# RWAlgorithms/ConjugateGradientOptim.jl

Hardware: NVIDIA B200
Metric: cg_iterations_per_s (higher is better)
Workload: dtype f64

## Files before the change

conjugategradientoptim.jl_b200/csrc/blas1.cu:

```cuda
#include "internal.cuh"
#include "reduce.cuh"

template <class Op>
__global__ void __launch_bounds__(CGO_B, Op::OCC) k_blas1(Op op, int64_t n, RedArgs red) {
    constexpr int K = Op::K;
    __shared__ double sm[K * CGO_NW];
    const int64_t nq = (n + 1) >> 1;
    constexpr int64_t tileq = (int64_t)CGO_B * CGO_U_VEC;
    const int64_t ntiles = (nq + tileq - 1) / tileq;
    const int nact = (int)(ntiles < (int64_t)red.G ? ntiles : (int64_t)red.G);
    cgo_wait_flags(red, BarAll());
    op.prologue();
    for (int v = blockIdx.x; v < nact; v += gridDim.x) {
        double acc[K];
#pragma unroll
        for (int k = 0; k < K; ++k) acc[k] = 0.0;
        for (int64_t tile = v; tile < ntiles; tile += red.G) {
            const int64_t q0 = tile * tileq + threadIdx.x;
            typename Op::In in[CGO_U_VEC];
#pragma unroll
            for (int j = 0; j < CGO_U_VEC; ++j) {
                const int64_t q = q0 + (int64_t)j * CGO_B;
                if (q < nq) in[j] = op.load(q);
            }
#pragma unroll
            for (int j = 0; j < CGO_U_VEC; ++j) {
                const int64_t q = q0 + (int64_t)j * CGO_B;
                if (q < nq) op.apply(q, in[j], acc, 2 * q + 1 < n);
            }
        }
        cgo_cta_combine<K>(acc, sm);
        cgo_publish<K>(red, v, acc);
    }
    cgo_grid_finish<K>(red, nact, sm);
}

template <class Op>
static int launch_blas1(cgo_ctx *c, const Op &op, int64_t n, const RedArgs &red) {
    const int64_t nq = (n + 1) >> 1;
    const int64_t tileq = (int64_t)CGO_B * CGO_U_VEC;
    int64_t ntiles = (nq + tileq - 1) / tileq;
    int64_t nact = ntiles < red.G ? ntiles : red.G;
    int64_t phys = (int64_t)c->sms * Op::OCC;
    int grid = (int)(nact < phys ? nact : phys);
    if (grid < 1) grid = 1;
    cgo_timer_begin(c, Op::TCLASS);
    k_blas1<Op><<<grid, CGO_B, 0, c->stream>>>(op, n, red);
    cgo_timer_end(c);
    c->launches++;
    CGO_CUDA(cudaGetLastError());
    return 0;
}

__device__ __forceinline__ double2 ld2rw(const double2 *p) {
    double2 r;
    asm volatile("ld.global.L1::no_allocate.v2.f64 {%0, %1}, [%2];" : "=d"(r.x), "=d"(r.y) : "l"(p) : "memory");
    return r;
}

template <bool FUSED>
struct RosenTrial {
    static constexpr int TCLASS = CGO_T_TRIAL;
    static constexpr int K = 9;
    static constexpr int OCC = 2;
    struct In { double2 x, u, g; };
    const double2 *x, *g;
    double2 *u;
    double2 *xp, *gp;
    double a, beta;
    __device__ __forceinline__ void prologue() {}
    __device__ __forceinline__ In load(int64_t q) const {
        In r;
        r.x = cgo_ld2(x + q);
        r.g = cgo_ld2(g + q);
        r.u = FUSED ? ld2rw(u + q) : cgo_ld2(u + q);
        return r;
    }
    __device__ __forceinline__ void apply(int64_t q, const In &in, double (&acc)[K], bool) const {
        double2 uu = in.u;
        if (FUSED) {
            uu.x = -in.g.x + beta * in.u.x;
            uu.y = -in.g.y + beta * in.u.y;
            cgo_st2(u + q, uu);
        }
        double2 p;
        p.x = in.x.x + a * uu.x;
        p.y = in.x.y + a * uu.y;
        cgo_st2(xp + q, p);
        const double t = p.y - p.x * p.x;
        const double om = 1.0 - p.x;
        const double f = (100.0 * t) * t + om * om;
        double2 gn;
        gn.x = (-400.0 * p.x) * t - 2.0 * om;
        gn.y = 200.0 * t;
        cgo_st2(gp + q, gn);
        const double y1 = gn.x - in.g.x, y2 = gn.y - in.g.y;
        acc[CGO_P_PHI] = acc[CGO_P_PHI] + f;
        acc[CGO_P_DPHI] = acc[CGO_P_DPHI] + gn.x * uu.x;   acc[CGO_P_DPHI] = acc[CGO_P_DPHI] + gn.y * uu.y;
        acc[CGO_P_GPGP] = acc[CGO_P_GPGP] + gn.x * gn.x;   acc[CGO_P_GPGP] = acc[CGO_P_GPGP] + gn.y * gn.y;
        acc[CGO_P_YY] = acc[CGO_P_YY] + y1 * y1;           acc[CGO_P_YY] = acc[CGO_P_YY] + y2 * y2;
        acc[CGO_P_UY] = acc[CGO_P_UY] + uu.x * y1;         acc[CGO_P_UY] = acc[CGO_P_UY] + uu.y * y2;
        acc[CGO_P_YGP] = acc[CGO_P_YGP] + y1 * gn.x;       acc[CGO_P_YGP] = acc[CGO_P_YGP] + y2 * gn.y;
        acc[CGO_P_GPG] = acc[CGO_P_GPG] + gn.x * in.g.x;   acc[CGO_P_GPG] = acc[CGO_P_GPG] + gn.y * in.g.y;
        acc[CGO_P_UG] = acc[CGO_P_UG] + uu.x * in.g.x;     acc[CGO_P_UG] = acc[CGO_P_UG] + uu.y * in.g.y;
        acc[CGO_P_UU] = acc[CGO_P_UU] + uu.x * uu.x;       acc[CGO_P_UU] = acc[CGO_P_UU] + uu.y * uu.y;
    }
};

template <bool RESET>
struct DirUpdate {
    static constexpr int TCLASS = CGO_T_DIR;
    static constexpr int K = 2;
    static constexpr int OCC = 4;
    struct In { double2 g, u; };
    const double2 *g;
    double2 *u;
    double beta;
    __device__ __forceinline__ void prologue() {}
    __device__ __forceinline__ In load(int64_t q) const {
        In r;
        r.g = cgo_ld2(g + q);
        if (!RESET) r.u = ld2rw(u + q);
        return r;
    }
    __device__ __forceinline__ void apply(int64_t q, const In &in, double (&acc)[K], bool v2) const {
        double2 un;
        if (RESET) { un.x = -in.g.x; un.y = -in.g.y; }
        else { un.x = -in.g.x + beta * in.u.x; un.y = -in.g.y + beta * in.u.y; }
        if (!v2) un.y = 0.0;
        cgo_st2(u + q, un);
        acc[CGO_D_GU] = acc[CGO_D_GU] + in.g.x * un.x;
        acc[CGO_D_UU] = acc[CGO_D_UU] + un.x * un.x;
        if (v2) {
            acc[CGO_D_GU] = acc[CGO_D_GU] + in.g.y * un.y;
            acc[CGO_D_UU] = acc[CGO_D_UU] + un.y * un.y;
        }
    }
};

struct BetaLiteral {
    static constexpr int TCLASS = CGO_T_OTHER;
    static constexpr int K = 1;
    static constexpr int OCC = 2;
    struct In { double2 gp, g, u; };
    const double2 *gp, *g, *u;
    double R, m;
    __device__ __forceinline__ void prologue() {}
    __device__ __forceinline__ In load(int64_t q) const {
        In r;
        r.gp = cgo_ld2(gp + q); r.g = cgo_ld2(g + q); r.u = cgo_ld2(u + q);
        return r;
    }
    __device__ __forceinline__ void apply(int64_t, const In &in, double (&acc)[K], bool v2) const {
        const double y1 = in.gp.x - in.g.x;
        const double t2a = in.gp.x / R;
        const double t1a = y1 - m * in.u.x;
        acc[0] = acc[0] + t1a * t2a;
        if (v2) {
            const double y2 = in.gp.y - in.g.y;
            const double t2b = in.gp.y / R;
            const double t1b = y2 - m * in.u.y;
            acc[0] = acc[0] + t1b * t2b;
        }
    }
};

struct NormUPlusG {
    static constexpr int TCLASS = CGO_T_OTHER;
    static constexpr int K = 1;
    static constexpr int OCC = 4;
    struct In { double2 g, u; };
    const double2 *g, *u;
    __device__ __forceinline__ void prologue() {}
    __device__ __forceinline__ In load(int64_t q) const {
        In r;
        r.g = cgo_ld2(g + q); r.u = cgo_ld2(u + q);
        return r;
    }
    __device__ __forceinline__ void apply(int64_t, const In &in, double (&acc)[K], bool v2) const {
        const double t1 = in.u.x + in.g.x;
        acc[0] = acc[0] + t1 * t1;
        if (v2) { const double t2 = in.u.y + in.g.y; acc[0] = acc[0] + t2 * t2; }
    }
};

template <bool FUSED, int PUSH>
struct AxpyDir {
    static constexpr int TCLASS = CGO_T_AXPY;
    static constexpr int K = 3;
    static constexpr int OCC = 2;
    struct In { double2 x, u, g; };
    const double2 *x, *g;
    double2 *u, *xp;
    double a, beta;
    double2 *prev_right, *next_left;
    int64_t hq, nq;
    void *const *dst_all;
    int nranks;
    __device__ __forceinline__ void prologue() {}
    __device__ __forceinline__ In load(int64_t q) const {
        In r;
        r.x = cgo_ld2(x + q);
        r.g = cgo_ld2(g + q);
        r.u = FUSED ? ld2rw(u + q) : cgo_ld2(u + q);
        return r;
    }
    __device__ __forceinline__ void apply(int64_t q, const In &in, double (&acc)[K], bool v2) const {
        double2 uu = in.u;
        if (FUSED) {
            uu.x = -in.g.x + beta * in.u.x;
            uu.y = v2 ? -in.g.y + beta * in.u.y : 0.0;
            cgo_st2(u + q, uu);
        }
        double2 p;
        p.x = in.x.x + a * uu.x;
        p.y = v2 ? in.x.y + a * uu.y : 0.0;
        cgo_st2(xp + q, p);
        if (PUSH == 1) {
            if (q < hq) cgo_st2(prev_right + q, p);
            if (q >= nq - hq) cgo_st2(next_left + (q - (nq - hq)), p);
        }
        if (PUSH == 2) {
            for (int r = 0; r < nranks; ++r) cgo_st2((double2 *)dst_all[r] + q, p);
        }
        acc[0] = acc[0] + in.g.x * uu.x;
        acc[1] = acc[1] + uu.x * uu.x;
        acc[2] = acc[2] + p.x * p.x;
        if (v2) {
            acc[0] = acc[0] + in.g.y * uu.y;
            acc[1] = acc[1] + uu.y * uu.y;
            acc[2] = acc[2] + p.y * p.y;
        }
    }
};

struct GradCombine {
    static constexpr int TCLASS = CGO_T_OTHER;
    static constexpr int K = 8;
    static constexpr int OCC = 2;
    struct In { double2 s, u, g, w; };
    const double2 *q, *u, *g, *w;
    double2 *gp;
    int nparts;
    int64_t stride2;
    double invN, lambda;
    __device__ __forceinline__ void prologue() {}
    __device__ __forceinline__ In load(int64_t i) const {
        In r;
        r.s = ld2rw(q + i);
        for (int p = 1; p < nparts; ++p) {
            const double2 t = ld2rw(q + (int64_t)p * stride2 + i);
            r.s.x = r.s.x + t.x;
            r.s.y = r.s.y + t.y;
        }
        r.u = cgo_ld2(u + i); r.g = cgo_ld2(g + i); r.w = cgo_ld2(w + i);
        return r;
    }
    __device__ __forceinline__ void apply(int64_t i, const In &in, double (&acc)[K], bool v2) const {
        double2 gn;
        gn.x = in.s.x * invN + lambda * in.w.x;
        gn.y = v2 ? in.s.y * invN + lambda * in.w.y : 0.0;
        cgo_st2(gp + i, gn);
        const double ux = in.u.x, uy = v2 ? in.u.y : 0.0, gx = in.g.x, gy = v2 ? in.g.y : 0.0;
        const double y1 = gn.x - gx, y2 = gn.y - gy;
        acc[CGO_P_DPHI - 1] = acc[CGO_P_DPHI - 1] + gn.x * ux;
        acc[CGO_P_GPGP - 1] = acc[CGO_P_GPGP - 1] + gn.x * gn.x;
        acc[CGO_P_YY - 1] = acc[CGO_P_YY - 1] + y1 * y1;
        acc[CGO_P_UY - 1] = acc[CGO_P_UY - 1] + ux * y1;
        acc[CGO_P_YGP - 1] = acc[CGO_P_YGP - 1] + y1 * gn.x;
        acc[CGO_P_GPG - 1] = acc[CGO_P_GPG - 1] + gn.x * gx;
        acc[CGO_P_UG - 1] = acc[CGO_P_UG - 1] + ux * gx;
        acc[CGO_P_UU - 1] = acc[CGO_P_UU - 1] + ux * ux;
        if (v2) {
            acc[CGO_P_DPHI - 1] = acc[CGO_P_DPHI - 1] + gn.y * uy;
            acc[CGO_P_GPGP - 1] = acc[CGO_P_GPGP - 1] + gn.y * gn.y;
            acc[CGO_P_YY - 1] = acc[CGO_P_YY - 1] + y2 * y2;
            acc[CGO_P_UY - 1] = acc[CGO_P_UY - 1] + uy * y2;
            acc[CGO_P_YGP - 1] = acc[CGO_P_YGP - 1] + y2 * gn.y;
            acc[CGO_P_GPG - 1] = acc[CGO_P_GPG - 1] + gn.y * gy;
            acc[CGO_P_UG - 1] = acc[CGO_P_UG - 1] + uy * gy;
            acc[CGO_P_UU - 1] = acc[CGO_P_UU - 1] + uy * uy;
        }
    }
};

struct VecSumSq {
    static constexpr int TCLASS = CGO_T_OTHER;
    static constexpr int K = 1;
    static constexpr int OCC = 4;
    struct In { double2 a; };
    const double2 *a;
    __device__ __forceinline__ void prologue() {}
    __device__ __forceinline__ In load(int64_t q) const { return In{cgo_ld2(a + q)}; }
    __device__ __forceinline__ void apply(int64_t, const In &in, double (&acc)[K], bool v2) const {
        acc[0] = acc[0] + in.a.x * in.a.x;
        if (v2) acc[0] = acc[0] + in.a.y * in.a.y;
    }
};
struct Dots3 {
    static constexpr int TCLASS = CGO_T_OTHER;
    static constexpr int K = 3;
    static constexpr int OCC = 4;
    struct In { double2 a, b; };
    const double2 *a, *b;
    __device__ __forceinline__ void prologue() {}
    __device__ __forceinline__ In load(int64_t q) const { return In{cgo_ld2(a + q), cgo_ld2(b + q)}; }
    __device__ __forceinline__ void apply(int64_t, const In &in, double (&acc)[K], bool v2) const {
        acc[0] = acc[0] + in.a.x * in.b.x; acc[1] = acc[1] + in.b.x * in.b.x; acc[2] = acc[2] + in.a.x * in.a.x;
        if (v2) { acc[0] = acc[0] + in.a.y * in.b.y; acc[1] = acc[1] + in.b.y * in.b.y; acc[2] = acc[2] + in.a.y * in.a.y; }
    }
};
struct GradDots {
    static constexpr int TCLASS = CGO_T_OTHER;
    static constexpr int K = 8;
    static constexpr int OCC = 2;
    struct In { double2 gp, g, u; };
    const double2 *gp, *g, *u;
    __device__ __forceinline__ void prologue() {}
    __device__ __forceinline__ In load(int64_t q) const { return In{cgo_ld2(gp + q), cgo_ld2(g + q), cgo_ld2(u + q)}; }
    __device__ __forceinline__ void one(double gn, double gg, double uu, double (&acc)[K]) const {
        const double y = gn - gg;
        acc[CGO_P_DPHI - 1] = acc[CGO_P_DPHI - 1] + gn * uu;
        acc[CGO_P_GPGP - 1] = acc[CGO_P_GPGP - 1] + gn * gn;
        acc[CGO_P_YY - 1] = acc[CGO_P_YY - 1] + y * y;
        acc[CGO_P_UY - 1] = acc[CGO_P_UY - 1] + uu * y;
        acc[CGO_P_YGP - 1] = acc[CGO_P_YGP - 1] + y * gn;
        acc[CGO_P_GPG - 1] = acc[CGO_P_GPG - 1] + gn * gg;
        acc[CGO_P_UG - 1] = acc[CGO_P_UG - 1] + uu * gg;
        acc[CGO_P_UU - 1] = acc[CGO_P_UU - 1] + uu * uu;
    }
    __device__ __forceinline__ void apply(int64_t, const In &in, double (&acc)[K], bool v2) const {
        one(in.gp.x, in.g.x, in.u.x, acc);
        if (v2) one(in.gp.y, in.g.y, in.u.y, acc);
    }
};

template <bool PUSH>
struct LogitLoss {
    static constexpr int TCLASS = CGO_T_OTHER;
    static constexpr int K = 1;
    static constexpr int OCC = 2;
    struct In { double2 z, y; };
    double2 *zc;
    const double2 *y;
    void *const *dst_all;
    int nranks;
    __device__ __forceinline__ void prologue() {}
    __device__ __forceinline__ In load(int64_t q) const { return In{ld2rw(zc + q), cgo_ld2(y + q)}; }
    __device__ __forceinline__ double one(double z, double yy, double (&acc)[K]) const {
        const double t = -yy * z;
        const double e = exp(-fabs(t));
        const double l = (t > 0.0 ? t : 0.0) + log1p(e);
        const double sg = t >= 0.0 ? 1.0 / (1.0 + e) : e / (1.0 + e);
        acc[0] = acc[0] + l;
        return -yy * sg;
    }
    __device__ __forceinline__ void apply(int64_t q, const In &in, double (&acc)[K], bool v2) const {
        double2 c;
        c.x = one(in.z.x, in.y.x, acc);
        c.y = v2 ? one(in.z.y, in.y.y, acc) : 0.0;
        cgo_st2(zc + q, c);
        if (PUSH) for (int r = 0; r < nranks; ++r) cgo_st2((double2 *)dst_all[r] + q, c);
    }
};

struct SolveSysProject {
    static constexpr int TCLASS = CGO_T_OTHER;
    static constexpr int K = 1;
    static constexpr int OCC = 4;
    struct In { double2 b, g; };
    const double2 *base, *gp;
    double2 *xn;
    double m;
    __device__ __forceinline__ void prologue() {}
    __device__ __forceinline__ In load(int64_t q) const {
        In r;
        r.b = ld2rw(base + q); r.g = cgo_ld2(gp + q);
        return r;
    }
    __device__ __forceinline__ void apply(int64_t q, const In &in, double (&acc)[K], bool v2) const {
        double2 o;
        o.x = in.b.x + m * in.g.x;
        o.y = v2 ? in.b.y + m * in.g.y : 0.0;
        cgo_st2(xn + q, o);
        acc[0] = acc[0] + o.x * o.x;
        if (v2) acc[0] = acc[0] + o.y * o.y;
    }
};

struct LbfgsStage {
    static constexpr int TCLASS = CGO_T_LBFGS;
    static constexpr int K = 2;
    static constexpr int OCC = 2;
    struct In { double2 xp, x, gp, g; };
    const double2 *xp, *x, *gp, *g;
    double2 *S, *Y;
    __device__ __forceinline__ void prologue() {}
    __device__ __forceinline__ In load(int64_t q) const {
        In r;
        r.xp = cgo_ld2(xp + q); r.x = cgo_ld2(x + q); r.gp = cgo_ld2(gp + q); r.g = cgo_ld2(g + q);
        return r;
    }
    __device__ __forceinline__ void apply(int64_t q, const In &in, double (&acc)[K], bool v2) const {
        double2 s, y;
        s.x = in.xp.x - in.x.x; y.x = in.gp.x - in.g.x;
        s.y = v2 ? in.xp.y - in.x.y : 0.0; y.y = v2 ? in.gp.y - in.g.y : 0.0;
        cgo_st2(S + q, s); cgo_st2(Y + q, y);
        acc[0] = acc[0] + s.x * y.x; acc[1] = acc[1] + y.x * y.x;
        if (v2) { acc[0] = acc[0] + s.y * y.y; acc[1] = acc[1] + y.y * y.y; }
    }
};

template <int MODE>
struct LbfgsStep {
    static constexpr int TCLASS = CGO_T_LBFGS;
    static constexpr int K = (MODE == 4) ? 2 : 1;
    static constexpr int OCC = 2;
    struct In { double2 q, a, b; };
    double2 *q;
    const double2 *A;
    const double2 *B;
    double2 *uout;
    const double *dprev;
    const double *alpha_dot;
    double rho_prev, gamma;
    double coef;
    __device__ __forceinline__ void prologue() {
        if (MODE == 1 || MODE == 2) coef = rho_prev * __ldcg(dprev);
        if (MODE == 3 || MODE == 4) coef = rho_prev * __ldcg(alpha_dot) - rho_prev * __ldcg(dprev);
    }
    __device__ __forceinline__ In load(int64_t i) const {
        In r;
        if (MODE != 0) r.q = ld2rw(q + i);
        r.a = cgo_ld2(A + i);
        r.b = cgo_ld2(B + i);
        return r;
    }
    __device__ __forceinline__ void apply(int64_t i, const In &in, double (&acc)[K], bool v2) const {
        double2 qn;
        if (MODE == 0) { qn = in.a; }
        else if (MODE == 1 || MODE == 2) { qn.x = in.q.x - coef * in.a.x; qn.y = in.q.y - coef * in.a.y; }
        else { qn.x = in.q.x + in.a.x * coef; qn.y = in.q.y + in.a.y * coef; }
        if (MODE == 2) { qn.x = gamma * qn.x; qn.y = gamma * qn.y; }
        if (!v2) qn.y = 0.0;
        if (MODE == 4) {
            double2 un; un.x = -qn.x; un.y = v2 ? -qn.y : 0.0;
            cgo_st2(uout + i, un);
            acc[0] = acc[0] + in.b.x * un.x; acc[1] = acc[1] + un.x * un.x;
            if (v2) { acc[0] = acc[0] + in.b.y * un.y; acc[1] = acc[1] + un.y * un.y; }
        } else {
            cgo_st2(q + i, qn);
            acc[0] = acc[0] + in.b.x * qn.x;
            if (v2) acc[0] = acc[0] + in.b.y * qn.y;
        }
    }
};

static inline uint64_t h_mix64(uint64_t z) {
    z ^= z >> 30; z *= 0xBF58476D1CE4E5B9ULL;
    z ^= z >> 27; z *= 0x94D049BB133111EBULL;
    z ^= z >> 31;
    return z;
}
double cgo_host_u01(uint64_t seed, uint64_t i, uint64_t k) {
    uint64_t h = h_mix64(seed + 0x9E3779B97F4A7C15ULL);
    h = h_mix64(h ^ (i + 0x9E3779B97F4A7C15ULL));
    h = h_mix64(h ^ (k + 0x632BE59BD9B4E019ULL));
    return (double)(h >> 11) * (1.0 / 9007199254740992.0);
}

struct RosenObj : cgo_obj {
    int eval_trial(cgo_state *st, double a, bool fused, double beta, double *out) override {
        RedArgs red = cgo_red_args(ctx);
        if (fused) {
            RosenTrial<true> op;
            op.x = (const double2 *)st->x; op.g = (const double2 *)st->g; op.u = (double2 *)st->u;
            op.xp = (double2 *)st->xp; op.gp = (double2 *)st->gp; op.a = a; op.beta = beta;
            CGO_TRY(launch_blas1(ctx, op, st->n, red));
        } else {
            RosenTrial<false> op;
            op.x = (const double2 *)st->x; op.g = (const double2 *)st->g; op.u = (double2 *)st->u;
            op.xp = (double2 *)st->xp; op.gp = (double2 *)st->gp; op.a = a; op.beta = 0.0;
            CGO_TRY(launch_blas1(ctx, op, st->n, red));
        }
        CGO_TRY(cgo_finish_pack(ctx, 9, out));
        out[CGO_P_DIR_GU] = out[CGO_P_UG];
        out[CGO_P_DIR_UU] = out[CGO_P_UU];
        return 0;
    }
    double bytes_per_eval() const override { return 8.0 * 5.0 * (double)n_local; }
    void reduction_site(int32_t *V, int32_t *U) const override { *V = 2; *U = CGO_U_VEC; }
    int default_x0(uint64_t seed, double perturb, double *x0) override {
        for (int64_t i = 0; i < n_local; ++i) {
            int64_t gi = offset + i;
            double base = (gi % 2 == 0) ? -1.2 : 1.0;
            x0[i] = perturb != 0.0 ? base + perturb * (2.0 * cgo_host_u01(seed, (uint64_t)gi, 0) - 1.0) : base;
        }
        return 0;
    }
};

__global__ void k_scalar_to_pack(const double *src, double *dst) { *dst = *src; }
struct UserObj : cgo_obj {
    cgo_user_fdf fn = nullptr;
    void *user = nullptr;
    double *d_f = nullptr;
    ~UserObj() override {
        if (ctx && cgo_ctx_alive(ctx)) cudaSetDevice(ctx->device);
        cudaFree(d_f);
    }
    int eval_trial(cgo_state *st, double a, bool fused, double beta, double *out) override {
        CGO_TRY(cgo_blas1_axpy_dir(st, a, fused, beta));
        const int rc = fn(user, (void *)ctx->stream, st->n, offset, st->xp, st->gp, d_f);
        CGO_CHECK(rc == 0, "user objective callback returned %d", rc);
        k_scalar_to_pack<<<1, 1, 0, ctx->stream>>>(d_f, cgo_red_args(ctx, CGO_P_PHI).out);
        ctx->launches++;
        CGO_CUDA(cudaGetLastError());
        CGO_TRY(cgo_blas1_grad_dots(st));
        return cgo_finish_pack(ctx, 12, out);
    }
    double bytes_per_eval() const override { return 8.0 * 6.0 * (double)n_local; }
    void reduction_site(int32_t *V, int32_t *U) const override { *V = 2; *U = CGO_U_VEC; }
    int default_x0(uint64_t, double, double *x0) override {
        for (int64_t i = 0; i < n_local; ++i) x0[i] = 0.0;
        return 0;
    }
};
extern "C" int cgo_obj_user_create(cgo_ctx *ctx, int64_t n_global, cgo_user_fdf fdf, void *user, cgo_obj **out) {
    CGO_CHECK(ctx && fdf && out, "NULL argument");
    CGO_CHECK(n_global >= 2 && n_global % 2 == 0, "user objective: need an even n >= 2 (got %lld; pad with a fixed coordinate)", (long long)n_global);
    CGO_CUDA(cudaSetDevice(ctx->device));
    int64_t lo, hi;
    CGO_TRY(cgo_shard_range(n_global, ctx->nranks, ctx->rank, 2, &lo, &hi));
    UserObj *o = new UserObj();
    o->ctx = ctx; o->fn = fdf; o->user = user;
    o->n_global = n_global; o->offset = lo; o->n_local = hi - lo;
    if (cudaMalloc(&o->d_f, sizeof(double)) != cudaSuccess) { delete o; cgo_set_error("cudaMalloc failed"); return 1; }
    *out = o;
    return 0;
}

struct RosenChainedEval {
    static constexpr int TCLASS = CGO_T_TRIAL;
    static constexpr int K = 9;
    static constexpr int OCC = 2;
    struct In { double2 p, u, g; double pm, pn; };
    const double *xp;
    const double2 *u, *g;
    double2 *gp;
    int64_t offset, n_global, n_local;
    __device__ __forceinline__ void prologue() {}
    __device__ __forceinline__ In load(int64_t q) const {
        In r;
        r.p = cgo_ld2((const double2 *)xp + q);
        r.u = cgo_ld2(u + q); r.g = cgo_ld2(g + q);
        const int64_t i0 = 2 * q, i1 = 2 * q + 1;
        r.pm = offset + i0 > 0 ? __ldg(xp + i0 - 1) : 0.0;
        r.pn = offset + i1 + 1 < n_global ? __ldg(xp + i1 + 1) : 0.0;
        return r;
    }
    __device__ __forceinline__ void dots(double gn, double gg, double uu, double (&acc)[K]) const {
        const double y = gn - gg;
        acc[CGO_P_DPHI] = acc[CGO_P_DPHI] + gn * uu;
        acc[CGO_P_GPGP] = acc[CGO_P_GPGP] + gn * gn;
        acc[CGO_P_YY] = acc[CGO_P_YY] + y * y;
        acc[CGO_P_UY] = acc[CGO_P_UY] + uu * y;
        acc[CGO_P_YGP] = acc[CGO_P_YGP] + y * gn;
        acc[CGO_P_GPG] = acc[CGO_P_GPG] + gn * gg;
        acc[CGO_P_UG] = acc[CGO_P_UG] + uu * gg;
        acc[CGO_P_UU] = acc[CGO_P_UU] + uu * uu;
    }
    __device__ __forceinline__ void apply(int64_t q, const In &in, double (&acc)[K], bool v2) const {
        const int64_t gi0 = offset + 2 * q, gi1 = gi0 + 1;
        const double x0 = in.p.x, x1 = in.p.y;
        const double tm = x0 - in.pm * in.pm;
        const double t0 = x1 - x0 * x0;
        const double t1 = in.pn - x1 * x1;
        const double om0 = 1.0 - x0, om1 = 1.0 - x1;
        double2 gn;
        double g0 = 0.0, f0 = 0.0;
        if (gi0 > 0) g0 = g0 + 200.0 * tm;
        if (gi0 < n_global - 1) { g0 = g0 + (-2.0 * om0 - (400.0 * x0) * t0); f0 = om0 * om0 + (100.0 * t0) * t0; }
        gn.x = g0;
        acc[CGO_P_PHI] = acc[CGO_P_PHI] + f0;
        dots(g0, in.g.x, in.u.x, acc);
        gn.y = 0.0;
        if (v2) {
            double g1 = 0.0, f1 = 0.0;
            g1 = g1 + 200.0 * t0;
            if (gi1 < n_global - 1) { g1 = g1 + (-2.0 * om1 - (400.0 * x1) * t1); f1 = om1 * om1 + (100.0 * t1) * t1; }
            gn.y = g1;
            acc[CGO_P_PHI] = acc[CGO_P_PHI] + f1;
            dots(g1, in.g.y, in.u.y, acc);
        }
        cgo_st2(gp + q, gn);
    }
};

struct RosenChainedObj : cgo_obj {
    int eval_trial(cgo_state *st, double a, bool fused, double beta, double *out) override {
        const int R = ctx->nranks, me = ctx->rank;
        RedArgs red = cgo_red_args(ctx, CGO_P_PHI);
        if (R > 1 && st->peer_x) {
            const int prev = (me + R - 1) % R, next = (me + 1) % R;
            const unsigned long long e = ++ctx->epoch;
            unsigned long long *fprev = (unsigned long long *)ctx->flags_peer[(size_t)prev];
            unsigned long long *fnext = (unsigned long long *)ctx->flags_peer[(size_t)next];
            int64_t plo, phi;
            CGO_TRY(cgo_shard_range(n_global, R, prev, 2, &plo, &phi));
            HaloPush hp;
            hp.prev_right = (double *)st->xpeers[st->xp_alloc][(size_t)prev] + halo + (phi - plo);
            hp.next_left = (double *)st->xpeers[st->xp_alloc][(size_t)next];
            hp.sig_prev = fprev + CGO_F_XP_FROM_NEXT;
            hp.sig_next = fnext + CGO_F_XP_FROM_PREV;
            hp.epoch = e;
            CGO_TRY(cgo_blas1_axpy_dir(st, a, fused, beta, &hp));
            red.wait0 = ctx->flags_local + CGO_F_XP_FROM_PREV; red.wait1 = ctx->flags_local + CGO_F_XP_FROM_NEXT;
            red.wait_val = e;
        } else {
            CGO_TRY(cgo_blas1_axpy_dir(st, a, fused, beta));
            if (R > 1) CGO_TRY(cgo_sendrecv_ring(ctx, st->xp, st->xp + st->n, st->xp + st->n - halo, st->xp - halo, halo));
        }
        RosenChainedEval op;
        op.xp = st->xp; op.u = (const double2 *)st->u; op.g = (const double2 *)st->g; op.gp = (double2 *)st->gp;
        op.offset = offset; op.n_global = n_global; op.n_local = st->n;
        CGO_TRY(launch_blas1(ctx, op, st->n, red));
        return cgo_finish_pack(ctx, 12, out);
    }
    double bytes_per_eval() const override { return 8.0 * 7.0 * (double)n_local; }
    void reduction_site(int32_t *V, int32_t *U) const override { *V = 2; *U = CGO_U_VEC; }
    int default_x0(uint64_t seed, double perturb, double *x0) override {
        for (int64_t i = 0; i < n_local; ++i) {
            int64_t gi = offset + i;
            double base = (gi % 2 == 0) ? -1.2 : 1.0;
            x0[i] = perturb != 0.0 ? base + perturb * (2.0 * cgo_host_u01(seed, (uint64_t)gi, 0) - 1.0) : base;
        }
        return 0;
    }
};
extern "C" int cgo_obj_rosenbrock_chained_create(cgo_ctx *ctx, int64_t n_global, cgo_obj **out) {
    CGO_CHECK(ctx && out, "NULL argument");
    CGO_CHECK(n_global >= 2 && n_global % 2 == 0, "chained Rosenbrock: need an even n >= 2 (got %lld)", (long long)n_global);
    CGO_CHECK(ctx->nranks == 1 || n_global >= 4 * ctx->nranks, "chained Rosenbrock: %d ranks need n >= %d", ctx->nranks, 4 * ctx->nranks);
    int64_t lo, hi;
    CGO_TRY(cgo_shard_range(n_global, ctx->nranks, ctx->rank, 2, &lo, &hi));
    RosenChainedObj *o = new RosenChainedObj();
    o->ctx = ctx;
    o->n_global = n_global;
    o->offset = lo;
    o->n_local = hi - lo;
    o->halo = ctx->nranks > 1 ? 2 : 0;
    for (int q = 0; q < ctx->nranks; ++q) {
        int64_t a, b;
        cgo_shard_range(n_global, ctx->nranks, q, 2, &a, &b);
        if (b - a > o->n_alloc) o->n_alloc = b - a;
    }
    *out = o;
    return 0;
}

extern "C" int cgo_obj_rosenbrock_create(cgo_ctx *ctx, int64_t n_global, cgo_obj **out) {
    CGO_CHECK(ctx && out, "NULL argument");
    CGO_CHECK(n_global >= 2 && n_global % 2 == 0, "extended Rosenbrock needs an even n >= 2 (got %lld)", (long long)n_global);
    RosenObj *o = new RosenObj();
    o->ctx = ctx;
    o->n_global = n_global;
    int64_t lo, hi;
    CGO_TRY(cgo_shard_range(n_global, ctx->nranks, ctx->rank, 2, &lo, &hi));
    o->offset = lo;
    o->n_local = hi - lo;
    *out = o;
    return 0;
}
int cgo_obj::hessvec_dir(cgo_state *, double *) {
    cgo_set_error("this objective has no Hessian-vector product (CSR least squares has)");
    return 2;
}
int cgo_obj::quad_begin(cgo_state *, double *) {
    cgo_set_error("this objective has no quadratic-aware line search (CSR least squares has)");
    return 2;
}
int cgo_obj::quad_accept(cgo_state *, double, double *) {
    cgo_set_error("this objective has no quadratic-aware line search (CSR least squares has)");
    return 2;
}
extern "C" int cgo_quad_begin(cgo_state *st, double out[CGO_PACK_LEN]) {
    CGO_CHECK(st && out, "NULL argument");
    return st->obj->quad_begin(st, out);
}
extern "C" int cgo_quad_accept(cgo_state *st, double a, double out[CGO_PACK_LEN]) {
    CGO_CHECK(st && out, "NULL argument");
    return st->obj->quad_accept(st, a, out);
}
struct ResidualAxpy {
    static constexpr int TCLASS = CGO_T_AXPY;
    static constexpr int K = 1;
    static constexpr int OCC = 4;
    struct In { double2 r, v; };
    double2 *r;
    const double2 *v;
    double a;
    __device__ __forceinline__ void prologue() {}
    __device__ __forceinline__ In load(int64_t q) const {
        In o;
        o.r = ld2rw(r + q); o.v = cgo_ld2(v + q);
        return o;
    }
    __device__ __forceinline__ void apply(int64_t q, const In &in, double (&acc)[K], bool v2) const {
        double2 o;
        o.x = in.r.x + a * in.v.x;
        o.y = v2 ? in.r.y + a * in.v.y : 0.0;
        cgo_st2(r + q, o);
        acc[0] = acc[0] + o.x * o.x;
        if (v2) acc[0] = acc[0] + o.y * o.y;
    }
};
int cgo_blas1_residual_axpy(cgo_ctx *c, double *r, const double *v, double a, int64_t nrows, int slot) {
    ResidualAxpy op;
    op.r = (double2 *)r; op.v = (const double2 *)v; op.a = a;
    return launch_blas1(c, op, nrows, cgo_red_args(c, slot));
}
extern "C" int cgo_hessvec_dir(cgo_state *st, double out[CGO_PACK_LEN]) {
    CGO_CHECK(st && out, "NULL argument");
    if (!st->hv) {
        CGO_CUDA(cudaMalloc(&st->hv, sizeof(double) * (size_t)(st->n + 4)));
        CGO_CUDA(cudaMemsetAsync(st->hv, 0, sizeof(double) * (size_t)(st->n + 4), st->ctx->stream));
    }
    return st->obj->hessvec_dir(st, out);
}
extern "C" int cgo_obj_destroy(cgo_obj *o) {
    delete o;
    return 0;
}
extern "C" int cgo_obj_dims(cgo_obj *o, int64_t *nl, int64_t *ng, int64_t *off) {
    CGO_CHECK(o != nullptr, "NULL objective");
    if (nl) *nl = o->n_local;
    if (ng) *ng = o->n_global;
    if (off) *off = o->offset;
    return 0;
}
extern "C" int cgo_obj_reduction_site(cgo_obj *o, int32_t *V, int32_t *U) {
    CGO_CHECK(o && V && U, "NULL argument");
    o->reduction_site(V, U);
    return 0;
}
extern "C" int cgo_obj_bytes_per_eval(cgo_obj *o, double *bytes) {
    CGO_CHECK(o && bytes, "NULL argument");
    *bytes = o->bytes_per_eval();
    return 0;
}
extern "C" int cgo_obj_default_x0(cgo_obj *o, uint64_t seed, double perturb, double *x0) {
    CGO_CHECK(o && x0, "NULL argument");
    return o->default_x0(seed, perturb, x0);
}

struct BarrierFinish {
    static constexpr int TCLASS = CGO_T_OTHER;
    static constexpr int K = 9;
    static constexpr int OCC = 2;
    struct In { double2 xp, gp, u, g, lo, hi; };
    const double2 *xp, *u, *g, *lo, *hi;
    double2 *gp;
    double t;
    __device__ __forceinline__ void prologue() {}
    __device__ __forceinline__ In load(int64_t q) const {
        In r;
        r.xp = cgo_ld2(xp + q); r.gp = ld2rw(gp + q); r.u = cgo_ld2(u + q); r.g = cgo_ld2(g + q);
        r.lo = cgo_ld2(lo + q); r.hi = cgo_ld2(hi + q);
        return r;
    }
    __device__ __forceinline__ void one(double x, double g0, double uu, double gg, double lb, double ub, double &gn,
                                        double (&acc)[K]) const {
        double fu = x - ub, fl = lb - x;
        if (fu > 0.0) fu = 0.0;
        if (fl > 0.0) fl = 0.0;
        const double term = log(-fu) + log(-fl);
        double dpsi = 0.0 - 1.0 / fu;
        dpsi = dpsi - (-1.0) / fl;
        gn = t * g0 + dpsi;
        const double y = gn - gg;
        acc[CGO_P_PHI] = acc[CGO_P_PHI] + term;
        acc[CGO_P_DPHI] = acc[CGO_P_DPHI] + gn * uu;
        acc[CGO_P_GPGP] = acc[CGO_P_GPGP] + gn * gn;
        acc[CGO_P_YY] = acc[CGO_P_YY] + y * y;
        acc[CGO_P_UY] = acc[CGO_P_UY] + uu * y;
        acc[CGO_P_YGP] = acc[CGO_P_YGP] + y * gn;
        acc[CGO_P_GPG] = acc[CGO_P_GPG] + gn * gg;
        acc[CGO_P_UG] = acc[CGO_P_UG] + uu * gg;
        acc[CGO_P_UU] = acc[CGO_P_UU] + uu * uu;
    }
    __device__ __forceinline__ void apply(int64_t q, const In &in, double (&acc)[K], bool v2) const {
        double2 gn;
        one(in.xp.x, in.gp.x, in.u.x, in.g.x, in.lo.x, in.hi.x, gn.x, acc);
        if (v2) one(in.xp.y, in.gp.y, in.u.y, in.g.y, in.lo.y, in.hi.y, gn.y, acc);
        else gn.y = 0.0;
        cgo_st2(gp + q, gn);
    }
};
struct BoxInfeasible {
    static constexpr int TCLASS = CGO_T_OTHER;
    static constexpr int K = 1;
    static constexpr int OCC = 4;
    struct In { double2 x, lo, hi; };
    const double2 *x, *lo, *hi;
    __device__ __forceinline__ void prologue() {}
    __device__ __forceinline__ In load(int64_t q) const {
        In r;
        r.x = cgo_ld2(x + q); r.lo = cgo_ld2(lo + q); r.hi = cgo_ld2(hi + q);
        return r;
    }
    __device__ __forceinline__ void apply(int64_t, const In &in, double (&acc)[K], bool v2) const {
        if (in.x.x - in.hi.x >= 0.0 || in.lo.x - in.x.x >= 0.0) acc[0] = acc[0] + 1.0;
        if (v2 && (in.x.y - in.hi.y >= 0.0 || in.lo.y - in.x.y >= 0.0)) acc[0] = acc[0] + 1.0;
    }
};

struct BarrierObj : cgo_obj {
    cgo_obj *inner = nullptr;
    double *lo = nullptr, *hi = nullptr;
    double t = 1.0;
    ~BarrierObj() override {
        if (ctx && cgo_ctx_alive(ctx)) cudaSetDevice(ctx->device);
        cudaFree(lo); cudaFree(hi);
    }
    int eval_trial(cgo_state *st, double a, bool fused, double beta, double *out) override {
        double in[CGO_PACK_LEN];
        CGO_TRY(inner->eval_trial(st, a, fused, beta, in));
        BarrierFinish op;
        op.xp = (const double2 *)st->xp; op.gp = (double2 *)st->gp; op.u = (const double2 *)st->u;
        op.g = (const double2 *)st->g; op.lo = (const double2 *)lo; op.hi = (const double2 *)hi; op.t = t;
        CGO_TRY(launch_blas1(ctx, op, st->n, cgo_red_args(ctx)));
        CGO_TRY(cgo_finish_pack(ctx, 9, out));
        out[CGO_P_PHI] = t * in[CGO_P_PHI] + (-out[CGO_P_PHI]);
        out[CGO_P_DIR_GU] = in[CGO_P_DIR_GU];
        out[CGO_P_DIR_UU] = in[CGO_P_DIR_UU];
        out[CGO_P_XPXP] = in[CGO_P_XPXP];
        return 0;
    }
    double bytes_per_eval() const override { return inner->bytes_per_eval() + 8.0 * 7.0 * (double)n_local; }
    void reduction_site(int32_t *V, int32_t *U) const override { *V = 2; *U = CGO_U_VEC; }
    int default_x0(uint64_t seed, double perturb, double *x0) override { return inner->default_x0(seed, perturb, x0); }
};

extern "C" int cgo_obj_box_barrier_create(cgo_ctx *ctx, cgo_obj *inner, const double *lbs, const double *ubs,
                                          double t, cgo_obj **out) {
    CGO_CHECK(ctx && inner && lbs && ubs && out, "NULL argument");
    CGO_CHECK(inner->ctx == ctx, "inner objective belongs to another ctx");
    CGO_CUDA(cudaSetDevice(ctx->device));
    BarrierObj *o = new BarrierObj();
    o->ctx = ctx; o->inner = inner; o->t = t;
    o->n_global = inner->n_global; o->n_local = inner->n_local; o->offset = inner->offset;
    o->halo = inner->halo; o->n_alloc = inner->n_alloc;
    const size_t len = (size_t)(o->n_local + 4);
    auto body = [&]() -> int {
        CGO_CUDA(cudaMalloc(&o->lo, sizeof(double) * len));
        CGO_CUDA(cudaMalloc(&o->hi, sizeof(double) * len));
        CGO_CUDA(cudaMemsetAsync(o->lo, 0, sizeof(double) * len, ctx->stream));
        CGO_CUDA(cudaMemsetAsync(o->hi, 0, sizeof(double) * len, ctx->stream));
        CGO_CUDA(cudaMemcpyAsync(o->lo, lbs, sizeof(double) * (size_t)o->n_local, cudaMemcpyHostToDevice, ctx->stream));
        CGO_CUDA(cudaMemcpyAsync(o->hi, ubs, sizeof(double) * (size_t)o->n_local, cudaMemcpyHostToDevice, ctx->stream));
        CGO_CUDA(cudaStreamSynchronize(ctx->stream));
        return 0;
    };
    int rc = body();
    if (rc) { delete o; return rc; }
    *out = o;
    return 0;
}
extern "C" int cgo_obj_barrier_set_t(cgo_obj *obj, double t) {
    BarrierObj *o = dynamic_cast<BarrierObj *>(obj);
    CGO_CHECK(o != nullptr, "not a barrier objective");
    o->t = t;
    return 0;
}
extern "C" int cgo_obj_barrier_infeasible(cgo_obj *obj, const double *x_host, int64_t *count) {
    BarrierObj *o = dynamic_cast<BarrierObj *>(obj);
    CGO_CHECK(o && x_host && count, "not a barrier objective / NULL argument");
    cgo_ctx *c = o->ctx;
    CGO_CUDA(cudaSetDevice(c->device));
    double *dx = nullptr;
    auto body = [&]() -> int {
        CGO_CUDA(cudaMalloc(&dx, sizeof(double) * (size_t)(o->n_local + 4)));
        CGO_CUDA(cudaMemsetAsync(dx, 0, sizeof(double) * (size_t)(o->n_local + 4), c->stream));
        CGO_CUDA(cudaMemcpyAsync(dx, x_host, sizeof(double) * (size_t)o->n_local, cudaMemcpyHostToDevice, c->stream));
        BoxInfeasible op;
        op.x = (const double2 *)dx; op.lo = (const double2 *)o->lo; op.hi = (const double2 *)o->hi;
        CGO_TRY(launch_blas1(c, op, o->n_local, cgo_red_args(c)));
        double v[CGO_PACK_LEN];
        CGO_TRY(cgo_finish_pack(c, 1, v));
        *count = (int64_t)v[0];
        return 0;
    };
    int rc = body();
    cudaFree(dx);
    return rc;
}

static size_t vec_bytes(const cgo_state *st) { return sizeof(double) * (size_t)(st->n + 2 * st->halo + 4); }
static int alloc_vec(cgo_state *st, double **base, double **ptr) {
    void *p = nullptr;
    CGO_TRY(cgo_dev_alloc(st->ctx, vec_bytes(st), &p));
    *base = (double *)p;
    *ptr = *base + st->halo;
    return 0;
}

extern "C" int cgo_state_destroy(cgo_state *st) {
    if (!st) return 0;
    if (cgo_ctx_alive(st->ctx)) {
        cudaSetDevice(st->ctx->device);
        cudaStreamSynchronize(st->ctx->stream);
    } else {
        cudaDeviceSynchronize();
    }
    if (st->peer_x) {
        for (int k = 0; k < 2; ++k) {
            if (st->xpeers[k].size() != (size_t)st->ctx->nranks) continue;
            double *mine = (double *)st->xpeers[k][(size_t)st->ctx->rank];
            for (int i = 0; i < 5; ++i) if (st->base[i] == mine) st->base[i] = nullptr;
            cgo_peer_free(st->ctx, mine, st->xpeers[k], true);
        }
    }
    for (int i = 0; i < 5; ++i) cgo_dev_free(st->ctx, st->base[i], vec_bytes(st));
    const size_t hist_bytes = sizeof(double) * (size_t)(st->n + 4);
    for (auto p : st->S) cgo_dev_free(st->ctx, p, hist_bytes);
    for (auto p : st->Y) cgo_dev_free(st->ctx, p, hist_bytes);
    cgo_dev_free(st->ctx, st->q, hist_bytes);
    cudaFree(st->xn);
    cudaFree(st->hv);
    delete st;
    return 0;
}

static int state_create(cgo_ctx *ctx, cgo_obj *obj, const double *x0, bool x0_on_device, int32_t lbfgs_m,
                        cgo_state **out_state, double out[CGO_PACK_LEN]) {
    CGO_CHECK(ctx && obj && x0 && out_state && out, "cgo_state_create: NULL argument");
    CGO_CHECK(obj->ctx == ctx, "objective belongs to another ctx");
    CGO_CHECK(lbfgs_m >= 0 && lbfgs_m <= CGO_LBFGS_MAX_M, "lbfgs_m=%d out of [0,%d]", lbfgs_m, CGO_LBFGS_MAX_M);
    CGO_CHECK(obj->halo % 2 == 0, "halo must be even");
    CGO_CUDA(cudaSetDevice(ctx->device));
    cgo_state *st = new cgo_state();
    st->ctx = ctx; st->obj = obj; st->n = obj->n_local; st->halo = obj->halo;
    auto body = [&]() -> int {
        double **ptrs[5] = {&st->x, &st->g, &st->u, &st->xp, &st->gp};
        st->peer_x = ctx->nranks > 1 && ctx->peer_ok && st->halo > 0;
        for (int i = 0; i < 5; ++i) {
            if (st->peer_x && (i == 0 || i == 3)) {
                void *p = nullptr;
                const int64_t len = (obj->n_alloc > st->n ? obj->n_alloc : st->n) + 2 * st->halo + 4;
                CGO_TRY(cgo_peer_alloc(ctx, sizeof(double) * (size_t)len, &p, st->xpeers[i == 0 ? 0 : 1]));
                st->base[i] = (double *)p;
                *ptrs[i] = st->base[i] + st->halo;
            } else {
                CGO_TRY(alloc_vec(st, &st->base[i], ptrs[i]));
            }
        }
        st->xp_alloc = 1;
        st->m = lbfgs_m;
        if (lbfgs_m > 0) {
            const size_t hist_bytes = sizeof(double) * (size_t)(st->n + 4);
            for (int k = 0; k < lbfgs_m; ++k) {
                void *s = nullptr, *y = nullptr;
                CGO_TRY(cgo_dev_alloc(ctx, hist_bytes, &s));
                st->S.push_back((double *)s);
                CGO_TRY(cgo_dev_alloc(ctx, hist_bytes, &y));
                st->Y.push_back((double *)y);
            }
            st->rho.assign(lbfgs_m, 0.0);
            void *q = nullptr;
            CGO_TRY(cgo_dev_alloc(ctx, hist_bytes, &q));
            st->q = (double *)q;
        }
        CGO_CUDA(cudaMemcpyAsync(st->x, x0, sizeof(double) * (size_t)st->n,
                                 x0_on_device ? cudaMemcpyDeviceToDevice : cudaMemcpyHostToDevice, ctx->stream));
        CGO_TRY(obj->eval_trial(st, 0.0, false, 0.0, out));
        return 0;
    };
    const int rc = body();
    if (rc) { cgo_state_destroy(st); return rc; }
    cgo_accept(st);
    *out_state = st;
    return 0;
}
extern "C" int cgo_state_create(cgo_ctx *ctx, cgo_obj *obj, const double *x0, int32_t lbfgs_m,
                                cgo_state **out_state, double out[CGO_PACK_LEN]) {
    return state_create(ctx, obj, x0, false, lbfgs_m, out_state, out);
}
extern "C" int cgo_state_create_from_state(cgo_ctx *ctx, cgo_obj *obj, cgo_state *src, int32_t which, int32_t lbfgs_m,
                                           cgo_state **out_state, double out[CGO_PACK_LEN]) {
    CGO_CHECK(src != nullptr, "cgo_state_create_from_state: NULL source state");
    CGO_CHECK(src->ctx == ctx && src->n == (obj ? obj->n_local : -1), "source state belongs to another ctx or has another dimension");
    double *v[5] = {src->x, src->g, src->u, src->xp, src->gp};
    CGO_CHECK(which >= 0 && which < 5, "which=%d out of range", which);
    return state_create(ctx, obj, v[which], true, lbfgs_m, out_state, out);
}

extern "C" int cgo_accept(cgo_state *st) {
    CGO_CHECK(st != nullptr, "NULL state");
    std::swap(st->x, st->xp);
    std::swap(st->g, st->gp);
    std::swap(st->base[0], st->base[3]);
    std::swap(st->base[1], st->base[4]);
    st->xp_alloc ^= 1;
    st->obj->on_accept(st);
    return 0;
}

extern "C" int cgo_eval_trial(cgo_state *st, double a, double out[CGO_PACK_LEN]) {
    CGO_CHECK(st && out, "NULL argument");
    return st->obj->eval_trial(st, a, false, 0.0, out);
}
extern "C" int cgo_eval_trial_fused_dir(cgo_state *st, double beta, double a, double out[CGO_PACK_LEN]) {
    CGO_CHECK(st && out, "NULL argument");
    return st->obj->eval_trial(st, a, true, beta, out);
}

extern "C" int cgo_update_dir(cgo_state *st, double beta, double out[CGO_PACK_LEN]) {
    CGO_CHECK(st && out, "NULL argument");
    DirUpdate<false> op;
    op.g = (const double2 *)st->g; op.u = (double2 *)st->u; op.beta = beta;
    CGO_TRY(launch_blas1(st->ctx, op, st->n, cgo_red_args(st->ctx)));
    return cgo_finish_pack(st->ctx, 2, out);
}
extern "C" int cgo_reset_direction(cgo_state *st, double out[CGO_PACK_LEN]) {
    CGO_CHECK(st && out, "NULL argument");
    DirUpdate<true> op;
    op.g = (const double2 *)st->g; op.u = (double2 *)st->u; op.beta = 0.0;
    CGO_TRY(launch_blas1(st->ctx, op, st->n, cgo_red_args(st->ctx)));
    return cgo_finish_pack(st->ctx, 2, out);
}
extern "C" int cgo_beta_literal(cgo_state *st, double R, double m, double *beta_out) {
    CGO_CHECK(st && beta_out, "NULL argument");
    BetaLiteral op;
    op.gp = (const double2 *)st->gp; op.g = (const double2 *)st->g; op.u = (const double2 *)st->u;
    op.R = R; op.m = m;
    CGO_TRY(launch_blas1(st->ctx, op, st->n, cgo_red_args(st->ctx)));
    double tmp[CGO_PACK_LEN];
    CGO_TRY(cgo_finish_pack(st->ctx, 1, tmp));
    *beta_out = tmp[0];
    return 0;
}
extern "C" int cgo_norm_sq_u_plus_g(cgo_state *st, double *outv) {
    CGO_CHECK(st && outv, "NULL argument");
    NormUPlusG op;
    op.g = (const double2 *)st->g; op.u = (const double2 *)st->u;
    CGO_TRY(launch_blas1(st->ctx, op, st->n, cgo_red_args(st->ctx)));
    double tmp[CGO_PACK_LEN];
    CGO_TRY(cgo_finish_pack(st->ctx, 1, tmp));
    *outv = tmp[0];
    return 0;
}

template <bool FUSED, int PUSH>
static int launch_axpy_dir(cgo_state *st, double a, double beta, const HaloPush *push) {
    cgo_ctx *c = st->ctx;
    RedArgs red = cgo_red_args(c, CGO_P_DIR_GU);
    AxpyDir<FUSED, PUSH> op;
    op.x = (const double2 *)st->x; op.g = (const double2 *)st->g; op.u = (double2 *)st->u;
    op.xp = (double2 *)st->xp; op.a = a; op.beta = FUSED ? beta : 0.0;
    op.prev_right = op.next_left = nullptr; op.hq = 0; op.nq = st->n / 2;
    op.dst_all = nullptr; op.nranks = c->nranks;
    if (PUSH == 1) {
        op.prev_right = (double2 *)push->prev_right; op.next_left = (double2 *)push->next_left;
        op.hq = st->halo / 2;
        red.sig0 = push->sig_prev; red.sig1 = push->sig_next; red.sig_val = push->epoch;
    }
    if (PUSH == 2) {
        op.dst_all = push->dst_all;
        red.flags_all = c->d_flags_peer; red.sig_all_slot = CGO_F_XPALL; red.nranks = c->nranks; red.me = c->rank;
        red.sig_val = push->epoch;
    }
    return launch_blas1(c, op, st->n, red);
}
int cgo_blas1_axpy_dir(cgo_state *st, double a, bool fused, double beta, const HaloPush *push) {
    if (push && push->dst_all)
        return fused ? launch_axpy_dir<true, 2>(st, a, beta, push) : launch_axpy_dir<false, 2>(st, a, beta, push);
    if (push) return fused ? launch_axpy_dir<true, 1>(st, a, beta, push) : launch_axpy_dir<false, 1>(st, a, beta, push);
    return fused ? launch_axpy_dir<true, 0>(st, a, beta, nullptr) : launch_axpy_dir<false, 0>(st, a, beta, nullptr);
}

int cgo_blas1_sumsq(cgo_ctx *c, const double *a, int64_t n, int slot) {
    VecSumSq op;
    op.a = (const double2 *)a;
    return launch_blas1(c, op, n, cgo_red_args(c, slot));
}
int cgo_blas1_dots3(cgo_ctx *c, const double *a, const double *b, int64_t n, int slot) {
    Dots3 op;
    op.a = (const double2 *)a; op.b = (const double2 *)b;
    return launch_blas1(c, op, n, cgo_red_args(c, slot));
}
int cgo_blas1_logit(cgo_ctx *c, double *zc, const double *y, int64_t n, int slot, void *const *dst_all, unsigned long long epoch) {
    RedArgs red = cgo_red_args(c, slot);
    if (dst_all) {
        LogitLoss<true> op;
        op.zc = (double2 *)zc; op.y = (const double2 *)y; op.dst_all = dst_all; op.nranks = c->nranks;
        red.flags_all = c->d_flags_peer; red.sig_all_slot = CGO_F_GPART; red.nranks = c->nranks; red.me = c->rank;
        red.sig_val = epoch;
        return launch_blas1(c, op, n, red);
    }
    LogitLoss<false> op;
    op.zc = (double2 *)zc; op.y = (const double2 *)y; op.dst_all = nullptr; op.nranks = 1;
    return launch_blas1(c, op, n, red);
}
int cgo_blas1_grad_dots(cgo_state *st) {
    GradDots op;
    op.gp = (const double2 *)st->gp; op.g = (const double2 *)st->g; op.u = (const double2 *)st->u;
    return launch_blas1(st->ctx, op, st->n, cgo_red_args(st->ctx, CGO_P_DPHI));
}

int cgo_blas1_grad_combine(cgo_state *st, const double *q, int nparts, int64_t stride, double invN, double lambda,
                           unsigned long long wait_epoch) {
    GradCombine op;
    op.q = (const double2 *)q; op.u = (const double2 *)st->u; op.g = (const double2 *)st->g;
    op.w = (const double2 *)st->xp; op.gp = (double2 *)st->gp;
    op.nparts = nparts; op.stride2 = stride / 2; op.invN = invN; op.lambda = lambda;
    RedArgs red = cgo_red_args(st->ctx, CGO_P_DPHI);
    if (wait_epoch) {
        red.wait_all = st->ctx->flags_local + CGO_F_GPART; red.wait_val = wait_epoch; red.nranks = st->ctx->nranks;
    }
    return launch_blas1(st->ctx, op, st->n, red);
}

extern "C" int cgo_solvesys_begin(cgo_state *st) {
    CGO_CHECK(st != nullptr, "NULL state");
    cudaStream_t s = st->ctx->stream;
    if (!st->xn) CGO_CUDA(cudaMalloc(&st->xn, sizeof(double) * (size_t)(st->n + 4)));
    CGO_CUDA(cudaMemsetAsync(st->xn, 0, sizeof(double) * (size_t)(st->n + 4), s));
    CGO_CUDA(cudaMemcpyAsync(st->xn, st->x, sizeof(double) * (size_t)st->n, cudaMemcpyDeviceToDevice, s));
    return 0;
}
extern "C" int cgo_solvesys_project(cgo_state *st, double m, int32_t fix_stale_iterate, double out[CGO_PACK_LEN]) {
    CGO_CHECK(st && out, "NULL argument");
    CGO_CHECK(st->xn != nullptr, "cgo_solvesys_project before cgo_solvesys_begin");
    SolveSysProject op;
    op.base = (const double2 *)(fix_stale_iterate ? st->x : st->xn);
    op.gp = (const double2 *)st->gp; op.xn = (double2 *)st->xn; op.m = m;
    CGO_TRY(launch_blas1(st->ctx, op, st->n, cgo_red_args(st->ctx, CGO_PACK_LEN - 1)));
    double *x_saved = st->x;
    st->x = st->xn;
    int rc = st->obj->eval_trial(st, 0.0, false, 0.0, out);
    st->x = x_saved;
    return rc;
}
extern "C" int cgo_solvesys_accept(cgo_state *st, int32_t fix_stale_iterate) {
    CGO_CHECK(st != nullptr, "NULL state");
    CGO_TRY(cgo_accept(st));
    if (!fix_stale_iterate)
        CGO_CUDA(cudaMemcpyAsync(st->xn, st->xp, sizeof(double) * (size_t)st->n, cudaMemcpyDeviceToDevice, st->ctx->stream));
    return 0;
}

extern "C" int cgo_lbfgs_stage_pair(cgo_state *st, double out[CGO_PACK_LEN]) {
    CGO_CHECK(st && out, "NULL argument");
    CGO_CHECK(st->m > 0, "state was created without an L-BFGS history (lbfgs_m = 0)");
    int slot = (st->count == 0) ? 0 : (st->head + 1) % st->m;
    LbfgsStage op;
    op.xp = (const double2 *)st->xp; op.x = (const double2 *)st->x;
    op.gp = (const double2 *)st->gp; op.g = (const double2 *)st->g;
    op.S = (double2 *)st->S[slot]; op.Y = (double2 *)st->Y[slot];
    CGO_TRY(launch_blas1(st->ctx, op, st->n, cgo_red_args(st->ctx)));
    st->staged = slot;
    return cgo_finish_pack(st->ctx, 2, out);
}
extern "C" int cgo_lbfgs_commit_pair(cgo_state *st, int32_t commit, double rho, double gamma) {
    CGO_CHECK(st != nullptr, "NULL state");
    CGO_CHECK(st->staged >= 0, "cgo_lbfgs_commit_pair without a staged pair");
    if (commit) {
        st->head = st->staged;
        if (st->count < st->m) st->count++;
        st->rho[st->staged] = rho;
        st->gamma = gamma;
    } else if (st->count == st->m) {
        st->count--;
    }
    st->staged = -1;
    return 0;
}

static RedArgs red_to_slot(cgo_ctx *c, int slot) {
    RedArgs r = cgo_red_args(c);
    r.out = (c->nranks > 1) ? c->d_pack : c->d_scal + slot;
    return r;
}
static int publish_slot(cgo_ctx *c, int slot) {
    if (c->nranks > 1) CGO_TRY(cgo_combine_ranks(c, 1, c->d_scal + slot));
    return 0;
}

extern "C" int cgo_lbfgs_update_dir(cgo_state *st, double out[CGO_PACK_LEN]) {
    CGO_CHECK(st && out, "NULL argument");
    CGO_CHECK(st->m > 0, "state was created without an L-BFGS history (lbfgs_m = 0)");
    cgo_ctx *c = st->ctx;
    if (st->count == 0) return cgo_reset_direction(st, out);
    const int cnt = st->count, m = st->m;
    auto slot_of = [&](int k) { return ((st->head - k) % m + m) % m; };
    double2 *q = (double2 *)st->q;
    for (int k = 0; k < cnt; ++k) {
        int s = slot_of(k);
        if (k == 0) {
            LbfgsStep<0> op{};
            op.q = q; op.A = (const double2 *)st->g; op.B = (const double2 *)st->S[s];
            CGO_TRY(launch_blas1(c, op, st->n, red_to_slot(c, k)));
        } else {
            int sp = slot_of(k - 1);
            LbfgsStep<1> op{};
            op.q = q; op.A = (const double2 *)st->Y[sp]; op.B = (const double2 *)st->S[s];
            op.dprev = c->d_scal + (k - 1); op.rho_prev = st->rho[sp];
            CGO_TRY(launch_blas1(c, op, st->n, red_to_slot(c, k)));
        }
        CGO_TRY(publish_slot(c, k));
    }
    {
        int sp = slot_of(cnt - 1);
        LbfgsStep<2> op{};
        op.q = q; op.A = (const double2 *)st->Y[sp]; op.B = (const double2 *)st->Y[sp];
        op.dprev = c->d_scal + (cnt - 1); op.rho_prev = st->rho[sp]; op.gamma = st->gamma;
        CGO_TRY(launch_blas1(c, op, st->n, red_to_slot(c, 64 + cnt - 1)));
        CGO_TRY(publish_slot(c, 64 + cnt - 1));
    }
    for (int k = cnt - 2; k >= 0; --k) {
        int sp = slot_of(k + 1), s = slot_of(k);
        LbfgsStep<3> op{};
        op.q = q; op.A = (const double2 *)st->S[sp]; op.B = (const double2 *)st->Y[s];
        op.dprev = c->d_scal + 64 + (k + 1); op.alpha_dot = c->d_scal + (k + 1); op.rho_prev = st->rho[sp];
        CGO_TRY(launch_blas1(c, op, st->n, red_to_slot(c, 64 + k)));
        CGO_TRY(publish_slot(c, 64 + k));
    }
    {
        int sp = slot_of(0);
        LbfgsStep<4> op{};
        op.q = q; op.A = (const double2 *)st->S[sp]; op.B = (const double2 *)st->g; op.uout = (double2 *)st->u;
        op.dprev = c->d_scal + 64; op.alpha_dot = c->d_scal; op.rho_prev = st->rho[sp];
        CGO_TRY(launch_blas1(c, op, st->n, cgo_red_args(c)));
    }
    return cgo_finish_pack(c, 2, out);
}

extern "C" int cgo_download(cgo_state *st, double *x_host, double *g_host) {
    CGO_CHECK(st != nullptr, "NULL state");
    cudaStream_t s = st->ctx->stream;
    if (x_host) CGO_CUDA(cudaMemcpyAsync(x_host, st->x, sizeof(double) * (size_t)st->n, cudaMemcpyDeviceToHost, s));
    if (g_host) CGO_CUDA(cudaMemcpyAsync(g_host, st->g, sizeof(double) * (size_t)st->n, cudaMemcpyDeviceToHost, s));
    CGO_CUDA(cudaStreamSynchronize(s));
    return 0;
}
extern "C" int cgo_download_vector(cgo_state *st, int32_t which, double *host) {
    CGO_CHECK(st && host, "NULL argument");
    double *src[6] = {st->x, st->g, st->u, st->xp, st->gp, st->hv};
    CGO_CHECK(which >= 0 && which < 6 && src[which] != nullptr, "which=%d out of range (5 = hv needs cgo_hessvec_dir first)", which);
    CGO_CUDA(cudaMemcpyAsync(host, src[which], sizeof(double) * (size_t)st->n, cudaMemcpyDeviceToHost, st->ctx->stream));
    CGO_CUDA(cudaStreamSynchronize(st->ctx->stream));
    return 0;
}
```

conjugategradientoptim.jl_b200/csrc/csr.cu:

```cuda
#include <cub/device/device_scan.cuh>

#include "internal.cuh"
#include "reduce.cuh"


constexpr int CSR_PAD = 16;

__device__ __forceinline__ double ld_stream_f64(const double *p) {
    double r;
    asm volatile("ld.global.nc.L1::no_allocate.f64 %0, [%1];" : "=d"(r) : "l"(p));
    return r;
}
__device__ __forceinline__ int32_t ld_stream_s32(const int32_t *p) {
    int32_t r;
    asm volatile("ld.global.nc.L1::no_allocate.s32 %0, [%1];" : "=r"(r) : "l"(p));
    return r;
}
__device__ __forceinline__ void st_stream_f64(double *p, double v) {
    asm volatile("st.global.L1::no_allocate.f64 [%0], %1;" ::"l"(p), "d"(v) : "memory");
}

__device__ __forceinline__ uint32_t smem_u32(const void *p) { return (uint32_t)__cvta_generic_to_shared(p); }
__device__ __forceinline__ void mbar_init(uint64_t *b, uint32_t count) {
    asm volatile("mbarrier.init.shared::cta.b64 [%0], %1;" ::"r"(smem_u32(b)), "r"(count) : "memory");
}
__device__ __forceinline__ void mbar_expect_tx(uint64_t *b, uint32_t bytes) {
    asm volatile("mbarrier.arrive.expect_tx.shared::cta.b64 _, [%0], %1;" ::"r"(smem_u32(b)), "r"(bytes) : "memory");
}
__device__ __forceinline__ void mbar_arrive(uint64_t *b) {
    asm volatile("mbarrier.arrive.shared::cta.b64 _, [%0];" ::"r"(smem_u32(b)) : "memory");
}
__device__ __forceinline__ void mbar_wait(uint64_t *b, uint32_t parity) {
    asm volatile(
        "{\n"
        ".reg .pred P1;\n"
        "LAB_WAIT:\n"
        "mbarrier.try_wait.parity.shared::cta.b64 P1, [%0], %1;\n"
        "@P1 bra DONE;\n"
        "bra LAB_WAIT;\n"
        "DONE:\n"
        "}\n" ::"r"(smem_u32(b)), "r"(parity) : "memory");
}
__device__ __forceinline__ uint64_t l2_policy_evict_first() {
    uint64_t pol;
    asm volatile("createpolicy.fractional.L2::evict_first.b64 %0, 1.0;" : "=l"(pol));
    return pol;
}
__device__ __forceinline__ void tma_load_1d(void *dst, const void *src, uint32_t bytes, uint64_t *bar, uint64_t pol) {
    asm volatile(
        "cp.async.bulk.shared::cluster.global.mbarrier::complete_tx::bytes.L2::cache_hint [%0], [%1], %2, [%3], %4;"
        ::"r"(smem_u32(dst)), "l"(src), "r"(bytes), "r"(smem_u32(bar)), "l"(pol) : "memory");
}

constexpr int TS_ND = 3;
constexpr int TS_THREADS = CGO_B + 32;
constexpr int TS_OCC = 2;
constexpr int TS_UN = 10;
constexpr int TS_SMEM_BUDGET = 115200;
template <int NOPS, int OCC = TS_OCC>
struct TsLayout {
    static constexpr int BUDGET = OCC == 2 ? TS_SMEM_BUDGET : (228 * 1024) / OCC - 1024 - 256;
    static constexpr int RP_BYTES = (CGO_B + 2) * 8;
    static constexpr int OP_BYTES = CGO_B * 8;
    static constexpr int DESC_BYTES = RP_BYTES + NOPS * OP_BYTES;
    static constexpr int TAIL_BYTES = 2 * TS_ND * 8 + TS_ND * 4 + CGO_MAXK * CGO_NW * 8;
    static constexpr int RING = ((BUDGET - TS_ND * DESC_BYTES - TAIL_BYTES - 64) / 12) & ~3;
    static constexpr int CHMAX = (RING / 2) & ~3;
    static constexpr int OFF_VAL = 0;
    static constexpr int OFF_COL = OFF_VAL + RING * 8;
    static constexpr int OFF_DESC = (OFF_COL + RING * 4 + 15) & ~15;
    static constexpr int OFF_BAR = OFF_DESC + TS_ND * DESC_BYTES;
    static constexpr int OFF_LEN = OFF_BAR + 2 * TS_ND * 8;
    static constexpr int OFF_RED = (OFF_LEN + TS_ND * 4 + 15) & ~15;
    static constexpr int BYTES = OFF_RED + CGO_MAXK * CGO_NW * 8;
    static_assert(BYTES <= BUDGET && RP_BYTES % 16 == 0 && DESC_BYTES % 16 == 0, "smem layout");
};

__device__ __forceinline__ bool ts_next_tile(int &v, int64_t &tile, int nact, int64_t ntiles, int G) {
    tile += G;
    if (tile < ntiles) return true;
    v += gridDim.x;
    if (v >= nact) return false;
    tile = v;
    return true;
}
__device__ __forceinline__ uint64_t l2_policy_evict_last() {
    uint64_t pol;
    asm volatile("createpolicy.fractional.L2::evict_last.b64 %0, 1.0;" : "=l"(pol));
    return pol;
}
__device__ __forceinline__ double ld_gather_f64(const double *p, uint64_t pol) {
    double r;
    asm volatile("ld.global.nc.L2::cache_hint.f64 %0, [%1], %2;" : "=d"(r) : "l"(p), "l"(pol));
    return r;
}
__device__ __forceinline__ double ld_gather_f64_if(const double *p, uint64_t pol, bool on) {
    double r = 0.0;
    asm volatile(
        "{\n"
        ".reg .pred q;\n"
        "setp.ne.s32 q, %3, 0;\n"
        "@q ld.global.nc.L2::cache_hint.f64 %0, [%1], %2;\n"
        "}\n" : "+d"(r) : "l"(p), "l"(pol), "r"((int)on));
    return r;
}

template <class L, class Epi>
__device__ __forceinline__ void ts_produce(const CsrMat &A, const Epi &epi, const RedArgs &red,
                                           double *s_val, int32_t *s_col, unsigned char *s_desc, uint64_t *s_full,
                                           uint64_t *s_empty, uint32_t *s_len, int nact, int64_t ntiles) {
    constexpr int NOPS = Epi::NOPS;
    constexpr int RING = L::RING, CHMAX = L::CHMAX;
    const int64_t nrows = A.nrows;
    const uint64_t pol = l2_policy_evict_first();
    uint32_t c = 0, tail = 0;
    uint32_t head = 0, nfree = RING;
    int v = blockIdx.x;
    int64_t tile = v;
    bool have = true;
    int nvalid_n = (int)(nrows - tile * CGO_B < CGO_B ? nrows - tile * CGO_B : CGO_B);
    int64_t p0n = __ldg(A.rowptr + tile * CGO_B), p1n = __ldg(A.rowptr + tile * CGO_B + nvalid_n);
    while (have) {
        const int64_t r0 = tile * CGO_B, p0 = p0n, p1 = p1n;
        const int nvalid = nvalid_n;
        have = ts_next_tile(v, tile, nact, ntiles, red.G);
        if (have) {
            nvalid_n = (int)(nrows - tile * CGO_B < CGO_B ? nrows - tile * CGO_B : CGO_B);
            p0n = __ldg(A.rowptr + tile * CGO_B);
            p1n = __ldg(A.rowptr + tile * CGO_B + nvalid_n);
        }
        bool first = true;
        for (int64_t cs = p0 & ~(int64_t)3; first || cs < p1; cs += CHMAX) {
            const int64_t ce = cs + CHMAX < p1 ? cs + CHMAX : p1;
            const uint32_t cnt4 = p1 > p0 ? (uint32_t)((ce - cs + 3) & ~(int64_t)3) : 0u;
            while (tail + TS_ND <= c || nfree < cnt4) {
                mbar_wait(&s_empty[tail % TS_ND], (tail / TS_ND) & 1);
                nfree += s_len[tail % TS_ND];
                ++tail;
            }
            const int d = c % TS_ND;
            s_len[d] = cnt4;
            nfree -= cnt4;
            unsigned char *desc = s_desc + d * L::DESC_BYTES;
            const uint32_t rpb = first ? (uint32_t)((((nvalid + 1) * 8) + 15) & ~15) : 0u;
            const uint32_t opb = first ? (uint32_t)(((nvalid * 8) + 15) & ~15) : 0u;
            mbar_expect_tx(&s_full[d], cnt4 * 12u + rpb + NOPS * opb);
            if (first) {
                tma_load_1d(desc, A.rowptr + r0, rpb, &s_full[d], pol);
#pragma unroll
                for (int o = 0; o < NOPS; ++o)
                    tma_load_1d(desc + L::RP_BYTES + o * L::OP_BYTES, epi.operand(o) + r0, opb, &s_full[d], pol);
            }
            if (cnt4) {
                const uint32_t n1 = cnt4 < RING - head ? cnt4 : RING - head;
                tma_load_1d(s_val + head, A.val + cs, n1 * 8u, &s_full[d], pol);
                tma_load_1d(s_col + head, A.col + cs, n1 * 4u, &s_full[d], pol);
                if (n1 < cnt4) {
                    tma_load_1d(s_val, A.val + cs + n1, (cnt4 - n1) * 8u, &s_full[d], pol);
                    tma_load_1d(s_col, A.col + cs + n1, (cnt4 - n1) * 4u, &s_full[d], pol);
                }
                head += cnt4;
                if (head >= RING) head -= RING;
            }
            first = false;
            ++c;
        }
    }
}

template <class Epi, int OCC>
__global__ void __launch_bounds__(TS_THREADS, OCC)
k_csr_rows(CsrMat A, const double *__restrict__ xg, Epi epi, RedArgs red) {
    constexpr int K = Epi::K;
    constexpr int NOPS = Epi::NOPS;
    using L = TsLayout<NOPS, OCC>;
    constexpr int RING = L::RING, CHMAX = L::CHMAX;
    extern __shared__ __align__(128) unsigned char smem_raw[];
    double *s_val = reinterpret_cast<double *>(smem_raw + L::OFF_VAL);
    int32_t *s_col = reinterpret_cast<int32_t *>(smem_raw + L::OFF_COL);
    unsigned char *s_desc = smem_raw + L::OFF_DESC;
    uint64_t *s_full = reinterpret_cast<uint64_t *>(smem_raw + L::OFF_BAR);
    uint64_t *s_empty = s_full + TS_ND;
    uint32_t *s_len = reinterpret_cast<uint32_t *>(smem_raw + L::OFF_LEN);
    double *s_red = reinterpret_cast<double *>(smem_raw + L::OFF_RED);
    const int tid = threadIdx.x;
    const int64_t nrows = A.nrows;
    const int64_t ntiles = (nrows + CGO_B - 1) / CGO_B;
    const int nact = (int)(ntiles < (int64_t)red.G ? ntiles : (int64_t)red.G);
    if (tid == 0) {
        for (int s = 0; s < TS_ND; ++s) { mbar_init(&s_full[s], 1); mbar_init(&s_empty[s], CGO_NW); }
        asm volatile("fence.mbarrier_init.release.cluster;" ::: "memory");
    }
    __syncthreads();

    if (tid >= CGO_B) {
        if (tid == CGO_B && (int)blockIdx.x < nact)
            ts_produce<L, Epi>(A, epi, red, s_val, s_col, s_desc, s_full, s_empty, s_len, nact, ntiles);
        return;
    }

    const BarLanes bar;
    cgo_wait_flags(red, bar);
    const uint64_t gpol = l2_policy_evict_last();
    uint32_t c = 0, head = 0;
    for (int v = blockIdx.x; v < nact; v += gridDim.x) {
        double acc[K];
#pragma unroll
        for (int k = 0; k < K; ++k) acc[k] = 0.0;
        for (int64_t tile = v; tile < ntiles; tile += red.G) {
            const int64_t r0 = tile * CGO_B;
            const int nvalid = (int)(nrows - r0 < CGO_B ? nrows - r0 : CGO_B);
            const bool valid = tid < nvalid;
            typename Epi::Pre pre;
            int64_t rs = 0, re = 0, p0 = 0, p1 = 0, cs = 0;
            double sum = 0.0;
            bool first = true;
            do {
                const int d = c % TS_ND;
                mbar_wait(&s_full[d], (c / TS_ND) & 1);
                if (first) {
                    const unsigned char *desc = s_desc + d * L::DESC_BYTES;
                    const int64_t *rp = reinterpret_cast<const int64_t *>(desc);
                    if (valid) {
                        rs = rp[tid]; re = rp[tid + 1];
                        pre = epi.load(reinterpret_cast<const double *>(desc + L::RP_BYTES), tid);
                        if (Epi::HAS_INIT) sum = epi.init(pre);
                    }
                    p0 = rp[0];
                    p1 = rp[nvalid];
                    cs = p0 & ~(int64_t)3;
                    first = false;
                }
                const int64_t ce = cs + CHMAX < p1 ? cs + CHMAX : p1;
                const uint32_t cnt4 = p1 > p0 ? (uint32_t)((ce - cs + 3) & ~(int64_t)3) : 0u;
                const int lo = (int)((rs > cs ? rs : cs) - cs);
                const int hi = (int)((re < ce ? re : ce) - cs);
                for (int k0 = lo; k0 < hi; k0 += TS_UN) {
                    double vj[TS_UN], xj[TS_UN];
#pragma unroll
                    for (int j = 0; j < TS_UN; ++j) {
                        const int kk = k0 + j < hi ? k0 + j : hi - 1;
                        uint32_t idx = head + (uint32_t)kk;
                        if (idx >= RING) idx -= RING;
                        vj[j] = s_val[idx];
                        xj[j] = ld_gather_f64_if(xg + s_col[idx], gpol, k0 + j < hi);
                    }
#pragma unroll
                    for (int j = 0; j < TS_UN; ++j) {
                        const double t = sum + vj[j] * xj[j];
                        sum = k0 + j < hi ? t : sum;
                    }
                }
                __syncwarp();
                if ((tid & 31) == 0) mbar_arrive(&s_empty[d]);
                head += cnt4;
                if (head >= RING) head -= RING;
                ++c;
                cs += CHMAX;
            } while (cs < p1);
            if (valid) epi.row(r0 + tid, sum, pre, acc);
        }
        cgo_cta_combine<K, BarLanes>(acc, s_red, bar);
        cgo_publish<K>(red, v, acc);
    }
    cgo_grid_finish<K, BarLanes>(red, nact, s_red, bar);
}

template <class Epi, int OCC>
static int launch_csr_occ(cgo_ctx *c, const CsrMat &A, const double *xg, const Epi &epi, const RedArgs &red, int tclass) {
    const int64_t ntiles = (A.nrows + CGO_B - 1) / CGO_B;
    int64_t nact = ntiles < red.G ? ntiles : red.G;
    int64_t phys = (int64_t)c->sms * OCC;
    int grid = (int)(nact < phys ? nact : phys);
    if (grid < 1) grid = 1;
    CGO_CHECK(!A.sliced, "internal: k_csr_rows on a matrix in the sliced layout");
    const size_t smem = TsLayout<Epi::NOPS, OCC>::BYTES;
    CGO_CUDA(cudaFuncSetAttribute(k_csr_rows<Epi, OCC>, cudaFuncAttributeMaxDynamicSharedMemorySize, (int)smem));
    cgo_timer_begin(c, tclass);
    k_csr_rows<Epi, OCC><<<grid, TS_THREADS, smem, c->stream>>>(A, xg, epi, red);
    cgo_timer_end(c);
    c->launches++;
    CGO_CUDA(cudaGetLastError());
    return 0;
}
template <class Epi>
static int launch_csr(cgo_ctx *c, const CsrMat &A, const double *xg, const Epi &epi, const RedArgs &red, int tclass) {
    return launch_csr_occ<Epi, TS_OCC>(c, A, xg, epi, red, tclass);
}
template <class Epi>
static int launch_csr_pass(cgo_ctx *c, const CsrMat &A, const double *xg, const Epi &epi, const RedArgs &red, int tclass) {
    if (c->csr_pass_occ == 3) return launch_csr_occ<Epi, 3>(c, A, xg, epi, red, tclass);
    return launch_csr_occ<Epi, TS_OCC>(c, A, xg, epi, red, tclass);
}

struct EpiStore {
    static constexpr int K = 1, NOPS = 0;
    static constexpr bool HAS_INIT = false;
    struct Pre {};
    __device__ __forceinline__ double init(const Pre &) const { return 0.0; }
    double *y;
    __device__ __forceinline__ const double *operand(int) const { return nullptr; }
    __device__ __forceinline__ Pre load(const double *, int) const { return Pre(); }
    __device__ __forceinline__ void row(int64_t i, double sum, const Pre &, double (&)[K]) const { y[i] = sum; }
};
template <bool PUSH>
struct EpiResidualT {
    static constexpr int K = 1, NOPS = 1;
    static constexpr bool HAS_INIT = false;
    struct Pre { double b; };
    __device__ __forceinline__ double init(const Pre &) const { return 0.0; }
    const double *b;
    double *r;
    double *prev_right, *next_left;
    int64_t halo, nrows;
    __device__ __forceinline__ const double *operand(int) const { return b; }
    __device__ __forceinline__ Pre load(const double *ops, int t) const { return Pre{ops[t]}; }
    __device__ __forceinline__ void row(int64_t i, double sum, const Pre &p, double (&acc)[K]) const {
        const double rr = sum - p.b;
        r[i] = rr;
        if (PUSH) {
            if (i < halo) prev_right[i] = rr;
            if (i >= nrows - halo) next_left[i - (nrows - halo)] = rr;
        }
        acc[0] = acc[0] + rr * rr;
    }
};
template <bool LOGREG>
struct EpiGrad {
    static constexpr int K = 8, NOPS = LOGREG ? 3 : 2;
    static constexpr bool HAS_INIT = false;
    struct Pre { double u, g, w; };
    __device__ __forceinline__ double init(const Pre &) const { return 0.0; }
    double *gp;
    const double *g, *u, *w;
    double invN, lambda;
    __device__ __forceinline__ const double *operand(int o) const { return o == 0 ? u : (o == 1 ? g : w); }
    __device__ __forceinline__ Pre load(const double *ops, int t) const {
        Pre p;
        p.u = ops[t]; p.g = ops[CGO_B + t];
        p.w = LOGREG ? ops[2 * CGO_B + t] : 0.0;
        return p;
    }
    __device__ __forceinline__ void row(int64_t j, double sum, const Pre &p, double (&acc)[K]) const {
        double gn = sum;
        if (LOGREG) gn = sum * invN + lambda * p.w;
        st_stream_f64(gp + j, gn);
        const double uu = p.u, gg = p.g;
        const double y = gn - gg;
        acc[CGO_P_DPHI - 1] = acc[CGO_P_DPHI - 1] + gn * uu;
        acc[CGO_P_GPGP - 1] = acc[CGO_P_GPGP - 1] + gn * gn;
        acc[CGO_P_YY - 1] = acc[CGO_P_YY - 1] + y * y;
        acc[CGO_P_UY - 1] = acc[CGO_P_UY - 1] + uu * y;
        acc[CGO_P_YGP - 1] = acc[CGO_P_YGP - 1] + y * gn;
        acc[CGO_P_GPG - 1] = acc[CGO_P_GPG - 1] + gn * gg;
        acc[CGO_P_UG - 1] = acc[CGO_P_UG - 1] + uu * gg;
        acc[CGO_P_UU - 1] = acc[CGO_P_UU - 1] + uu * uu;
    }
};
struct EpiLogit {
    static constexpr int K = 1, NOPS = 1;
    static constexpr bool HAS_INIT = false;
    struct Pre { double y; };
    __device__ __forceinline__ double init(const Pre &) const { return 0.0; }
    const double *label;
    double *c;
    __device__ __forceinline__ const double *operand(int) const { return label; }
    __device__ __forceinline__ Pre load(const double *ops, int t) const { return Pre{ops[t]}; }
    __device__ __forceinline__ void row(int64_t i, double z, const Pre &p, double (&acc)[K]) const {
        const double y = p.y;
        const double t = -y * z;
        const double e = exp(-fabs(t));
        const double l = (t > 0.0 ? t : 0.0) + log1p(e);
        const double sg = t >= 0.0 ? 1.0 / (1.0 + e) : e / (1.0 + e);
        c[i] = -y * sg;
        acc[0] = acc[0] + l;
    }
};

struct EpiStoreSq {
    static constexpr int K = 1, NOPS = 0;
    static constexpr bool HAS_INIT = false;
    struct Pre {};
    __device__ __forceinline__ double init(const Pre &) const { return 0.0; }
    double *y;
    __device__ __forceinline__ const double *operand(int) const { return nullptr; }
    __device__ __forceinline__ Pre load(const double *, int) const { return Pre(); }
    __device__ __forceinline__ void row(int64_t i, double sum, const Pre &, double (&acc)[K]) const {
        y[i] = sum;
        acc[0] = acc[0] + sum * sum;
    }
};
struct EpiHv {
    static constexpr int K = 2, NOPS = 1;
    static constexpr bool HAS_INIT = false;
    struct Pre { double u; };
    __device__ __forceinline__ double init(const Pre &) const { return 0.0; }
    double *hv;
    const double *u;
    __device__ __forceinline__ const double *operand(int) const { return u; }
    __device__ __forceinline__ Pre load(const double *ops, int t) const { return Pre{ops[t]}; }
    __device__ __forceinline__ void row(int64_t j, double sum, const Pre &p, double (&acc)[K]) const {
        hv[j] = sum;
        acc[0] = acc[0] + p.u * sum;
        acc[1] = acc[1] + sum * sum;
    }
};

struct EpiQuadV {
    static constexpr int K = 3, NOPS = 1;
    static constexpr bool HAS_INIT = false;
    struct Pre { double r; };
    __device__ __forceinline__ double init(const Pre &) const { return 0.0; }
    double *v;
    const double *r;
    __device__ __forceinline__ const double *operand(int) const { return r; }
    __device__ __forceinline__ Pre load(const double *ops, int t) const { return Pre{ops[t]}; }
    __device__ __forceinline__ void row(int64_t i, double sum, const Pre &p, double (&acc)[K]) const {
        v[i] = sum;
        acc[0] = acc[0] + p.r * sum;
        acc[1] = acc[1] + sum * sum;
        acc[2] = acc[2] + p.r * p.r;
    }
};

template <class Base>
struct WithInit : Base {
    static constexpr int K = Base::K, NOPS = Base::NOPS + 1;
    static constexpr bool HAS_INIT = true;
    struct Pre { typename Base::Pre base; double init; };
    const double *partial;
    __device__ __forceinline__ const double *operand(int o) const { return o < Base::NOPS ? Base::operand(o) : partial; }
    __device__ __forceinline__ Pre load(const double *ops, int t) const {
        Pre p;
        p.base = Base::load(ops, t);
        p.init = ops[Base::NOPS * CGO_B + t];
        return p;
    }
    __device__ __forceinline__ double init(const Pre &p) const { return p.init; }
    __device__ __forceinline__ void row(int64_t i, double sum, const Pre &p, double (&acc)[K]) const {
        Base::row(i, sum, p.base, acc);
    }
};
template <class Base>
static WithInit<Base> with_init(const Base &b, const double *partial) {
    WithInit<Base> w;
    static_cast<Base &>(w) = b;
    w.partial = partial;
    return w;
}

constexpr int DIR_GRAB = 4;
struct DirArgs {
    unsigned long long *next;
    unsigned int *ticket;
    unsigned long long *sig0, *sig1;
    const unsigned long long *wait0, *wait1;
    unsigned long long sig_val, wait_val;
    void *const *flags_all;
    const unsigned long long *wait_all;
    int sig_all_slot, nranks, me;
};
__device__ __forceinline__ int32_t ld_stream_s32_if(const int32_t *p, bool on) {
    int32_t r = 0;
    asm volatile("{\n.reg .pred q;\nsetp.ne.s32 q, %2, 0;\n@q ld.global.nc.L1::no_allocate.s32 %0, [%1];\n}\n" : "+r"(r) : "l"(p), "r"((int)on));
    return r;
}
__device__ __forceinline__ double ld_stream_f64_if(const double *p, bool on) {
    double r = 0.0;
    asm volatile("{\n.reg .pred q;\nsetp.ne.s32 q, %2, 0;\n@q ld.global.nc.L1::no_allocate.f64 %0, [%1];\n}\n" : "+d"(r) : "l"(p), "r"((int)on));
    return r;
}

template <int UN, bool UNIFORM>
__device__ __forceinline__ double dir_batch(const CsrMat &A, const double *__restrict__ xg, uint64_t gpol, int64_t sb,
                                            int64_t &off, int len, int k0, int lane, uint32_t lt, double sum) {
    int32_t cj[UN];
    double vj[UN], xj[UN];
#pragma unroll
    for (int j = 0; j < UN; ++j) {
        const bool on = len > k0 + j;
        int64_t idx;
        if (UNIFORM) { idx = sb + off + lane; off += 32; }
        else {
            const uint32_t m = __ballot_sync(0xffffffffu, on);
            idx = sb + off + __popc(m & lt);
            off += __popc(m);
        }
        cj[j] = ld_stream_s32_if(A.col + idx, on);
        vj[j] = ld_stream_f64_if(A.val + idx, on);
    }
#pragma unroll
    for (int j = 0; j < UN; ++j) xj[j] = ld_gather_f64_if(xg + cj[j], gpol, len > k0 + j);
#pragma unroll
    for (int j = 0; j < UN; ++j) {
        const double p = vj[j] * xj[j];
        if (len > k0 + j) sum = sum + p;
    }
    return sum;
}

template <class F, int UN, int OCC>
__global__ void __launch_bounds__(CGO_B, OCC)
k_spmv_direct(CsrMat A, const double *__restrict__ xg, F f, DirArgs da) {
    const int tid = threadIdx.x, lane = tid & 31;
    const uint32_t lt = (1u << lane) - 1u;
    const int64_t nrows = A.nrows, nslices = (nrows + 31) / 32;
    if (da.wait0 != nullptr || da.wait_all != nullptr) {
        if (tid == 0 && da.wait0 != nullptr) {
            cgo_spin_until(da.wait0, da.wait_val);
            if (da.wait1 != nullptr) cgo_spin_until(da.wait1, da.wait_val);
        }
        if (da.wait_all != nullptr && tid < da.nranks) cgo_spin_until(da.wait_all + tid, da.wait_val);
        __syncthreads();
    }
    const uint64_t gpol = l2_policy_evict_last();
    for (;;) {
        unsigned long long s0 = 0;
        if (lane == 0) s0 = atomicAdd(da.next, (unsigned long long)DIR_GRAB);
        s0 = __shfl_sync(0xffffffffu, s0, 0);
        if ((int64_t)s0 >= nslices) break;
#pragma unroll 1
        for (int g = 0; g < DIR_GRAB; ++g) {
            const int64_t s = (int64_t)s0 + g;
            if (s >= nslices) break;
            const int64_t row = s * 32 + lane;
            const bool valid = row < nrows;
            int64_t rp0 = 0, rp1 = 0;
            if (valid) { rp0 = __ldg(A.rowptr + row); rp1 = __ldg(A.rowptr + row + 1); }
            const int len = valid ? (int)(rp1 - rp0) : -1;
            const int64_t sb = __shfl_sync(0xffffffffu, rp0, 0);
            const int maxlen = __reduce_max_sync(0xffffffffu, len);
            const bool uniform = __all_sync(0xffffffffu, len == maxlen);
            double sum = valid ? f.init(row) : 0.0;
            int64_t off = 0;
            if (uniform) { for (int k0 = 0; k0 < maxlen; k0 += UN) sum = dir_batch<UN, true>(A, xg, gpol, sb, off, len, k0, lane, lt, sum); }
            else { for (int k0 = 0; k0 < maxlen; k0 += UN) sum = dir_batch<UN, false>(A, xg, gpol, sb, off, len, k0, lane, lt, sum); }
            if (valid) f.row(row, sum);
        }
    }
    __shared__ bool is_last;
    if (da.sig0 != nullptr || da.flags_all != nullptr) __threadfence_system();
    else __threadfence();
    __syncthreads();
    if (tid == 0) is_last = atomicAdd(da.ticket, 1u) == gridDim.x - 1;
    __syncthreads();
    if (is_last && tid == 0) {
        *da.ticket = 0u;
        *da.next = 0ULL;
        __threadfence_system();
        if (da.sig0 != nullptr) {
            cgo_st_release_sys(da.sig0, da.sig_val);
            if (da.sig1 != nullptr) cgo_st_release_sys(da.sig1, da.sig_val);
        }
        if (da.flags_all != nullptr)
            for (int r = 0; r < da.nranks; ++r)
                cgo_st_release_sys((unsigned long long *)da.flags_all[r] + da.sig_all_slot + da.me, da.sig_val);
    }
}

struct DirStore {
    double *y;
    __device__ __forceinline__ double init(int64_t) const { return 0.0; }
    __device__ __forceinline__ void row(int64_t i, double sum) const { y[i] = sum; }
};
struct DirStoreInit {
    double *y;
    const double *partial;
    __device__ __forceinline__ double init(int64_t i) const { return ld_stream_f64(partial + i); }
    __device__ __forceinline__ void row(int64_t i, double sum) const { y[i] = sum; }
};
template <bool PUSH>
struct DirResidual {
    const double *b;
    double *r;
    double *prev_right, *next_left;
    int64_t halo, nrows;
    __device__ __forceinline__ double init(int64_t) const { return 0.0; }
    __device__ __forceinline__ void row(int64_t i, double sum) const {
        const double rr = sum - ld_stream_f64(b + i);
        r[i] = rr;
        if (PUSH) {
            if (i < halo) prev_right[i] = rr;
            if (i >= nrows - halo) next_left[i - (nrows - halo)] = rr;
        }
    }
};
struct DirGradLS {
    double *gp;
    __device__ __forceinline__ double init(int64_t) const { return 0.0; }
    __device__ __forceinline__ void row(int64_t j, double sum) const { st_stream_f64(gp + j, sum); }
};

static DirArgs dir_args(cgo_ctx *c, const RedArgs *red = nullptr) {
    DirArgs d;
    d.next = c->d_progress + 4;
    d.ticket = c->d_ticket + 1;
    d.sig0 = d.sig1 = nullptr; d.wait0 = d.wait1 = nullptr; d.sig_val = d.wait_val = 0;
    d.flags_all = nullptr; d.wait_all = nullptr; d.sig_all_slot = -1; d.nranks = 1; d.me = 0;
    if (red) {
        d.sig0 = red->sig0; d.sig1 = red->sig1; d.wait0 = red->wait0; d.wait1 = red->wait1;
        d.sig_val = red->sig_val; d.wait_val = red->wait_val;
        d.flags_all = red->flags_all; d.wait_all = red->wait_all; d.sig_all_slot = red->sig_all_slot;
        d.nranks = red->nranks; d.me = red->me;
    }
    return d;
}
template <class F, int UN, int OCC>
static int launch_direct_k(cgo_ctx *c, const CsrMat &A, const double *xg, const F &f, const DirArgs &da, int tclass) {
    const int64_t nslices = (A.nrows + 31) / 32;
    int64_t want = (nslices + 8 * DIR_GRAB - 1) / (8 * DIR_GRAB), phys = (int64_t)c->sms * OCC;
    int grid = (int)(want < phys ? want : phys);
    if (grid < 1) grid = 1;
    cgo_timer_begin(c, tclass);
    k_spmv_direct<F, UN, OCC><<<grid, CGO_B, 0, c->stream>>>(A, xg, f, da);
    cgo_timer_end(c);
    c->launches++;
    CGO_CUDA(cudaGetLastError());
    return 0;
}
template <class F>
static int launch_direct(cgo_ctx *c, const CsrMat &A, const double *xg, const F &f, const DirArgs &da, int tclass) {
    CGO_CHECK(A.sliced, "internal: k_spmv_direct needs the sliced layout");
    const int cfg = c->direct_cfg ? c->direct_cfg : (A.ragged ? 3 : 2);
    if (cfg == 1) return launch_direct_k<F, 8, 4>(c, A, xg, f, da, tclass);
    if (cfg == 3) return launch_direct_k<F, 6, 5>(c, A, xg, f, da, tclass);
    return launch_direct_k<F, 10, 4>(c, A, xg, f, da, tclass);
}

__host__ __device__ __forceinline__ uint64_t g_mix64(uint64_t z) {
    z ^= z >> 30; z *= 0xBF58476D1CE4E5B9ULL;
    z ^= z >> 27; z *= 0x94D049BB133111EBULL;
    z ^= z >> 31;
    return z;
}
__host__ __device__ __forceinline__ uint64_t g_hash3(uint64_t seed, uint64_t i, uint64_t k) {
    uint64_t h = g_mix64(seed + 0x9E3779B97F4A7C15ULL);
    h = g_mix64(h ^ (i + 0x9E3779B97F4A7C15ULL));
    h = g_mix64(h ^ (k + 0x632BE59BD9B4E019ULL));
    return h;
}
__host__ __device__ __forceinline__ double g_u01(uint64_t seed, uint64_t i, uint64_t k) {
    return (double)(g_hash3(seed, i, k) >> 11) * (1.0 / 9007199254740992.0);
}

struct LsSpec {
    int64_t n;
    int32_t K;
    int32_t coh;
    int64_t W, w;
    uint64_t seed;
    __host__ __device__ __forceinline__ void entry(int64_t i, int k, int64_t &d, double &v) const {
        if (k == 0) { d = 0; v = 4.0 + g_u01(seed, (uint64_t)i, 0); return; }
        const int64_t lo = -W + (int64_t)(k - 1) * w;
        d = lo + (int64_t)(g_hash3(seed ^ 0xA5A5A5A5A5A5A5A5ULL, (uint64_t)(i >> coh), (uint64_t)k) % (uint64_t)w);
        if (d == 0) d = (lo + w > 1) ? 1 : -1;
        v = 0.3 * (2.0 * g_u01(seed, (uint64_t)i, (uint64_t)k) - 1.0);
    }
    __host__ __device__ __forceinline__ int64_t wrap(int64_t c) const {
        if (c < 0) c += n;
        if (c >= n) c -= n;
        return c;
    }
};
struct LrSpec {
    int64_t N, d;
    int32_t K;
    int64_t w;
    uint64_t seed;
    __host__ __device__ __forceinline__ void entry(int64_t i, int k, int64_t &c, double &v) const {
        c = (int64_t)k * w + (int64_t)(g_hash3(seed, (uint64_t)i, (uint64_t)k) % (uint64_t)w);
        v = 2.0 * g_u01(seed + 7, (uint64_t)i, (uint64_t)k) - 1.0;
    }
};

static inline int grid_for(int64_t items, int sms) {
    int64_t b = (items + 255) / 256;
    int64_t cap = (int64_t)sms * 32;
    return (int)(b < 1 ? 1 : (b < cap ? b : cap));
}
#define GRID_STRIDE(idx, total) \
    for (int64_t idx = (int64_t)blockIdx.x * blockDim.x + threadIdx.x; idx < (total); idx += (int64_t)gridDim.x * blockDim.x)

__global__ void k_ls_fill_A(LsSpec s, int64_t lo, int64_t nloc, bool unwrapped, CsrMat A) {
    const int64_t total = nloc * s.K;
    GRID_STRIDE(p, total) {
        const int64_t il = p / s.K;
        const int k = (int)(p - il * s.K);
        int64_t d; double v;
        s.entry(lo + il, k, d, v);
        A.col[p] = (int32_t)(unwrapped ? il + d : s.wrap(lo + il + d));
        A.val[p] = v;
        if (k == 0) A.rowptr[il] = p;
        if (p == total - 1) A.rowptr[nloc] = total;
    }
}
__global__ void k_ls_xtrue(LsSpec s, int64_t lo, int64_t nloc, int64_t halo, double *xt ) {
    GRID_STRIDE(e, nloc + 2 * halo) {
        int64_t i = s.wrap(lo - halo + e);
        xt[e - halo] = 2.0 * g_u01(s.seed + 1, (uint64_t)i, 0) - 1.0;
    }
}
__global__ void k_lr_fill_A(LrSpec s, int64_t i0, int64_t nloc, CsrMat A, double *label) {
    GRID_STRIDE(il, nloc) {
        const int64_t i = i0 + il;
        const int64_t p = il * s.K;
        A.rowptr[il] = p;
        double acc = 0.0;
        for (int k = 0; k < s.K; ++k) {
            int64_t c; double v;
            s.entry(i, k, c, v);
            A.col[p + k] = (int32_t)c;
            A.val[p + k] = v;
            const double wt = 2.0 * g_u01(s.seed + 2, (uint64_t)c, 0) - 1.0;
            acc += v * wt;
        }
        const double noise = 2.0 * g_u01(s.seed + 3, (uint64_t)i, 0) - 1.0;
        label[il] = (acc + 0.1 * noise >= 0.0) ? 1.0 : -1.0;
        if (il == nloc - 1) A.rowptr[nloc] = nloc * s.K;
    }
}

struct CsrSrc {
    const int32_t *col;
    int64_t total;
    __device__ __forceinline__ bool get(int64_t e, int64_t &trow, int64_t &key) const {
        trow = col[e]; key = e;
        return true;
    }
};
struct LsExtSrc {
    LsSpec s;
    int64_t lo, hi, total;
    __device__ __forceinline__ bool get(int64_t e, int64_t &trow, int64_t &key) const {
        const int64_t ie = e / s.K;
        const int k = (int)(e - ie * s.K);
        const int64_t i = s.wrap(lo - s.W + ie);
        int64_t d; double v;
        s.entry(i, k, d, v);
        const int64_t c = s.wrap(i + d);
        if (c < lo || c >= hi) return false;
        trow = c - lo; key = i * s.K + k;
        return true;
    }
};
template <class Src>
__global__ void k_tr_count(Src src, unsigned long long *counts) {
    GRID_STRIDE(e, src.total) {
        int64_t trow, key;
        if (src.get(e, trow, key)) atomicAdd(counts + trow, 1ULL);
    }
}
template <class Src>
__global__ void k_tr_fill(Src src, unsigned long long *cursor, int64_t *perm) {
    GRID_STRIDE(e, src.total) {
        int64_t trow, key;
        if (src.get(e, trow, key)) perm[atomicAdd(cursor + trow, 1ULL)] = key;
    }
}
__global__ void k_tr_sort(const int64_t *rowptrT, int64_t nT, int64_t *perm) {
    GRID_STRIDE(j, nT) {
        int64_t *a = perm + rowptrT[j];
        const int64_t L = rowptrT[j + 1] - rowptrT[j];
        if (L <= 48) {
            for (int64_t i = 1; i < L; ++i) {
                const int64_t key = a[i];
                int64_t q = i - 1;
                while (q >= 0 && a[q] > key) { a[q + 1] = a[q]; --q; }
                a[q + 1] = key;
            }
        } else {
            for (int64_t start = L / 2 - 1; start >= 0; --start) {
                int64_t root = start;
                for (;;) {
                    int64_t ch = 2 * root + 1;
                    if (ch >= L) break;
                    if (ch + 1 < L && a[ch] < a[ch + 1]) ++ch;
                    if (a[root] >= a[ch]) break;
                    int64_t t = a[root]; a[root] = a[ch]; a[ch] = t;
                    root = ch;
                }
            }
            for (int64_t end = L - 1; end > 0; --end) {
                int64_t t = a[0]; a[0] = a[end]; a[end] = t;
                int64_t root = 0;
                for (;;) {
                    int64_t ch = 2 * root + 1;
                    if (ch >= end) break;
                    if (ch + 1 < end && a[ch] < a[ch + 1]) ++ch;
                    if (a[root] >= a[ch]) break;
                    int64_t t2 = a[root]; a[root] = a[ch]; a[ch] = t2;
                    root = ch;
                }
            }
        }
    }
}
struct CsrFin {
    const int64_t *rowptr;
    int64_t nrows;
    const double *val;
    __device__ __forceinline__ void get(int64_t key, int32_t &srow, double &v) const {
        int64_t lo = 0, hi = nrows;
        while (hi - lo > 1) {
            int64_t mid = (lo + hi) >> 1;
            if (rowptr[mid] <= key) lo = mid; else hi = mid;
        }
        srow = (int32_t)lo; v = val[key];
    }
};
struct FixedKFin {
    int32_t K;
    const double *val;
    __device__ __forceinline__ void get(int64_t key, int32_t &srow, double &v) const {
        srow = (int32_t)(key / K); v = val[key];
    }
};
struct LsExtFin {
    LsSpec s;
    int64_t lo;
    __device__ __forceinline__ void get(int64_t key, int32_t &srow, double &v) const {
        const int64_t i = key / s.K;
        const int k = (int)(key - i * s.K);
        int64_t d;
        s.entry(i, k, d, v);
        int64_t rel = i - lo;
        if (rel < -s.W) rel += s.n;
        if (rel >= s.n - s.W) rel -= s.n;
        srow = (int32_t)rel;
    }
};
template <class Fin>
__global__ void k_tr_finalize(Fin fin, int64_t nnzT, const int64_t *perm, CsrMat AT) {
    GRID_STRIDE(q, nnzT) {
        int32_t srow; double v;
        fin.get(perm[q], srow, v);
        AT.col[q] = srow;
        AT.val[q] = v;
    }
}

static void csr_free(CsrMat &M) {
    cudaFree(M.rowptr); cudaFree(M.col); cudaFree(M.val);
    M = CsrMat();
}
static int csr_alloc(CsrMat &M, int64_t nrows, int64_t nnz) {
    M.nrows = nrows; M.nnz = nnz;
    CGO_CUDA(cudaMalloc(&M.rowptr, sizeof(int64_t) * (size_t)(nrows + 1 + CSR_PAD)));
    CGO_CUDA(cudaMalloc(&M.col, sizeof(int32_t) * (size_t)(nnz + CSR_PAD)));
    CGO_CUDA(cudaMalloc(&M.val, sizeof(double) * (size_t)(nnz + CSR_PAD)));
    return 0;
}

__global__ void k_slice_permute(CsrMat M, const int32_t *col_in, const double *val_in, int32_t *col_out, double *val_out,
                                bool inverse, unsigned long long *n_ragged = nullptr) {
    const int lane = threadIdx.x & 31;
    const uint32_t lt = (1u << lane) - 1u;
    const int64_t nslices = (M.nrows + 31) / 32;
    const int64_t wstride = (int64_t)gridDim.x * (blockDim.x / 32);
    for (int64_t s = (int64_t)blockIdx.x * (blockDim.x / 32) + (threadIdx.x >> 5); s < nslices; s += wstride) {
        const int64_t row = s * 32 + lane;
        int64_t rs = 0, len = 0;
        if (row < M.nrows) { rs = M.rowptr[row]; len = M.rowptr[row + 1] - rs; }
        const int64_t sb = M.rowptr[s * 32];
        if (n_ragged != nullptr) {
            const int64_t len0 = __shfl_sync(0xffffffffu, len, 0);
            const bool same = __all_sync(0xffffffffu, row >= M.nrows || len == len0);
            if (!same && lane == 0) atomicAdd(n_ragged, 1ULL);
        }
        int64_t off = 0;
        for (int64_t k = 0;; ++k) {
            const uint32_t m = __ballot_sync(0xffffffffu, len > k);
            if (m == 0) break;
            if (len > k) {
                const int64_t lvl = sb + off + __popc(m & lt), rm = rs + k;
                const int64_t src = inverse ? lvl : rm, dst = inverse ? rm : lvl;
                col_out[dst] = col_in[src];
                val_out[dst] = val_in[src];
            }
            off += __popc(m);
        }
    }
}
__global__ void k_gather_lines(CsrMat M, unsigned long long *stats) {
    const int lane = threadIdx.x & 31;
    const uint32_t lt = (1u << lane) - 1u;
    const int64_t nslices = (M.nrows + 31) / 32;
    const int64_t wstride = (int64_t)gridDim.x * (blockDim.x / 32);
    for (int64_t s = ((int64_t)blockIdx.x * (blockDim.x / 32) + (threadIdx.x >> 5)) * 64; s < nslices; s += wstride * 64) {
        const int64_t row = s * 32 + lane;
        int64_t rs = 0, len = 0;
        if (row < M.nrows) { rs = M.rowptr[row]; len = M.rowptr[row + 1] - rs; }
        unsigned int nlev = 0, nlines = 0;
        for (int64_t k = 0;; ++k) {
            const uint32_t m = __ballot_sync(0xffffffffu, len > k);
            if (m == 0) break;
            if (len > k) {
                const uint32_t same = __match_any_sync(m, M.col[rs + k] >> 4);
                if ((same & lt) == 0) ++nlines;
            }
            ++nlev;
        }
        nlines = __reduce_add_sync(0xffffffffu, nlines);
        if (lane == 0) { atomicAdd(stats, (unsigned long long)nlev); atomicAdd(stats + 1, (unsigned long long)nlines); }
    }
}
static int csr_gather_lines(cgo_ctx *c, const CsrMat &M, float *lines) {
    unsigned long long *d_stats = c->d_progress + 2, h_stats[2] = {0, 0};
    *lines = 1.0f;
    if (M.nnz == 0) return 0;
    CGO_CUDA(cudaMemsetAsync(d_stats, 0, sizeof(h_stats), c->stream));
    k_gather_lines<<<grid_for((M.nrows + 31) / 32 * 32, c->sms), 256, 0, c->stream>>>(M, d_stats);
    CGO_CUDA(cudaGetLastError());
    CGO_CUDA(cudaMemcpyAsync(h_stats, d_stats, sizeof(h_stats), cudaMemcpyDeviceToHost, c->stream));
    CGO_CUDA(cudaStreamSynchronize(c->stream));
    if (h_stats[0]) *lines = (float)((double)h_stats[1] / (double)h_stats[0]);
    return 0;
}
static int csr_make_sliced(cgo_ctx *c, CsrMat &M) {
    if (M.sliced || M.nnz == 0 || !M.col || !M.val) return 0;
    int32_t *col2 = nullptr; double *val2 = nullptr;
    unsigned long long n_ragged = 0;
    auto body = [&]() -> int {
        CGO_CUDA(cudaMalloc(&col2, sizeof(int32_t) * (size_t)(M.nnz + CSR_PAD)));
        CGO_CUDA(cudaMalloc(&val2, sizeof(double) * (size_t)(M.nnz + CSR_PAD)));
        CGO_CUDA(cudaMemsetAsync(col2 + M.nnz, 0, sizeof(int32_t) * CSR_PAD, c->stream));
        CGO_CUDA(cudaMemsetAsync(val2 + M.nnz, 0, sizeof(double) * CSR_PAD, c->stream));
        unsigned long long *d_ragged = c->d_progress + 1;
        CGO_CUDA(cudaMemsetAsync(d_ragged, 0, sizeof(unsigned long long), c->stream));
        k_slice_permute<<<grid_for((M.nrows + 31) / 32 * 32, c->sms), 256, 0, c->stream>>>(M, M.col, M.val, col2, val2, false,
                                                                                          d_ragged);
        CGO_CUDA(cudaGetLastError());
        CGO_CUDA(cudaMemcpyAsync(&n_ragged, d_ragged, sizeof(n_ragged), cudaMemcpyDeviceToHost, c->stream));
        CGO_CUDA(cudaStreamSynchronize(c->stream));
        return 0;
    };
    int rc = body();
    if (rc) { cudaFree(col2); cudaFree(val2); return rc; }
    cudaFree(M.col); cudaFree(M.val);
    M.col = col2; M.val = val2;
    M.sliced = 1;
    M.ragged = 16 * n_ragged > (unsigned long long)((M.nrows + 31) / 32);
    return 0;
}

template <class Src, class Fin>
static int build_transpose(cgo_ctx *c, const Src &src, const Fin &fin, int64_t nT, CsrMat &AT) {
    cudaStream_t s = c->stream;
    unsigned long long *counts = nullptr, *cursor = nullptr;
    int64_t *perm = nullptr;
    void *tmp = nullptr;
    int rc = 0;
    auto body = [&]() -> int {
        CGO_CUDA(cudaMalloc(&counts, sizeof(unsigned long long) * (size_t)(nT + 1)));
        CGO_CUDA(cudaMemsetAsync(counts, 0, sizeof(unsigned long long) * (size_t)(nT + 1), s));
        if (src.total > 0) k_tr_count<<<grid_for(src.total, c->sms), 256, 0, s>>>(src, counts);
        CGO_CUDA(cudaGetLastError());
        AT.nrows = nT;
        CGO_CUDA(cudaMalloc(&AT.rowptr, sizeof(int64_t) * (size_t)(nT + 1 + CSR_PAD)));
        size_t tmp_bytes = 0;
        CGO_CUDA(cub::DeviceScan::ExclusiveSum(nullptr, tmp_bytes, (const int64_t *)counts, AT.rowptr, nT + 1, s));
        CGO_CUDA(cudaMalloc(&tmp, tmp_bytes > 0 ? tmp_bytes : 1));
        CGO_CUDA(cub::DeviceScan::ExclusiveSum(tmp, tmp_bytes, (const int64_t *)counts, AT.rowptr, nT + 1, s));
        int64_t nnzT = 0;
        CGO_CUDA(cudaMemcpyAsync(&nnzT, AT.rowptr + nT, sizeof(int64_t), cudaMemcpyDeviceToHost, s));
        CGO_CUDA(cudaStreamSynchronize(s));
        AT.nnz = nnzT;
        cudaFree(counts); counts = nullptr;
        cudaFree(tmp); tmp = nullptr;
        CGO_CUDA(cudaMalloc(&cursor, sizeof(unsigned long long) * (size_t)(nT + 1)));
        CGO_CUDA(cudaMemcpyAsync(cursor, AT.rowptr, sizeof(int64_t) * (size_t)(nT + 1), cudaMemcpyDeviceToDevice, s));
        CGO_CUDA(cudaMalloc(&perm, sizeof(int64_t) * (size_t)(nnzT > 0 ? nnzT : 1)));
        if (src.total > 0) k_tr_fill<<<grid_for(src.total, c->sms), 256, 0, s>>>(src, cursor, perm);
        CGO_CUDA(cudaGetLastError());
        if (nT > 0) k_tr_sort<<<grid_for(nT, c->sms), 256, 0, s>>>(AT.rowptr, nT, perm);
        CGO_CUDA(cudaGetLastError());
        CGO_CUDA(cudaMalloc(&AT.col, sizeof(int32_t) * (size_t)(nnzT + CSR_PAD)));
        CGO_CUDA(cudaMalloc(&AT.val, sizeof(double) * (size_t)(nnzT + CSR_PAD)));
        if (nnzT > 0) k_tr_finalize<<<grid_for(nnzT, c->sms), 256, 0, s>>>(fin, nnzT, perm, AT);
        CGO_CUDA(cudaGetLastError());
        CGO_CUDA(cudaStreamSynchronize(s));
        return 0;
    };
    rc = body();
    cudaFree(counts); cudaFree(cursor); cudaFree(perm); cudaFree(tmp);
    return rc;
}

struct CsrBlocked {
    std::vector<CsrMat> blk;
    void free_all() { for (auto &m : blk) csr_free(m); blk.clear(); }
};
__global__ void k_blk_check_sorted(CsrMat A, int *bad) {
    GRID_STRIDE(i, A.nrows) {
        for (int64_t p = A.rowptr[i] + 1; p < A.rowptr[i + 1]; ++p)
            if (A.col[p] < A.col[p - 1]) { *bad = 1; break; }
    }
}
__global__ void k_blk_count(CsrMat A, int32_t c0, int32_t c1, int64_t *first, int64_t *cnt) {
    GRID_STRIDE(i, A.nrows + 1) {
        if (i == A.nrows) { cnt[i] = 0; continue; }
        const int64_t rs = A.rowptr[i], re = A.rowptr[i + 1];
        int64_t lo = rs, hi = re;
        while (lo < hi) { const int64_t mid = (lo + hi) >> 1; if (A.col[mid] < c0) lo = mid + 1; else hi = mid; }
        const int64_t b0 = lo;
        hi = re;
        while (lo < hi) { const int64_t mid = (lo + hi) >> 1; if (A.col[mid] < c1) lo = mid + 1; else hi = mid; }
        first[i] = b0;
        cnt[i] = lo - b0;
    }
}
__global__ void k_blk_copy(CsrMat A, const int64_t *first, CsrMat B) {
    GRID_STRIDE(i, A.nrows) {
        const int64_t d0 = B.rowptr[i], n = B.rowptr[i + 1] - d0, s0 = first[i];
        for (int64_t e = 0; e < n; ++e) { B.col[d0 + e] = A.col[s0 + e]; B.val[d0 + e] = A.val[s0 + e]; }
    }
}
static int build_blocked(cgo_ctx *c, const CsrMat &A, int64_t ncols, CsrBlocked &out) {
    out.free_all();
    const int64_t cap = (int64_t)(c->gather_block_bytes / sizeof(double));
    if (cap <= 0 || ncols <= cap || A.nnz == 0) return 0;
    const int64_t nb = (ncols + cap - 1) / cap;
    const int64_t bc = (((ncols + nb - 1) / nb) + 1) & ~(int64_t)1;
    cudaStream_t s = c->stream;
    int *bad = nullptr;
    int64_t *first = nullptr, *cnt = nullptr;
    void *tmp = nullptr;
    auto body = [&]() -> int {
        CGO_CUDA(cudaMalloc(&bad, sizeof(int)));
        CGO_CUDA(cudaMemsetAsync(bad, 0, sizeof(int), s));
        k_blk_check_sorted<<<grid_for(A.nrows, c->sms), 256, 0, s>>>(A, bad);
        int hbad = 0;
        CGO_CUDA(cudaMemcpyAsync(&hbad, bad, sizeof(int), cudaMemcpyDeviceToHost, s));
        CGO_CUDA(cudaStreamSynchronize(s));
        if (hbad) return 0;
        CGO_CUDA(cudaMalloc(&first, sizeof(int64_t) * (size_t)(A.nrows + 1)));
        CGO_CUDA(cudaMalloc(&cnt, sizeof(int64_t) * (size_t)(A.nrows + 1)));
        size_t tmp_bytes = 0;
        CGO_CUDA(cub::DeviceScan::ExclusiveSum(nullptr, tmp_bytes, cnt, cnt, A.nrows + 1, s));
        CGO_CUDA(cudaMalloc(&tmp, tmp_bytes > 0 ? tmp_bytes : 1));
        out.blk.resize((size_t)nb);
        for (int64_t j = 0; j < nb; ++j) {
            CsrMat &B = out.blk[(size_t)j];
            const int64_t c0 = j * bc, c1 = (j + 1) * bc < ncols ? (j + 1) * bc : ncols;
            k_blk_count<<<grid_for(A.nrows + 1, c->sms), 256, 0, s>>>(A, (int32_t)c0, (int32_t)c1, first, cnt);
            CGO_CUDA(cudaGetLastError());
            B.nrows = A.nrows;
            CGO_CUDA(cudaMalloc(&B.rowptr, sizeof(int64_t) * (size_t)(A.nrows + 1 + CSR_PAD)));
            CGO_CUDA(cub::DeviceScan::ExclusiveSum(tmp, tmp_bytes, cnt, B.rowptr, A.nrows + 1, s));
            int64_t nnzb = 0;
            CGO_CUDA(cudaMemcpyAsync(&nnzb, B.rowptr + A.nrows, sizeof(int64_t), cudaMemcpyDeviceToHost, s));
            CGO_CUDA(cudaStreamSynchronize(s));
            B.nnz = nnzb;
            CGO_CUDA(cudaMalloc(&B.col, sizeof(int32_t) * (size_t)(nnzb + CSR_PAD)));
            CGO_CUDA(cudaMalloc(&B.val, sizeof(double) * (size_t)(nnzb + CSR_PAD)));
            k_blk_copy<<<grid_for(A.nrows, c->sms), 256, 0, s>>>(A, first, B);
            CGO_CUDA(cudaGetLastError());
        }
        CGO_CUDA(cudaStreamSynchronize(s));
        return 0;
    };
    int rc = body();
    cudaFree(bad); cudaFree(first); cudaFree(cnt); cudaFree(tmp);
    if (rc) out.free_all();
    return rc;
}
template <class Epi>
static int launch_csr_blocked(cgo_ctx *c, const CsrMat &A, const CsrBlocked &B, const double *xg, const Epi &epi,
                              double *partial, const RedArgs &red, int tclass, bool wait_first = false) {
    if (B.blk.empty()) return launch_csr(c, A, xg, epi, red, tclass);
    const size_t nb = B.blk.size();
    RedArgs scratch = cgo_red_args(c, CGO_PACK_LEN - 1);
    if (c->csr_pass_occ == 3) scratch.G = c->sms * 3;
    if (wait_first) {
        scratch.wait0 = red.wait0; scratch.wait1 = red.wait1; scratch.wait_all = red.wait_all;
        scratch.wait_val = red.wait_val; scratch.nranks = red.nranks;
    }
    for (size_t j = 0; j + 1 < nb; ++j) {
        EpiStore es{partial};
        if (j == 0) CGO_TRY(launch_csr_pass(c, B.blk[j], xg, es, scratch, tclass));
        else CGO_TRY(launch_csr_pass(c, B.blk[j], xg, with_init(es, partial), scratch, tclass));
    }
    return launch_csr_pass(c, B.blk[nb - 1], xg, with_init(epi, partial), red, tclass);
}

static int spmv_direct_passes(cgo_ctx *c, const CsrMat &M, const CsrBlocked &B, const double *xg, double *out,
                              const RedArgs *wait, int tclass) {
    if (B.blk.empty()) return launch_direct(c, M, xg, DirStore{out}, dir_args(c, wait), tclass);
    for (size_t j = 0; j < B.blk.size(); ++j) {
        if (j == 0) CGO_TRY(launch_direct(c, B.blk[j], xg, DirStore{out}, dir_args(c, wait), tclass));
        else CGO_TRY(launch_direct(c, B.blk[j], xg, DirStoreInit{out, out}, dir_args(c), tclass));
    }
    return 0;
}

struct CsrObj : cgo_obj {
    bool logreg = false;
    CsrMat A, AT;
    CsrBlocked Ab, ATb;
    bool have_unblocked = true;
    int64_t nrows = 0;
    double *b = nullptr;
    double *r_base = nullptr, *r = nullptr;
    double *qv = nullptr;
    const cgo_state *r_state = nullptr;
    bool r_at_xp = false, r_at_x = false;
    int quad_steps = 0;
    std::vector<void *> rpeers;
    bool r_is_peer = false;
    double lambda = 0.0;
    int64_t nsamples = 0;
    bool lr_sharded = false;
    bool lr_direct = false;
    std::vector<int64_t> flo, slo;
    double *xp_full = nullptr;
    double *c_full = nullptr;
    bool lr_peer = false;
    std::vector<void *> xpf_peers, cf_peers;
    void **d_xpf_dst = nullptr;
    void **d_cf_dst = nullptr;
    ~CsrObj() override {
        if (ctx && cgo_ctx_alive(ctx)) cudaSetDevice(ctx->device);
        csr_free(A); csr_free(AT);
        Ab.free_all(); ATb.free_all();
        if (r_is_peer) { cgo_peer_free(ctx, r_base, rpeers, true); r_base = nullptr; }
        if (lr_peer) {
            cgo_peer_free(ctx, xp_full, xpf_peers, true); xp_full = nullptr;
            cgo_peer_free(ctx, c_full, cf_peers, true); c_full = nullptr;
        }
        cudaFree(d_xpf_dst); cudaFree(d_cf_dst);
        cudaFree(b); cudaFree(r_base); cudaFree(qv);
        cudaFree(xp_full); cudaFree(c_full);
    }
    int alloc_r() {
        size_t bytes = sizeof(double) * (size_t)(nrows + 2 * halo + 4);
        if (ctx->nranks > 1 && ctx->peer_ok && halo > 0) {
            bytes = sizeof(double) * (size_t)((n_alloc > nrows ? n_alloc : nrows) + 2 * halo + 4);
            void *p = nullptr;
            r_is_peer = true;
            CGO_TRY(cgo_peer_alloc(ctx, bytes, &p, rpeers));
            r_base = (double *)p;
        } else {
            CGO_CUDA(cudaMalloc(&r_base, bytes));
            CGO_CUDA(cudaMemsetAsync(r_base, 0, bytes, ctx->stream));
        }
        r = r_base + halo;
        return 0;
    }
    int64_t shard_len_of(int q) const {
        int64_t lo, hi;
        cgo_shard_range(n_global, ctx->nranks, q, 2, &lo, &hi);
        return hi - lo;
    }
    int eval_trial_ls_peer(cgo_state *st, double a, bool fused, double beta, double *out) {
        const int R = ctx->nranks, me = ctx->rank, prev = (me + R - 1) % R, next = (me + 1) % R;
        const unsigned long long e = ++ctx->epoch;
        unsigned long long *fprev = (unsigned long long *)ctx->flags_peer[(size_t)prev];
        unsigned long long *fnext = (unsigned long long *)ctx->flags_peer[(size_t)next];
        const int64_t nprev = shard_len_of(prev);
        HaloPush hp;
        double *xp_prev = (double *)st->xpeers[st->xp_alloc][(size_t)prev] + halo;
        double *xp_next = (double *)st->xpeers[st->xp_alloc][(size_t)next] + halo;
        hp.prev_right = xp_prev + nprev;
        hp.next_left = xp_next - halo;
        hp.sig_prev = fprev + CGO_F_XP_FROM_NEXT;
        hp.sig_next = fnext + CGO_F_XP_FROM_PREV;
        hp.epoch = e;
        CGO_TRY(cgo_blas1_axpy_dir(st, a, fused, beta, &hp));
        EpiResidualT<true> e1;
        e1.b = b; e1.r = r; e1.halo = halo; e1.nrows = nrows;
        e1.prev_right = (double *)rpeers[(size_t)prev] + halo + nprev;
        e1.next_left = (double *)rpeers[(size_t)next];
        RedArgs rb = cgo_red_args(ctx, CGO_P_PHI);
        rb.wait0 = ctx->flags_local + CGO_F_XP_FROM_PREV; rb.wait1 = ctx->flags_local + CGO_F_XP_FROM_NEXT; rb.wait_val = e;
        rb.sig0 = fprev + CGO_F_R_FROM_NEXT; rb.sig1 = fnext + CGO_F_R_FROM_PREV; rb.sig_val = e;
        CGO_TRY(launch_csr(ctx, A, st->xp, e1, rb, CGO_T_SPMV));
        EpiGrad<false> e2{st->gp, st->g, st->u, nullptr, 0.0, 0.0};
        RedArgs rc = cgo_red_args(ctx, CGO_P_DPHI);
        rc.wait0 = ctx->flags_local + CGO_F_R_FROM_PREV; rc.wait1 = ctx->flags_local + CGO_F_R_FROM_NEXT; rc.wait_val = e;
        CGO_TRY(launch_csr(ctx, AT, r, e2, rc, CGO_T_SPMVT));
        CGO_TRY(cgo_finish_pack(ctx, 12, out));
        out[CGO_P_PHI] = 0.5 * out[CGO_P_PHI];
        return 0;
    }
    int exchange(double *v, int64_t nloc) {
        if (halo == 0) return 0;
        return cgo_sendrecv_ring(ctx, v, v + nloc, v + nloc - halo, v - halo, halo);
    }
    bool direct() const { return A.sliced != 0; }
    void reduction_site(int32_t *V, int32_t *U) const override {
        if (direct() || lr_direct) { *V = 2; *U = CGO_U_VEC; } else { *V = 1; *U = 1; }
    }
    int eval_trial_lr_direct(cgo_state *st, double a, bool fused, double beta, double *out) {
        const int R = ctx->nranks;
        const double invN = 1.0 / (double)nsamples;
        RedArgs wx, wc;
        const RedArgs *pwx = nullptr, *pwc = nullptr;
        unsigned long long e = 0;
        if (R > 1 && lr_peer) {
            e = ++ctx->epoch;
            HaloPush hp;
            hp.dst_all = d_xpf_dst; hp.epoch = e;
            CGO_TRY(cgo_blas1_axpy_dir(st, a, fused, beta, &hp));
            wx.wait_all = ctx->flags_local + CGO_F_XPALL; wx.wait_val = e; wx.nranks = R; pwx = &wx;
            wc.wait_all = ctx->flags_local + CGO_F_GPART; wc.wait_val = e; wc.nranks = R; pwc = &wc;
        } else {
            CGO_TRY(cgo_blas1_axpy_dir(st, a, fused, beta));
            if (R > 1) CGO_TRY(cgo_allgatherv_f64(ctx, st->xp, xp_full, flo.data()));
        }
        const double *w_all = R > 1 ? xp_full : st->xp;
        CGO_TRY(spmv_direct_passes(ctx, A, Ab, w_all, r, pwx, CGO_T_SPMV));
        CGO_TRY(cgo_blas1_logit(ctx, r, b, nrows, CGO_P_PHI, (R > 1 && lr_peer) ? d_cf_dst : nullptr, e));
        if (R > 1 && !lr_peer) CGO_TRY(cgo_allgatherv_f64(ctx, r, c_full, slo.data()));
        const double *c_all = R > 1 ? c_full : r;
        CGO_TRY(spmv_direct_passes(ctx, AT, ATb, c_all, st->gp, pwc, CGO_T_SPMVT));
        CGO_TRY(cgo_blas1_grad_combine(st, st->gp, 1, 0, invN, lambda));
        CGO_TRY(cgo_finish_pack(ctx, 12, out));
        out[CGO_P_PHI] = out[CGO_P_PHI] / (double)nsamples + (0.5 * lambda) * out[CGO_P_XPXP];
        return 0;
    }
    int eval_trial_ls_direct(cgo_state *st, double a, bool fused, double beta, double *out) {
        const bool peer = r_is_peer && st->peer_x;
        RedArgs fb, fc;
        if (peer) {
            const int R = ctx->nranks, me = ctx->rank, prev = (me + R - 1) % R, next = (me + 1) % R;
            const unsigned long long e = ++ctx->epoch;
            unsigned long long *fprev = (unsigned long long *)ctx->flags_peer[(size_t)prev];
            unsigned long long *fnext = (unsigned long long *)ctx->flags_peer[(size_t)next];
            const int64_t nprev = shard_len_of(prev);
            HaloPush hp;
            hp.prev_right = (double *)st->xpeers[st->xp_alloc][(size_t)prev] + halo + nprev;
            hp.next_left = (double *)st->xpeers[st->xp_alloc][(size_t)next];
            hp.sig_prev = fprev + CGO_F_XP_FROM_NEXT;
            hp.sig_next = fnext + CGO_F_XP_FROM_PREV;
            hp.epoch = e;
            CGO_TRY(cgo_blas1_axpy_dir(st, a, fused, beta, &hp));
            DirResidual<true> f1{b, r, (double *)rpeers[(size_t)prev] + halo + nprev, (double *)rpeers[(size_t)next], halo, nrows};
            fb.wait0 = ctx->flags_local + CGO_F_XP_FROM_PREV; fb.wait1 = ctx->flags_local + CGO_F_XP_FROM_NEXT; fb.wait_val = e;
            fb.sig0 = fprev + CGO_F_R_FROM_NEXT; fb.sig1 = fnext + CGO_F_R_FROM_PREV; fb.sig_val = e;
            CGO_TRY(launch_direct(ctx, A, st->xp, f1, dir_args(ctx, &fb), CGO_T_SPMV));
            fc.wait0 = ctx->flags_local + CGO_F_R_FROM_PREV; fc.wait1 = ctx->flags_local + CGO_F_R_FROM_NEXT; fc.wait_val = e;
        } else {
            CGO_TRY(cgo_blas1_axpy_dir(st, a, fused, beta));
            CGO_TRY(exchange(st->xp, st->n));
            DirResidual<false> f1{b, r, nullptr, nullptr, 0, nrows};
            CGO_TRY(launch_direct(ctx, A, st->xp, f1, dir_args(ctx), CGO_T_SPMV));
        }
        CGO_TRY(cgo_blas1_sumsq(ctx, r, nrows, CGO_P_PHI));
        if (!peer) CGO_TRY(exchange(r, nrows));
        DirGradLS f2{st->gp};
        CGO_TRY(launch_direct(ctx, AT, r, f2, peer ? dir_args(ctx, &fc) : dir_args(ctx), CGO_T_SPMVT));
        CGO_TRY(cgo_blas1_grad_dots(st));
        CGO_TRY(cgo_finish_pack(ctx, 12, out));
        out[CGO_P_PHI] = 0.5 * out[CGO_P_PHI];
        return 0;
    }
    int hessvec_dir(cgo_state *st, double *out) override {
        CGO_CHECK(!logreg, "the Hessian-vector product is implemented for least squares");
        r_state = nullptr; r_at_x = r_at_xp = false;
        CGO_TRY(cgo_sendrecv_ring(ctx, st->u, st->u + st->n, st->u + st->n - halo, st->u - halo, halo));
        if (direct()) {
            CGO_TRY(launch_direct(ctx, A, st->u, DirStore{r}, dir_args(ctx), CGO_T_SPMV));
            CGO_TRY(cgo_blas1_sumsq(ctx, r, nrows, 0));
            CGO_TRY(exchange(r, nrows));
            CGO_TRY(launch_direct(ctx, AT, r, DirStore{st->hv}, dir_args(ctx), CGO_T_SPMVT));
            CGO_TRY(cgo_blas1_dots3(ctx, st->u, st->hv, st->n, 1));
            return cgo_finish_pack(ctx, 3, out);
        }
        EpiStoreSq e1{r};
        CGO_TRY(launch_csr(ctx, A, st->u, e1, cgo_red_args(ctx, 0), CGO_T_SPMV));
        CGO_TRY(exchange(r, nrows));
        EpiHv e2{st->hv, st->u};
        CGO_TRY(launch_csr(ctx, AT, r, e2, cgo_red_args(ctx, 1), CGO_T_SPMVT));
        return cgo_finish_pack(ctx, 3, out);
    }
    int quad_begin(cgo_state *st, double *out) override {
        CGO_CHECK(!logreg, "the quadratic-aware line search is for least squares");
        if (!qv) {
            CGO_CUDA(cudaMalloc(&qv, sizeof(double) * (size_t)(nrows + CSR_PAD)));
            CGO_CUDA(cudaMemsetAsync(qv, 0, sizeof(double) * (size_t)(nrows + CSR_PAD), ctx->stream));
        }
        if (!(r_state == st && r_at_x) || quad_steps >= 64) {
            CGO_TRY(cgo_sendrecv_ring(ctx, st->x, st->x + st->n, st->x + st->n - halo, st->x - halo, halo));
            if (direct()) {
                DirResidual<false> f1{b, r, nullptr, nullptr, 0, nrows};
                CGO_TRY(launch_direct(ctx, A, st->x, f1, dir_args(ctx), CGO_T_SPMV));
            } else {
                EpiResidualT<false> e0;
                e0.b = b; e0.r = r; e0.prev_right = e0.next_left = nullptr; e0.halo = 0; e0.nrows = nrows;
                CGO_TRY(launch_csr(ctx, A, st->x, e0, cgo_red_args(ctx, CGO_PACK_LEN - 1), CGO_T_SPMV));
            }
            r_state = st; r_at_x = true; r_at_xp = false; quad_steps = 0;
        }
        CGO_TRY(cgo_sendrecv_ring(ctx, st->u, st->u + st->n, st->u + st->n - halo, st->u - halo, halo));
        if (direct()) {
            CGO_TRY(launch_direct(ctx, A, st->u, DirStore{qv}, dir_args(ctx), CGO_T_SPMV));
            CGO_TRY(cgo_blas1_dots3(ctx, r, qv, nrows, 0));
            return cgo_finish_pack(ctx, 3, out);
        }
        EpiQuadV e1{qv, r};
        CGO_TRY(launch_csr(ctx, A, st->u, e1, cgo_red_args(ctx, 0), CGO_T_SPMV));
        return cgo_finish_pack(ctx, 3, out);
    }
    int quad_accept(cgo_state *st, double a, double *out) override {
        CGO_CHECK(!logreg && qv != nullptr, "cgo_quad_accept before cgo_quad_begin");
        CGO_CHECK(r_state == st && r_at_x, "cgo_quad_accept: the residual of this state was overwritten since cgo_quad_begin");
        r_at_x = false; r_at_xp = true; ++quad_steps;
        CGO_TRY(cgo_blas1_axpy_dir(st, a, false, 0.0));
        CGO_TRY(cgo_blas1_residual_axpy(ctx, r, qv, a, nrows, CGO_P_PHI));
        CGO_TRY(exchange(r, nrows));
        if (direct()) {
            CGO_TRY(launch_direct(ctx, AT, r, DirGradLS{st->gp}, dir_args(ctx), CGO_T_SPMVT));
            CGO_TRY(cgo_blas1_grad_dots(st));
            CGO_TRY(cgo_finish_pack(ctx, 12, out));
            out[CGO_P_PHI] = 0.5 * out[CGO_P_PHI];
            return 0;
        }
        EpiGrad<false> e2{st->gp, st->g, st->u, nullptr, 0.0, 0.0};
        CGO_TRY(launch_csr(ctx, AT, r, e2, cgo_red_args(ctx, CGO_P_DPHI), CGO_T_SPMVT));
        CGO_TRY(cgo_finish_pack(ctx, 12, out));
        out[CGO_P_PHI] = 0.5 * out[CGO_P_PHI];
        return 0;
    }
    void on_accept(cgo_state *st) override {
        r_at_x = (r_state == st) && r_at_xp;
        r_at_xp = false;
        if (r_state != st) r_state = nullptr;
    }
    int eval_trial(cgo_state *st, double a, bool fused, double beta, double *out) override {
        r_state = st; r_at_xp = true; r_at_x = false; quad_steps = 0;
        if (!logreg && direct()) return eval_trial_ls_direct(st, a, fused, beta, out);
        if (!logreg && r_is_peer && st->peer_x) return eval_trial_ls_peer(st, a, fused, beta, out);
        if (logreg && lr_direct) return eval_trial_lr_direct(st, a, fused, beta, out);
        CGO_TRY(cgo_blas1_axpy_dir(st, a, fused, beta));
        CGO_TRY(exchange(st->xp, st->n));
        if (logreg) {
            EpiLogit e1{b, r};
            CGO_TRY(launch_csr_blocked(ctx, A, Ab, st->xp, e1, r, cgo_red_args(ctx, CGO_P_PHI), CGO_T_SPMV));
            EpiGrad<true> e2{st->gp, st->g, st->u, st->xp, 1.0 / (double)nsamples, lambda};
            CGO_TRY(launch_csr_blocked(ctx, AT, ATb, r, e2, st->gp, cgo_red_args(ctx, CGO_P_DPHI), CGO_T_SPMVT));
            CGO_TRY(cgo_finish_pack(ctx, 12, out));
            out[CGO_P_PHI] = out[CGO_P_PHI] / (double)nsamples + (0.5 * lambda) * out[CGO_P_XPXP];
        } else {
            EpiResidualT<false> e1;
            e1.b = b; e1.r = r; e1.prev_right = e1.next_left = nullptr; e1.halo = 0; e1.nrows = nrows;
            CGO_TRY(launch_csr(ctx, A, st->xp, e1, cgo_red_args(ctx, CGO_P_PHI), CGO_T_SPMV));
            CGO_TRY(exchange(r, nrows));
            EpiGrad<false> e2{st->gp, st->g, st->u, nullptr, 0.0, 0.0};
            CGO_TRY(launch_csr(ctx, AT, r, e2, cgo_red_args(ctx, CGO_P_DPHI), CGO_T_SPMVT));
            CGO_TRY(cgo_finish_pack(ctx, 12, out));
            out[CGO_P_PHI] = 0.5 * out[CGO_P_PHI];
        }
        return 0;
    }
    double bytes_per_eval() const override {
        if (lr_direct)
            return 12.0 * (double)(A.nnz + AT.nnz) + 8.0 * (double)(A.nrows + 1 + AT.nrows + 1) +
                   8.0 * (5.0 * (double)nrows + (ctx->nranks > 1 ? (double)n_global + (double)nsamples : 0.0) + 11.0 * (double)n_local);
        return 12.0 * (double)(A.nnz + AT.nnz) + 8.0 * (double)(A.nrows + 1 + AT.nrows + 1) +
               8.0 * (3.0 * (double)nrows + 6.0 * (double)n_local) + (direct() ? 8.0 * ((double)nrows + (double)n_local) : 0.0);
    }
    int default_x0(uint64_t, double, double *x0) override {
        for (int64_t i = 0; i < n_local; ++i) x0[i] = 0.0;
        return 0;
    }
};

static int check_i32(int64_t v, const char *what) {
    CGO_CHECK(v < 2147483647LL, "%s = %lld does not fit the int32 column index", what, (long long)v);
    return 0;
}

extern "C" int cgo_obj_sparse_ls_create_synthetic(cgo_ctx *ctx, int64_t n, int32_t K, int64_t W,
                                                  uint64_t seed, int32_t coh_log2, cgo_obj **out) {
    CGO_CHECK(ctx && out, "NULL argument");
    const int64_t S = K - 1;
    CGO_CHECK(K >= 1 && n >= 2 && n % 2 == 0, "sparse_ls: need nnz_per_row >= 1 and an even n >= 2");
    CGO_CHECK(S == 0 || (W >= S && n > 2 * W), "sparse_ls: need W >= nnz_per_row-1 and n > 2W (n=%lld, W=%lld)", (long long)n, (long long)W);
    CGO_CHECK(coh_log2 >= 0 && coh_log2 < 31, "sparse_ls: coh_log2 out of range");
    CGO_CUDA(cudaSetDevice(ctx->device));
    int64_t lo, hi, n_alloc = 0;
    CGO_TRY(cgo_shard_range(n, ctx->nranks, ctx->rank, 2, &lo, &hi));
    for (int q = 0; q < ctx->nranks; ++q) {
        int64_t a, b;
        CGO_TRY(cgo_shard_range(n, ctx->nranks, q, 2, &a, &b));
        if (b - a > n_alloc) n_alloc = b - a;
    }
    const bool multi = ctx->nranks > 1;
    if (multi) {
        CGO_CHECK(hi - lo >= W && hi - lo + 2 * W <= n, "sparse_ls: shard of %lld rows needs W <= rows and rows + 2W <= n (W=%lld, n=%lld)",
                  (long long)(hi - lo), (long long)W, (long long)n);
        CGO_CHECK(W % 2 == 0, "sparse_ls: W must be even with more than one rank");
    }
    CsrObj *o = new CsrObj();
    o->ctx = ctx; o->n_global = n;
    o->offset = lo; o->n_local = hi - lo; o->nrows = hi - lo; o->n_alloc = n_alloc;
    o->halo = multi ? W : 0;
    LsSpec sp;
    sp.n = n; sp.K = K; sp.coh = coh_log2; sp.W = W; sp.w = S > 0 ? (2 * W) / S : 0; sp.seed = seed;
    const int64_t nloc = o->n_local, nnz = nloc * K;
    double *xt_base = nullptr;
    auto body = [&]() -> int {
        CGO_TRY(check_i32(nloc + 2 * o->halo, "local dimension + halo"));
        CGO_TRY(csr_alloc(o->A, nloc, nnz));
        k_ls_fill_A<<<grid_for(nnz, ctx->sms), 256, 0, ctx->stream>>>(sp, lo, nloc, multi, o->A);
        CGO_CUDA(cudaGetLastError());
        CGO_CUDA(cudaMalloc(&xt_base, sizeof(double) * (size_t)(nloc + 2 * o->halo)));
        k_ls_xtrue<<<grid_for(nloc + 2 * o->halo, ctx->sms), 256, 0, ctx->stream>>>(sp, lo, nloc, o->halo, xt_base + o->halo);
        CGO_CUDA(cudaGetLastError());
        CGO_CUDA(cudaMalloc(&o->b, sizeof(double) * (size_t)(nloc + CSR_PAD)));
        EpiStore es{o->b};
        CGO_TRY(launch_csr(ctx, o->A, xt_base + o->halo, es, cgo_red_args(ctx, CGO_PACK_LEN - 1), CGO_T_OTHER));
        CGO_CUDA(cudaStreamSynchronize(ctx->stream));
        cudaFree(xt_base); xt_base = nullptr;
        CGO_TRY(o->alloc_r());
        if (multi) {
            LsExtSrc src{sp, lo, hi, (nloc + 2 * W) * K};
            LsExtFin fin{sp, lo};
            CGO_TRY(build_transpose(ctx, src, fin, nloc, o->AT));
        } else {
            CsrSrc src{o->A.col, nnz};
            FixedKFin fin{K, o->A.val};
            CGO_TRY(build_transpose(ctx, src, fin, nloc, o->AT));
        }
        if (ctx->csr_mode == 2 || (ctx->csr_mode == 0 && coh_log2 < 4 && K > 1)) {
            CGO_TRY(csr_make_sliced(ctx, o->A));
            CGO_TRY(csr_make_sliced(ctx, o->AT));
        }
        return 0;
    };
    int rc = body();
    cudaFree(xt_base);
    if (rc) { delete o; return rc; }
    *out = o;
    return 0;
}

extern "C" int cgo_obj_sparse_ls_create_csr(cgo_ctx *ctx, int64_t nrows, int64_t ncols, const int64_t *rowptr,
                                            const int32_t *col, const double *val, const double *b,
                                            cgo_obj **out) {
    CGO_CHECK(ctx && rowptr && b && out, "NULL argument");
    CGO_CHECK(ctx->nranks == 1, "cgo_obj_sparse_ls_create_csr is single-GPU");
    CGO_CHECK(nrows >= 1 && ncols >= 1, "empty matrix");
    const int64_t nnz = rowptr[nrows];
    CGO_CHECK(nnz == 0 || (col && val), "NULL col/val");
    for (int64_t i = 0; i < nrows; ++i) CGO_CHECK(rowptr[i] <= rowptr[i + 1], "rowptr not monotone at row %lld", (long long)i);
    for (int64_t p = 0; p < nnz; ++p) CGO_CHECK(col[p] >= 0 && col[p] < ncols, "column index out of range at entry %lld", (long long)p);
    CGO_CUDA(cudaSetDevice(ctx->device));
    CsrObj *o = new CsrObj();
    o->ctx = ctx; o->n_global = ncols; o->n_local = ncols; o->offset = 0; o->nrows = nrows; o->halo = 0;
    auto body = [&]() -> int {
        CGO_TRY(check_i32(nrows > ncols ? nrows : ncols, "matrix dimension"));
        CGO_TRY(csr_alloc(o->A, nrows, nnz));
        cudaStream_t s = ctx->stream;
        CGO_CUDA(cudaMemcpyAsync(o->A.rowptr, rowptr, sizeof(int64_t) * (size_t)(nrows + 1), cudaMemcpyHostToDevice, s));
        if (nnz) {
            CGO_CUDA(cudaMemcpyAsync(o->A.col, col, sizeof(int32_t) * (size_t)nnz, cudaMemcpyHostToDevice, s));
            CGO_CUDA(cudaMemcpyAsync(o->A.val, val, sizeof(double) * (size_t)nnz, cudaMemcpyHostToDevice, s));
        }
        CGO_CUDA(cudaMalloc(&o->b, sizeof(double) * (size_t)(nrows + CSR_PAD)));
        CGO_CUDA(cudaMemcpyAsync(o->b, b, sizeof(double) * (size_t)nrows, cudaMemcpyHostToDevice, s));
        CGO_TRY(o->alloc_r());
        CsrSrc src{o->A.col, nnz};
        CsrFin fin{o->A.rowptr, nrows, o->A.val};
        CGO_TRY(build_transpose(ctx, src, fin, ncols, o->AT));
        float la = 1.f, lt = 1.f;
        CGO_TRY(csr_gather_lines(ctx, o->A, &la));
        CGO_TRY(csr_gather_lines(ctx, o->AT, &lt));
        o->A.lines_per_gather = la; o->AT.lines_per_gather = lt;
        if (ctx->csr_mode == 2 || (ctx->csr_mode == 0 && la > 4.0f && lt > 4.0f && nrows >= 4096)) {
            CGO_TRY(csr_make_sliced(ctx, o->A));
            CGO_TRY(csr_make_sliced(ctx, o->AT));
        }
        return 0;
    };
    int rc = body();
    if (rc) { delete o; return rc; }
    *out = o;
    return 0;
}

struct LrFeatSrc {
    LrSpec s;
    int64_t flo, fhi, total;
    int32_t k0, nk;
    __device__ __forceinline__ bool get(int64_t e, int64_t &trow, int64_t &key) const {
        const int64_t i = e / nk;
        const int k = k0 + (int)(e - i * nk);
        int64_t c; double v;
        s.entry(i, k, c, v);
        if (c < flo || c >= fhi) return false;
        trow = c - flo; key = i * s.K + k;
        return true;
    }
};
struct LrFeatFin {
    LrSpec s;
    __device__ __forceinline__ void get(int64_t key, int32_t &srow, double &v) const {
        const int64_t i = key / s.K;
        int64_t c;
        s.entry(i, (int)(key - i * s.K), c, v);
        srow = (int32_t)i;
    }
};

extern "C" int cgo_obj_logreg_create_synthetic(cgo_ctx *ctx, int64_t N, int64_t d, int32_t K, uint64_t seed,
                                               double lambda, cgo_obj **out) {
    CGO_CHECK(ctx && out, "NULL argument");
    CGO_CHECK(K >= 1 && N >= 1 && d >= K, "logreg: need nnz_per_row >= 1, nsamples >= 1, nfeat >= nnz_per_row");
    const int R = ctx->nranks, me = ctx->rank;
    CGO_CHECK(R == 1 || (N >= 2 * R && d >= 2 * R), "logreg: %d ranks need nsamples >= %d and nfeat >= %d", R, 2 * R, 2 * R);
    CGO_CHECK(R == 1 || ctx->csr_mode != 1, "logreg: the sharded objective runs on k_spmv_direct (CGO_CSR_MODE=1 forbids it)");
    CGO_CUDA(cudaSetDevice(ctx->device));
    CsrObj *o = new CsrObj();
    o->ctx = ctx; o->logreg = true; o->lambda = lambda; o->nsamples = N;
    o->n_global = d; o->halo = 0;
    LrSpec sp;
    sp.N = N; sp.d = d; sp.K = K; sp.w = d / K; sp.seed = seed;
    auto body = [&]() -> int {
        o->flo.assign(R + 1, 0); o->slo.assign(R + 1, 0);
        for (int r = 0; r < R; ++r) {
            int64_t lo, hi;
            CGO_TRY(cgo_shard_range(d, R, r, 2, &lo, &hi));
            o->flo[r] = lo; o->flo[r + 1] = hi;
            CGO_TRY(cgo_shard_range(N, R, r, 2, &lo, &hi));
            o->slo[r] = lo; o->slo[r + 1] = hi;
        }
        const int64_t slo = o->slo[me], nloc = o->slo[me + 1] - o->slo[me];
        o->offset = o->flo[me]; o->n_local = o->flo[me + 1] - o->flo[me];
        o->nrows = nloc;
        o->lr_sharded = R > 1;
        CGO_TRY(check_i32(N > d ? N : d, "matrix dimension"));
        CGO_TRY(csr_alloc(o->A, nloc, nloc * K));
        CGO_CUDA(cudaMalloc(&o->b, sizeof(double) * (size_t)(nloc + CSR_PAD)));
        CGO_CUDA(cudaMemsetAsync(o->b, 0, sizeof(double) * (size_t)(nloc + CSR_PAD), ctx->stream));
        k_lr_fill_A<<<grid_for(nloc, ctx->sms), 256, 0, ctx->stream>>>(sp, slo, nloc, o->A, o->b);
        CGO_CUDA(cudaGetLastError());
        CGO_TRY(o->alloc_r());
        if (R == 1) {
            CsrSrc src{o->A.col, nloc * K};
            FixedKFin fin{K, o->A.val};
            CGO_TRY(build_transpose(ctx, src, fin, d, o->AT));
        } else {
            const int64_t flo = o->flo[me], fhi = o->flo[me + 1];
            int64_t k0 = flo / sp.w, k1 = (fhi - 1) / sp.w;
            if (k0 > K - 1) k0 = K - 1;
            if (k1 > K - 1) k1 = K - 1;
            LrFeatSrc src{sp, flo, fhi, N * (k1 - k0 + 1), (int32_t)k0, (int32_t)(k1 - k0 + 1)};
            LrFeatFin fin{sp};
            CGO_TRY(build_transpose(ctx, src, fin, fhi - flo, o->AT));
        }
        CGO_TRY(build_blocked(ctx, o->A, d, o->Ab));
        CGO_TRY(build_blocked(ctx, o->AT, N, o->ATb));
        const bool blocked = !o->Ab.blk.empty() || !o->ATb.blk.empty();
        if (blocked && o->A.nnz > (int64_t)200000000 / R) {
            if (!o->Ab.blk.empty()) { cudaFree(o->A.col); cudaFree(o->A.val); o->A.col = nullptr; o->A.val = nullptr; }
            if (!o->ATb.blk.empty()) { cudaFree(o->AT.col); cudaFree(o->AT.val); o->AT.col = nullptr; o->AT.val = nullptr; }
            o->have_unblocked = false;
        }
        o->lr_direct = ctx->csr_mode != 1 && (R > 1 || blocked || ctx->csr_mode == 2);
        if (o->lr_direct) {
            if (o->Ab.blk.empty()) CGO_TRY(csr_make_sliced(ctx, o->A));
            if (o->ATb.blk.empty()) CGO_TRY(csr_make_sliced(ctx, o->AT));
            for (auto &m : o->Ab.blk) CGO_TRY(csr_make_sliced(ctx, m));
            for (auto &m : o->ATb.blk) CGO_TRY(csr_make_sliced(ctx, m));
        }
        if (o->lr_sharded) {
            const size_t xb = sizeof(double) * (size_t)(d + CSR_PAD), cb = sizeof(double) * (size_t)(N + CSR_PAD);
            if (ctx->peer_ok) {
                void *p = nullptr;
                o->lr_peer = true;
                CGO_TRY(cgo_peer_alloc(ctx, xb, &p, o->xpf_peers));
                o->xp_full = (double *)p;
                CGO_TRY(cgo_peer_alloc(ctx, cb, &p, o->cf_peers));
                o->c_full = (double *)p;
                std::vector<void *> xd((size_t)R), cd((size_t)R);
                for (int r = 0; r < R; ++r) {
                    xd[(size_t)r] = (double *)o->xpf_peers[(size_t)r] + o->flo[(size_t)me];
                    cd[(size_t)r] = (double *)o->cf_peers[(size_t)r] + o->slo[(size_t)me];
                }
                CGO_CUDA(cudaMalloc(&o->d_xpf_dst, sizeof(void *) * (size_t)R));
                CGO_CUDA(cudaMalloc(&o->d_cf_dst, sizeof(void *) * (size_t)R));
                CGO_CUDA(cudaMemcpy(o->d_xpf_dst, xd.data(), sizeof(void *) * (size_t)R, cudaMemcpyHostToDevice));
                CGO_CUDA(cudaMemcpy(o->d_cf_dst, cd.data(), sizeof(void *) * (size_t)R, cudaMemcpyHostToDevice));
            } else {
                CGO_CUDA(cudaMalloc(&o->xp_full, xb));
                CGO_CUDA(cudaMalloc(&o->c_full, cb));
                CGO_CUDA(cudaMemsetAsync(o->xp_full, 0, xb, ctx->stream));
                CGO_CUDA(cudaMemsetAsync(o->c_full, 0, cb, ctx->stream));
            }
            CGO_CUDA(cudaStreamSynchronize(ctx->stream));
        }
        return 0;
    };
    int rc = body();
    if (rc) { delete o; return rc; }
    *out = o;
    return 0;
}

static CsrObj *as_csr(cgo_obj *o) { return dynamic_cast<CsrObj *>(o); }

extern "C" int cgo_obj_csr_blocks(cgo_obj *obj, int transposed, int32_t *nblocks) {
    CsrObj *o = as_csr(obj);
    CGO_CHECK(o && nblocks, "not a CSR objective / NULL argument");
    const CsrBlocked &B = transposed ? o->ATb : o->Ab;
    *nblocks = B.blk.empty() ? 1 : (int32_t)B.blk.size();
    return 0;
}
extern "C" int cgo_obj_csr_nnz(cgo_obj *obj, int transposed, int64_t *nrows, int64_t *nnz) {
    CsrObj *o = as_csr(obj);
    CGO_CHECK(o != nullptr, "not a CSR objective");
    const CsrMat &M = transposed ? o->AT : o->A;
    if (nrows) *nrows = M.nrows;
    if (nnz) *nnz = M.nnz;
    return 0;
}
extern "C" int cgo_obj_csr_download(cgo_obj *obj, int transposed, int64_t *rowptr, int32_t *col, double *val, double *b) {
    CsrObj *o = as_csr(obj);
    CGO_CHECK(o != nullptr, "not a CSR objective");
    CGO_CHECK(o->have_unblocked, "the single-pass CSR copy was dropped at this size (column-blocked storage only)");
    const CsrMat &M = transposed ? o->AT : o->A;
    cudaStream_t s = o->ctx->stream;
    CGO_CUDA(cudaSetDevice(o->ctx->device));
    if (rowptr) CGO_CUDA(cudaMemcpyAsync(rowptr, M.rowptr, sizeof(int64_t) * (size_t)(M.nrows + 1), cudaMemcpyDeviceToHost, s));
    int32_t *ctmp = nullptr; double *vtmp = nullptr;
    auto body = [&]() -> int {
        const int32_t *csrc = M.col; const double *vsrc = M.val;
        if (M.sliced && M.nnz && (col || val)) {
            CGO_CUDA(cudaMalloc(&ctmp, sizeof(int32_t) * (size_t)M.nnz));
            CGO_CUDA(cudaMalloc(&vtmp, sizeof(double) * (size_t)M.nnz));
            k_slice_permute<<<grid_for((M.nrows + 31) / 32 * 32, o->ctx->sms), 256, 0, s>>>(M, M.col, M.val, ctmp, vtmp, true);
            CGO_CUDA(cudaGetLastError());
            csrc = ctmp; vsrc = vtmp;
        }
        if (col && M.nnz) CGO_CUDA(cudaMemcpyAsync(col, csrc, sizeof(int32_t) * (size_t)M.nnz, cudaMemcpyDeviceToHost, s));
        if (val && M.nnz) CGO_CUDA(cudaMemcpyAsync(val, vsrc, sizeof(double) * (size_t)M.nnz, cudaMemcpyDeviceToHost, s));
        if (b) CGO_CUDA(cudaMemcpyAsync(b, o->b, sizeof(double) * (size_t)o->nrows, cudaMemcpyDeviceToHost, s));
        CGO_CUDA(cudaStreamSynchronize(s));
        return 0;
    };
    int rc = body();
    cudaFree(ctmp); cudaFree(vtmp);
    return rc;
}
extern "C" int cgo_obj_spmv(cgo_obj *obj, int transposed, const double *x_host, double *y_host) {
    CsrObj *o = as_csr(obj);
    CGO_CHECK(o && x_host && y_host, "not a CSR objective / NULL argument");
    CGO_CHECK(o->halo == 0 && !o->lr_sharded, "cgo_obj_spmv is a single-GPU test hook");
    CGO_CHECK(o->have_unblocked, "the single-pass CSR copy was dropped at this size (column-blocked storage only)");
    cgo_ctx *c = o->ctx;
    CGO_CUDA(cudaSetDevice(c->device));
    const CsrMat &M = transposed ? o->AT : o->A;
    const int64_t nin = transposed ? o->A.nrows : o->AT.nrows, nout = M.nrows;
    double *dx = nullptr, *dy = nullptr;
    auto body = [&]() -> int {
        CGO_CUDA(cudaMalloc(&dx, sizeof(double) * (size_t)nin));
        CGO_CUDA(cudaMalloc(&dy, sizeof(double) * (size_t)nout));
        CGO_CUDA(cudaMemcpyAsync(dx, x_host, sizeof(double) * (size_t)nin, cudaMemcpyHostToDevice, c->stream));
        if (M.sliced) {
            CGO_TRY(launch_direct(c, M, dx, DirStore{dy}, dir_args(c), transposed ? CGO_T_SPMVT : CGO_T_SPMV));
        } else {
            EpiStore es{dy};
            CGO_TRY(launch_csr(c, M, dx, es, cgo_red_args(c, CGO_PACK_LEN - 1), transposed ? CGO_T_SPMVT : CGO_T_SPMV));
        }
        CGO_CUDA(cudaMemcpyAsync(y_host, dy, sizeof(double) * (size_t)nout, cudaMemcpyDeviceToHost, c->stream));
        CGO_CUDA(cudaStreamSynchronize(c->stream));
        return 0;
    };
    int rc = body();
    cudaFree(dx); cudaFree(dy);
    return rc;
}
```

conjugategradientoptim.jl_b200/csrc/internal.cuh:

```cuda
#pragma once
#include <cuda_runtime.h>
#include <stdint.h>
#include <stdio.h>
#include <map>
#include <string>
#include <vector>

#include "../../include/cgoptim.h"

void cgo_set_error(const char *fmt, ...);
#define CGO_CUDA(call)                                                                          \
    do {                                                                                        \
        cudaError_t e__ = (call);                                                               \
        if (e__ != cudaSuccess) {                                                               \
            cgo_set_error("%s failed: %s (%s:%d)", #call, cudaGetErrorString(e__), __FILE__,    \
                          __LINE__);                                                            \
            return 1;                                                                           \
        }                                                                                       \
    } while (0)
#define CGO_CHECK(cond, ...)                                                                    \
    do {                                                                                        \
        if (!(cond)) {                                                                          \
            cgo_set_error(__VA_ARGS__);                                                         \
            return 2;                                                                           \
        }                                                                                       \
    } while (0)
#define CGO_TRY(call)                                                                           \
    do {                                                                                        \
        int r__ = (call);                                                                       \
        if (r__) return r__;                                                                    \
    } while (0)

constexpr int CGO_B = 256;
constexpr int CGO_NW = CGO_B / 32;
constexpr int CGO_U_VEC = 4;
constexpr int CGO_MAXK = 12;

struct RedArgs {
    double *partial;
    unsigned int *ticket;
    double *out;
    int G;
    unsigned long long *sig0 = nullptr, *sig1 = nullptr;
    const unsigned long long *wait0 = nullptr, *wait1 = nullptr;
    unsigned long long sig_val = 0, wait_val = 0;
    void *const *flags_all = nullptr;
    const unsigned long long *wait_all = nullptr;
    int sig_all_slot = -1, nranks = 1, me = 0;
};

struct NcclApi;
enum { CGO_T_TRIAL = 0, CGO_T_DIR = 1, CGO_T_AXPY = 2, CGO_T_SPMV = 3, CGO_T_SPMVT = 4,
       CGO_T_LBFGS = 5, CGO_T_OTHER = 6, CGO_T_BATCHED = 7, CGO_T_N = 8 };
struct CgoPendingTimer { int cls; cudaEvent_t e0, e1; };
struct cgo_ctx {
    int device = 0;
    int sms = 0;
    cudaStream_t stream = nullptr;
    bool own_stream = false;
    int G = 296;
    size_t gather_block_bytes = (size_t)40 << 20;
    int csr_pass_occ = 2;
    int64_t launches = 0;
    int csr_mode = 0;
    int direct_cfg = 0;
    unsigned long long *d_progress = nullptr;
    double *d_partial = nullptr;
    unsigned int *d_ticket = nullptr;
    double *h_pack = nullptr;
    double *d_pack_map = nullptr;
    double *d_pack = nullptr;
    double *d_gather = nullptr;
    double *d_scal = nullptr;
    bool timing = false;
    std::vector<CgoPendingTimer> pending;
    std::vector<cudaEvent_t> ev_pool;
    double t_ms[CGO_T_N] = {0};
    int64_t t_cnt[CGO_T_N] = {0};
    int nranks = 1, rank = 0;
    void *comm = nullptr;
    NcclApi *nccl = nullptr;
    bool peer_ok = false;
    unsigned long long *flags_local = nullptr;
    std::vector<void *> flags_peer;
    unsigned long long epoch = 0;
    double *gather_local = nullptr;
    std::vector<void *> gather_peer;
    void **d_gather_peer = nullptr, **d_flags_peer = nullptr;
    unsigned long long pack_epoch = 0;
    std::map<size_t, std::vector<std::vector<void *>>> peer_pool;
    std::map<void *, size_t> peer_bytes;
    size_t peer_pool_bytes = 0;
    std::map<size_t, std::vector<void *>> dev_pool;
    size_t dev_pool_bytes = 0;
};
bool cgo_ctx_alive(cgo_ctx *ctx);
int cgo_dev_alloc(cgo_ctx *ctx, size_t bytes, void **out);
void cgo_dev_free(cgo_ctx *ctx, void *ptr, size_t bytes);
constexpr int CGO_MAX_RANKS = 64;
enum { CGO_F_XP_FROM_PREV = 0, CGO_F_XP_FROM_NEXT = 1, CGO_F_R_FROM_PREV = 2, CGO_F_R_FROM_NEXT = 3, CGO_F_PACK = 8,
       CGO_F_XPALL = 8 + CGO_MAX_RANKS, CGO_F_GPART = 8 + 2 * CGO_MAX_RANKS, CGO_F_N = 8 + 3 * CGO_MAX_RANKS };
int cgo_peer_alloc(cgo_ctx *ctx, size_t bytes, void **local, std::vector<void *> &peers);
int cgo_peer_free(cgo_ctx *ctx, void *local, std::vector<void *> &peers, bool collective);
constexpr int CGO_GMAX = 8192;
constexpr int CGO_NSCAL = 256;
constexpr int CGO_LBFGS_MAX_M = 64;

RedArgs cgo_red_args(cgo_ctx *ctx, int slot = 0);
void cgo_timer_begin(cgo_ctx *ctx, int cls);
void cgo_timer_end(cgo_ctx *ctx);
void cgo_timer_collect(cgo_ctx *ctx);
int cgo_finish_pack(cgo_ctx *ctx, int K, double *out_host);
int cgo_combine_ranks(cgo_ctx *ctx, int K, double *out_dev);
int cgo_allgather_bytes(cgo_ctx *ctx, const void *send_dev, void *recv_dev, size_t bytes_per_rank);
int cgo_sendrecv_ring(cgo_ctx *ctx, const double *send_to_prev, double *recv_from_next,
                      const double *send_to_next, double *recv_from_prev, int64_t count);
int cgo_allgatherv_f64(cgo_ctx *ctx, const double *mine, double *full, const int64_t *lo);
int cgo_alltoallv_f64(cgo_ctx *ctx, const double *full, const int64_t *lo, double *recv, int64_t stride);

struct cgo_state;
struct cgo_obj {
    cgo_ctx *ctx = nullptr;
    int64_t n_global = 0, n_local = 0, offset = 0;
    int64_t halo = 0;
    int64_t n_alloc = 0;
    virtual ~cgo_obj() {}
    virtual int eval_trial(cgo_state *st, double a, bool fused_dir, double beta,
                           double *out_host) = 0;
    virtual int hessvec_dir(cgo_state *st, double *out_host);
    virtual int quad_begin(cgo_state *st, double *out_host);
    virtual int quad_accept(cgo_state *st, double a, double *out_host);
    virtual void on_accept(cgo_state *) {}
    virtual double bytes_per_eval() const = 0;
    virtual void reduction_site(int32_t *V, int32_t *U) const = 0;
    virtual int default_x0(uint64_t seed, double perturb, double *x0_host) = 0;
};

struct cgo_state {
    cgo_ctx *ctx = nullptr;
    cgo_obj *obj = nullptr;
    int64_t n = 0;
    int64_t halo = 0;
    double *base[5] = {nullptr, nullptr, nullptr, nullptr, nullptr};
    double *x = nullptr, *g = nullptr, *u = nullptr, *xp = nullptr, *gp = nullptr;
    bool peer_x = false;
    std::vector<void *> xpeers[2];
    int xp_alloc = 1;
    double *hv = nullptr;
    double *xn = nullptr;
    int m = 0, count = 0, head = 0, staged = -1;
    std::vector<double *> S, Y;
    std::vector<double> rho;
    double gamma = 1.0;
    double *q = nullptr;
};

struct HaloPush {
    double *prev_right = nullptr;
    double *next_left = nullptr;
    unsigned long long *sig_prev = nullptr, *sig_next = nullptr;
    unsigned long long epoch = 0;
    void *const *dst_all = nullptr;
};
int cgo_blas1_axpy_dir(cgo_state *st, double a, bool fused_dir, double beta, const HaloPush *push = nullptr);
int cgo_blas1_residual_axpy(cgo_ctx *ctx, double *r, const double *v, double a, int64_t nrows, int slot);
int cgo_blas1_sumsq(cgo_ctx *ctx, const double *a, int64_t n, int slot);
int cgo_blas1_dots3(cgo_ctx *ctx, const double *a, const double *b, int64_t n, int slot);
int cgo_blas1_logit(cgo_ctx *ctx, double *zc, const double *y, int64_t n, int slot, void *const *dst_all, unsigned long long epoch);
int cgo_blas1_grad_dots(cgo_state *st);
int cgo_blas1_grad_combine(cgo_state *st, const double *q, int nparts, int64_t stride, double invN, double lambda,
                           unsigned long long wait_epoch = 0);

struct CsrMat {
    int64_t nrows = 0, nnz = 0;
    int64_t *rowptr = nullptr;
    int32_t *col = nullptr;
    double *val = nullptr;
    int32_t sliced = 0;
    int32_t ragged = 0;
    int64_t max_tile_nnz = 0;
    float lines_per_gather = 1.f;
};
```

conjugategradientoptim.jl_b200/csrc/reduce.cuh:

```cuda
#pragma once
#include "internal.cuh"

struct BarAll { __device__ __forceinline__ void operator()() const { __syncthreads(); } };
struct BarLanes {
    __device__ __forceinline__ void operator()() const { asm volatile("bar.sync 1, %0;" ::"n"(CGO_B) : "memory"); }
};

__device__ __forceinline__ void cgo_st_release_sys(unsigned long long *p, unsigned long long v) {
    asm volatile("st.release.sys.global.u64 [%0], %1;" ::"l"(p), "l"(v) : "memory");
}
__device__ __forceinline__ unsigned long long cgo_ld_acquire_sys(const unsigned long long *p) {
    unsigned long long v;
    asm volatile("ld.acquire.sys.global.u64 %0, [%1];" : "=l"(v) : "l"(p) : "memory");
    return v;
}

template <int K, class Bar = BarAll>
__device__ __forceinline__ void cgo_cta_combine(double (&acc)[K], double *sm , Bar bar = Bar()) {
    const int lane = threadIdx.x & 31, warp = threadIdx.x >> 5;
#pragma unroll
    for (int k = 0; k < K; ++k) {
        double v = acc[k];
#pragma unroll
        for (int off = 16; off >= 1; off >>= 1) v = v + __shfl_xor_sync(0xffffffffu, v, off);
        if (lane == 0) sm[k * CGO_NW + warp] = v;
    }
    bar();
    if (threadIdx.x == 0) {
#pragma unroll
        for (int k = 0; k < K; ++k) {
            double s = sm[k * CGO_NW];
#pragma unroll
            for (int w = 1; w < CGO_NW; ++w) s = s + sm[k * CGO_NW + w];
            acc[k] = s;
        }
    }
    bar();
}

template <int K>
__device__ __forceinline__ void cgo_publish(const RedArgs &red, int vcta, const double (&acc)[K]) {
    if (threadIdx.x == 0) {
#pragma unroll
        for (int k = 0; k < K; ++k) __stcg(&red.partial[(size_t)k * red.G + vcta], acc[k]);
    }
}

template <int K, class Bar = BarAll>
__device__ __forceinline__ void cgo_grid_finish(const RedArgs &red, int nact, double *sm, Bar bar = Bar()) {
    __shared__ bool is_last;
    if (red.sig0 != nullptr || red.flags_all != nullptr) __threadfence_system();
    else __threadfence();
    bar();
    if (threadIdx.x == 0) {
        unsigned int t = atomicAdd(red.ticket, 1u);
        is_last = (t == gridDim.x - 1);
    }
    bar();
    if (!is_last) return;
    __threadfence();
    double acc[K];
#pragma unroll
    for (int k = 0; k < K; ++k) {
        double s = 0.0;
        for (int c = threadIdx.x; c < nact; c += CGO_B) s = s + __ldcg(&red.partial[(size_t)k * red.G + c]);
        acc[k] = s;
    }
    cgo_cta_combine<K, Bar>(acc, sm, bar);
    if (threadIdx.x == 0) {
#pragma unroll
        for (int k = 0; k < K; ++k) red.out[k] = acc[k];
        *red.ticket = 0u;
        __threadfence_system();
        if (red.sig0 != nullptr) {
            cgo_st_release_sys(red.sig0, red.sig_val);
            if (red.sig1 != nullptr) cgo_st_release_sys(red.sig1, red.sig_val);
        }
        if (red.flags_all != nullptr)
            for (int r = 0; r < red.nranks; ++r)
                cgo_st_release_sys((unsigned long long *)red.flags_all[r] + red.sig_all_slot + red.me, red.sig_val);
    }
}

__device__ __forceinline__ void cgo_spin_until(const unsigned long long *flag, unsigned long long val) {
    unsigned int polls = 0;
    while (cgo_ld_acquire_sys(flag) < val) {
        __nanosleep(128);
        if (++polls > (1u << 28)) asm volatile("trap;");
    }
}
template <class Bar>
__device__ __forceinline__ void cgo_wait_flags(const RedArgs &red, Bar bar) {
    if (red.wait0 == nullptr && red.wait_all == nullptr) return;
    if (threadIdx.x == 0 && red.wait0 != nullptr) {
        cgo_spin_until(red.wait0, red.wait_val);
        if (red.wait1 != nullptr) cgo_spin_until(red.wait1, red.wait_val);
    }
    if (red.wait_all != nullptr && (int)threadIdx.x < red.nranks) cgo_spin_until(red.wait_all + threadIdx.x, red.wait_val);
    bar();
}

__device__ __forceinline__ double2 cgo_ld2(const double2 *p) {
    double2 r;
    asm volatile("ld.global.nc.L1::no_allocate.v2.f64 {%0, %1}, [%2];" : "=d"(r.x), "=d"(r.y) : "l"(p));
    return r;
}
__device__ __forceinline__ void cgo_st2(double2 *p, double2 v) {
    asm volatile("st.global.L1::no_allocate.v2.f64 [%0], {%1, %2};" ::"l"(p), "d"(v.x), "d"(v.y) : "memory");
}
```

Before: 50.18.

## Fuse trial-point axpy and residual sumsq into the SpMV kernel with dataflow chaining

Adds a fused persistent kernel that computes the trial point xp = x + a*u (and optional direction update) as a work item inside the CSR SpMV, gated by a precomputed per-tile column reach so SpMV tiles start once the xp entries they need are ready. The residual sum of squares is also folded in via per-warp carried partial sums, with release/acquire flags chaining the tiles. The goal is to remove separate blas1 launches and the extra read/write passes over xp and r during the line-search trial evaluation. In exchange it adds spin-waiting, coherent (.cg) gathers instead of non-coherent loads, a host-side reach precompute, and ordering complexity that could serialize work or stall.

```diff
diff --git a/conjugategradientoptim.jl_b200/csrc/blas1.cu b/conjugategradientoptim.jl_b200/csrc/blas1.cu
--- a/conjugategradientoptim.jl_b200/csrc/blas1.cu
+++ b/conjugategradientoptim.jl_b200/csrc/blas1.cu
@@ -1,5 +1,6 @@
 #include "internal.cuh"
 #include "reduce.cuh"
+#include "blas1_ops.cuh"
 
 template <class Op>
 __global__ void __launch_bounds__(CGO_B, Op::OCC) k_blas1(Op op, int64_t n, RedArgs red) {
@@ -52,12 +53,6 @@
     return 0;
 }
 
-__device__ __forceinline__ double2 ld2rw(const double2 *p) {
-    double2 r;
-    asm volatile("ld.global.L1::no_allocate.v2.f64 {%0, %1}, [%2];" : "=d"(r.x), "=d"(r.y) : "l"(p) : "memory");
-    return r;
-}
-
 template <bool FUSED>
 struct RosenTrial {
     static constexpr int TCLASS = CGO_T_TRIAL;
@@ -181,56 +176,6 @@
         const double t1 = in.u.x + in.g.x;
         acc[0] = acc[0] + t1 * t1;
         if (v2) { const double t2 = in.u.y + in.g.y; acc[0] = acc[0] + t2 * t2; }
-    }
-};
-
-template <bool FUSED, int PUSH>
-struct AxpyDir {
-    static constexpr int TCLASS = CGO_T_AXPY;
-    static constexpr int K = 3;
-    static constexpr int OCC = 2;
-    struct In { double2 x, u, g; };
-    const double2 *x, *g;
-    double2 *u, *xp;
-    double a, beta;
-    double2 *prev_right, *next_left;
-    int64_t hq, nq;
-    void *const *dst_all;
-    int nranks;
-    __device__ __forceinline__ void prologue() {}
-    __device__ __forceinline__ In load(int64_t q) const {
-        In r;
-        r.x = cgo_ld2(x + q);
-        r.g = cgo_ld2(g + q);
-        r.u = FUSED ? ld2rw(u + q) : cgo_ld2(u + q);
-        return r;
-    }
-    __device__ __forceinline__ void apply(int64_t q, const In &in, double (&acc)[K], bool v2) const {
-        double2 uu = in.u;
-        if (FUSED) {
-            uu.x = -in.g.x + beta * in.u.x;
-            uu.y = v2 ? -in.g.y + beta * in.u.y : 0.0;
-            cgo_st2(u + q, uu);
-        }
-        double2 p;
-        p.x = in.x.x + a * uu.x;
-        p.y = v2 ? in.x.y + a * uu.y : 0.0;
-        cgo_st2(xp + q, p);
-        if (PUSH == 1) {
-            if (q < hq) cgo_st2(prev_right + q, p);
-            if (q >= nq - hq) cgo_st2(next_left + (q - (nq - hq)), p);
-        }
-        if (PUSH == 2) {
-            for (int r = 0; r < nranks; ++r) cgo_st2((double2 *)dst_all[r] + q, p);
-        }
-        acc[0] = acc[0] + in.g.x * uu.x;
-        acc[1] = acc[1] + uu.x * uu.x;
-        acc[2] = acc[2] + p.x * p.x;
-        if (v2) {
-            acc[0] = acc[0] + in.g.y * uu.y;
-            acc[1] = acc[1] + uu.y * uu.y;
-            acc[2] = acc[2] + p.y * p.y;
-        }
     }
 };
 
@@ -284,19 +229,6 @@
     }
 };
 
-struct VecSumSq {
-    static constexpr int TCLASS = CGO_T_OTHER;
-    static constexpr int K = 1;
-    static constexpr int OCC = 4;
-    struct In { double2 a; };
-    const double2 *a;
-    __device__ __forceinline__ void prologue() {}
-    __device__ __forceinline__ In load(int64_t q) const { return In{cgo_ld2(a + q)}; }
-    __device__ __forceinline__ void apply(int64_t, const In &in, double (&acc)[K], bool v2) const {
-        acc[0] = acc[0] + in.a.x * in.a.x;
-        if (v2) acc[0] = acc[0] + in.a.y * in.a.y;
-    }
-};
 struct Dots3 {
     static constexpr int TCLASS = CGO_T_OTHER;
     static constexpr int K = 3;
@@ -308,30 +240,6 @@
     __device__ __forceinline__ void apply(int64_t, const In &in, double (&acc)[K], bool v2) const {
         acc[0] = acc[0] + in.a.x * in.b.x; acc[1] = acc[1] + in.b.x * in.b.x; acc[2] = acc[2] + in.a.x * in.a.x;
         if (v2) { acc[0] = acc[0] + in.a.y * in.b.y; acc[1] = acc[1] + in.b.y * in.b.y; acc[2] = acc[2] + in.a.y * in.a.y; }
-    }
-};
-struct GradDots {
-    static constexpr int TCLASS = CGO_T_OTHER;
-    static constexpr int K = 8;
-    static constexpr int OCC = 2;
-    struct In { double2 gp, g, u; };
-    const double2 *gp, *g, *u;
-    __device__ __forceinline__ void prologue() {}
-    __device__ __forceinline__ In load(int64_t q) const { return In{cgo_ld2(gp + q), cgo_ld2(g + q), cgo_ld2(u + q)}; }
-    __device__ __forceinline__ void one(double gn, double gg, double uu, double (&acc)[K]) const {
-        const double y = gn - gg;
-        acc[CGO_P_DPHI - 1] = acc[CGO_P_DPHI - 1] + gn * uu;
-        acc[CGO_P_GPGP - 1] = acc[CGO_P_GPGP - 1] + gn * gn;
-        acc[CGO_P_YY - 1] = acc[CGO_P_YY - 1] + y * y;
-        acc[CGO_P_UY - 1] = acc[CGO_P_UY - 1] + uu * y;
-        acc[CGO_P_YGP - 1] = acc[CGO_P_YGP - 1] + y * gn;
-        acc[CGO_P_GPG - 1] = acc[CGO_P_GPG - 1] + gn * gg;
-        acc[CGO_P_UG - 1] = acc[CGO_P_UG - 1] + uu * gg;
-        acc[CGO_P_UU - 1] = acc[CGO_P_UU - 1] + uu * uu;
-    }
-    __device__ __forceinline__ void apply(int64_t, const In &in, double (&acc)[K], bool v2) const {
-        one(in.gp.x, in.g.x, in.u.x, acc);
-        if (v2) one(in.gp.y, in.g.y, in.u.y, acc);
     }
 };
 
@@ -1080,7 +988,7 @@
 }
 
 int cgo_blas1_sumsq(cgo_ctx *c, const double *a, int64_t n, int slot) {
-    VecSumSq op;
+    VecSumSq<> op;
     op.a = (const double2 *)a;
     return launch_blas1(c, op, n, cgo_red_args(c, slot));
 }
@@ -1103,7 +1011,7 @@
     return launch_blas1(c, op, n, red);
 }
 int cgo_blas1_grad_dots(cgo_state *st) {
-    GradDots op;
+    GradDots<> op;
     op.gp = (const double2 *)st->gp; op.g = (const double2 *)st->g; op.u = (const double2 *)st->u;
     return launch_blas1(st->ctx, op, st->n, cgo_red_args(st->ctx, CGO_P_DPHI));
 }
diff --git a/conjugategradientoptim.jl_b200/csrc/blas1_ops.cuh b/conjugategradientoptim.jl_b200/csrc/blas1_ops.cuh
--- /dev/null
+++ b/conjugategradientoptim.jl_b200/csrc/blas1_ops.cuh
@@ -0,0 +1,156 @@
+#pragma once
+#include "internal.cuh"
+#include "reduce.cuh"
+
+__device__ __forceinline__ double2 ld2rw(const double2 *p) {
+    double2 r;
+    asm volatile("ld.global.L1::no_allocate.v2.f64 {%0, %1}, [%2];" : "=d"(r.x), "=d"(r.y) : "l"(p) : "memory");
+    return r;
+}
+
+template <bool FUSED, int PUSH>
+struct AxpyDir {
+    static constexpr int TCLASS = CGO_T_AXPY;
+    static constexpr int K = 3;
+    static constexpr int OCC = 2;
+    struct In { double2 x, u, g; };
+    const double2 *x, *g;
+    double2 *u, *xp;
+    double a, beta;
+    double2 *prev_right, *next_left;
+    int64_t hq, nq;
+    void *const *dst_all;
+    int nranks;
+    __device__ __forceinline__ void prologue() {}
+    __device__ __forceinline__ In load(int64_t q) const {
+        In r;
+        r.x = cgo_ld2(x + q);
+        r.g = cgo_ld2(g + q);
+        r.u = FUSED ? ld2rw(u + q) : cgo_ld2(u + q);
+        return r;
+    }
+    __device__ __forceinline__ double2 point(const In &in, double2 &uu, bool v2) const {
+        uu = in.u;
+        if (FUSED) {
+            uu.x = -in.g.x + beta * in.u.x;
+            uu.y = v2 ? -in.g.y + beta * in.u.y : 0.0;
+        }
+        double2 p;
+        p.x = in.x.x + a * uu.x;
+        p.y = v2 ? in.x.y + a * uu.y : 0.0;
+        return p;
+    }
+    __device__ __forceinline__ void apply(int64_t q, const In &in, double (&acc)[K], bool v2) const {
+        double2 uu;
+        const double2 p = point(in, uu, v2);
+        if (FUSED) cgo_st2(u + q, uu);
+        cgo_st2(xp + q, p);
+        if (PUSH == 1) {
+            if (q < hq) cgo_st2(prev_right + q, p);
+            if (q >= nq - hq) cgo_st2(next_left + (q - (nq - hq)), p);
+        }
+        if (PUSH == 2) {
+            for (int r = 0; r < nranks; ++r) cgo_st2((double2 *)dst_all[r] + q, p);
+        }
+        acc[0] = acc[0] + in.g.x * uu.x;
+        acc[1] = acc[1] + uu.x * uu.x;
+        acc[2] = acc[2] + p.x * p.x;
+        if (v2) {
+            acc[0] = acc[0] + in.g.y * uu.y;
+            acc[1] = acc[1] + uu.y * uu.y;
+            acc[2] = acc[2] + p.y * p.y;
+        }
+    }
+};
+
+template <bool COH = false>
+struct VecSumSq {
+    static constexpr int TCLASS = CGO_T_OTHER;
+    static constexpr int K = 1;
+    static constexpr int OCC = 4;
+    struct In { double2 a; };
+    const double2 *a;
+    __device__ __forceinline__ void prologue() {}
+    __device__ __forceinline__ In load(int64_t q) const { return In{COH ? cgo_ld2cg(a + q) : cgo_ld2(a + q)}; }
+    __device__ __forceinline__ void apply(int64_t, const In &in, double (&acc)[K], bool v2) const {
+        acc[0] = acc[0] + in.a.x * in.a.x;
+        if (v2) acc[0] = acc[0] + in.a.y * in.a.y;
+    }
+};
+template <bool COH = false>
+struct GradDots {
+    static constexpr int TCLASS = CGO_T_OTHER;
+    static constexpr int K = 8;
+    static constexpr int OCC = 2;
+    struct In { double2 gp, g, u; };
+    const double2 *gp, *g, *u;
+    __device__ __forceinline__ void prologue() {}
+    __device__ __forceinline__ In load(int64_t q) const {
+        return In{COH ? cgo_ld2cg(gp + q) : cgo_ld2(gp + q), cgo_ld2(g + q), cgo_ld2(u + q)};
+    }
+    __device__ __forceinline__ void one(double gn, double gg, double uu, double (&acc)[K]) const {
+        const double y = gn - gg;
+        acc[CGO_P_DPHI - 1] = acc[CGO_P_DPHI - 1] + gn * uu;
+        acc[CGO_P_GPGP - 1] = acc[CGO_P_GPGP - 1] + gn * gn;
+        acc[CGO_P_YY - 1] = acc[CGO_P_YY - 1] + y * y;
+        acc[CGO_P_UY - 1] = acc[CGO_P_UY - 1] + uu * y;
+        acc[CGO_P_YGP - 1] = acc[CGO_P_YGP - 1] + y * gn;
+        acc[CGO_P_GPG - 1] = acc[CGO_P_GPG - 1] + gn * gg;
+        acc[CGO_P_UG - 1] = acc[CGO_P_UG - 1] + uu * gg;
+        acc[CGO_P_UU - 1] = acc[CGO_P_UU - 1] + uu * uu;
+    }
+    __device__ __forceinline__ void apply(int64_t, const In &in, double (&acc)[K], bool v2) const {
+        one(in.gp.x, in.g.x, in.u.x, acc);
+        if (v2) one(in.gp.y, in.g.y, in.u.y, acc);
+    }
+};
+
+constexpr int64_t CGO_TILE_Q = (int64_t)CGO_B * CGO_U_VEC;
+__device__ __forceinline__ double cgo_ld_carry(const double *p, uint64_t pol) {
+    double r;
+    asm volatile("ld.global.cg.L2::cache_hint.f64 %0, [%1], %2;" : "=d"(r) : "l"(p), "l"(pol) : "memory");
+    return r;
+}
+__device__ __forceinline__ void cgo_st_carry(double *p, double v, uint64_t pol) {
+    asm volatile("st.global.cg.L2::cache_hint.f64 [%0], %1, %2;" ::"l"(p), "d"(v), "l"(pol) : "memory");
+}
+template <class Op>
+__device__ __forceinline__ void cgo_warp_subtile(const Op &op, int64_t T, int cw, int64_t n, const RedArgs &red,
+                                                 double *carry, uint64_t pol) {
+    constexpr int K = Op::K;
+    const int lane = threadIdx.x & 31, t = cw * 32 + lane;
+    const int64_t nq = (n + 1) >> 1, ntiles = (nq + CGO_TILE_Q - 1) / CGO_TILE_Q;
+    const int v = (int)(T % red.G);
+    const bool first = T < red.G, last = T + red.G >= ntiles;
+    double *cp = carry + (size_t)v * CGO_B + t;
+    double acc[K];
+#pragma unroll
+    for (int k = 0; k < K; ++k) acc[k] = first ? 0.0 : cgo_ld_carry(cp + (size_t)k * red.G * CGO_B, pol);
+    const int64_t q0 = T * CGO_TILE_Q + t;
+#pragma unroll 1
+    for (int j = 0; j < CGO_U_VEC; ++j) {
+        const int64_t q = q0 + (int64_t)j * CGO_B;
+        if (q < nq) op.apply(q, op.load(q), acc, 2 * q + 1 < n);
+    }
+#pragma unroll
+    for (int k = 0; k < K; ++k) {
+        double s = acc[k];
+        if (last) {
+#pragma unroll
+            for (int off = 16; off >= 1; off >>= 1) s = s + __shfl_xor_sync(0xffffffffu, s, off);
+        }
+        if (!last || lane == 0) cgo_st_carry(cp + (size_t)k * red.G * CGO_B, s, pol);
+    }
+}
+template <int K>
+__device__ __forceinline__ void cgo_subtile_publish(const RedArgs &red, int v, const double *carry, uint64_t pol) {
+    const double *c0 = carry + (size_t)v * CGO_B;
+#pragma unroll 1
+    for (int k = 0; k < K; ++k) {
+        const double *ck = c0 + (size_t)k * red.G * CGO_B;
+        double s = cgo_ld_carry(ck, pol);
+#pragma unroll
+        for (int w = 1; w < CGO_NW; ++w) s = s + cgo_ld_carry(ck + w * 32, pol);
+        __stcg(&red.partial[(size_t)k * red.G + v], s);
+    }
+}
diff --git a/conjugategradientoptim.jl_b200/csrc/csr.cu b/conjugategradientoptim.jl_b200/csrc/csr.cu
--- a/conjugategradientoptim.jl_b200/csrc/csr.cu
+++ b/conjugategradientoptim.jl_b200/csrc/csr.cu
@@ -2,6 +2,7 @@
 
 #include "internal.cuh"
 #include "reduce.cuh"
+#include "blas1_ops.cuh"
 
 
 constexpr int CSR_PAD = 16;
@@ -102,6 +103,16 @@
         "setp.ne.s32 q, %3, 0;\n"
         "@q ld.global.nc.L2::cache_hint.f64 %0, [%1], %2;\n"
         "}\n" : "+d"(r) : "l"(p), "l"(pol), "r"((int)on));
+    return r;
+}
+__device__ __forceinline__ double ld_gather_cg_f64_if(const double *p, uint64_t pol, bool on) {
+    double r = 0.0;
+    asm volatile(
+        "{\n"
+        ".reg .pred q;\n"
+        "setp.ne.s32 q, %3, 0;\n"
+        "@q ld.global.cg.L2::cache_hint.f64 %0, [%1], %2;\n"
+        "}\n" : "+d"(r) : "l"(p), "l"(pol), "r"((int)on) : "memory");
     return r;
 }
 
@@ -471,7 +482,7 @@
     return r;
 }
 
-template <int UN, bool UNIFORM>
+template <int UN, bool UNIFORM, bool COH>
 __device__ __forceinline__ double dir_batch(const CsrMat &A, const double *__restrict__ xg, uint64_t gpol, int64_t sb,
                                             int64_t &off, int len, int k0, int lane, uint32_t lt, double sum) {
     int32_t cj[UN];
@@ -490,7 +501,8 @@
         vj[j] = ld_stream_f64_if(A.val + idx, on);
     }
 #pragma unroll
-    for (int j = 0; j < UN; ++j) xj[j] = ld_gather_f64_if(xg + cj[j], gpol, len > k0 + j);
+    for (int j = 0; j < UN; ++j)
+        xj[j] = COH ? ld_gather_cg_f64_if(xg + cj[j], gpol, len > k0 + j) : ld_gather_f64_if(xg + cj[j], gpol, len > k0 + j);
 #pragma unroll
     for (int j = 0; j < UN; ++j) {
         const double p = vj[j] * xj[j];
@@ -499,9 +511,213 @@
     return sum;
 }
 
-template <class F, int UN, int OCC>
+constexpr int64_t FU_TILE = 2 * CGO_TILE_Q;
+constexpr int FU_SPT = (int)(FU_TILE / 32);
+constexpr int64_t FU_AHEAD = 512;
+constexpr int64_t FU_FAR = 1024;
+struct FuseState {
+    unsigned long long *frontier, *edone;
+    unsigned int *chain_a, *chain_d;
+    unsigned int *cnt_a;
+    unsigned int *cnt;
+    double *carry_a, *carry_d;
+};
+struct NoTileOp { static constexpr int K = 0; };
+struct DirNoItems { static constexpr bool ITEMS = false, COH = false; };
+
+__device__ __forceinline__ unsigned long long fu_ld_acquire(const unsigned long long *p) {
+    unsigned long long v;
+    asm volatile("ld.acquire.gpu.global.u64 %0, [%1];" : "=l"(v) : "l"(p) : "memory");
+    return v;
+}
+__device__ __forceinline__ unsigned long long fu_ld_acquire(const unsigned int *p) {
+    unsigned int v;
+    asm volatile("ld.acquire.gpu.global.u32 %0, [%1];" : "=r"(v) : "l"(p) : "memory");
+    return v;
+}
+__device__ __forceinline__ void fu_st_release(unsigned long long *p, unsigned long long v) {
+    asm volatile("st.release.gpu.global.u64 [%0], %1;" ::"l"(p), "l"(v) : "memory");
+}
+__device__ __forceinline__ void fu_st_release(unsigned int *p, unsigned int v) {
+    asm volatile("st.release.gpu.global.u32 [%0], %1;" ::"l"(p), "r"(v) : "memory");
+}
+template <class W>
+__device__ __forceinline__ unsigned long long fu_wait(const W *p, unsigned long long v) {
+    unsigned long long got;
+    unsigned int polls = 0;
+    while ((got = fu_ld_acquire(p)) < v) {
+        __nanosleep(64);
+        if (++polls > (1u << 28)) asm volatile("trap;");
+    }
+    return got;
+}
+__device__ __forceinline__ void fu_publish_fence() {
+    __threadfence();
+    __syncwarp();
+}
+
+template <class OpA, class OpD>
+struct DirFused {
+    static constexpr bool ITEMS = true;
+    static constexpr bool HAS_A = OpA::K > 0;
+    static constexpr bool COH = HAS_A;
+    static constexpr int PER = (HAS_A ? CGO_NW : 0) + FU_SPT + CGO_NW;
+    OpA opa;
+    OpD opd;
+    RedArgs ra, rd;
+    int64_t na, nd;
+    int64_t nta, ntd, nslices;
+    int64_t ne, e0;
+    int64_t lead, lag, steps;
+    const int32_t *reach;
+    FuseState fs;
+    __host__ __device__ int64_t nitems() const { return ne + steps * PER; }
+
+    __device__ __forceinline__ void xp_only(int64_t T) const {
+        if constexpr (HAS_A) {
+            const int lane = threadIdx.x & 31;
+            const int64_t nq = (na + 1) >> 1;
+#pragma unroll 1
+            for (int cw = 0; cw < CGO_NW; ++cw) {
+                const int64_t q0 = T * CGO_TILE_Q + cw * 32 + lane;
+#pragma unroll
+                for (int j = 0; j < CGO_U_VEC; ++j) {
+                    const int64_t q = q0 + (int64_t)j * CGO_B;
+                    if (q < nq) {
+                        double2 uu;
+                        cgo_st2(opa.xp + q, opa.point(opa.load(q), uu, 2 * q + 1 < na));
+                    }
+                }
+            }
+            fu_publish_fence();
+            if (lane == 0) atomicAdd(fs.edone, 1ULL);
+        }
+    }
+    __device__ __forceinline__ void tile_a(int64_t T, int cw, uint64_t pol) const {
+        if constexpr (HAS_A) {
+            const int lane = threadIdx.x & 31;
+            const int v = (int)(T % ra.G);
+            const unsigned int m = (unsigned int)(T / ra.G);
+            unsigned int *chain = fs.chain_a + v * CGO_NW + cw;
+            if (lane == 0) {
+                if (m > 0) fu_wait(chain, m);
+                if (T >= e0) fu_wait(fs.edone, (unsigned long long)ne);
+            }
+            __syncwarp();
+            cgo_warp_subtile(opa, T, cw, na, ra, fs.carry_a, pol);
+            fu_publish_fence();
+            int done = 0;
+            if (lane == 0) {
+                fu_st_release(chain, m + 1);
+                done = atomicAdd(fs.cnt_a + T, 1u) == CGO_NW - 1;
+                if (done) {
+                    __threadfence();
+                    if (T + ra.G >= nta) cgo_subtile_publish<OpA::K>(ra, v, fs.carry_a, pol);
+                }
+            }
+            if (__shfl_sync(0xffffffffu, done, 0)) advance();
+            __syncwarp();
+        }
+    }
+    __device__ __forceinline__ void tile_d(int64_t T, int cw, uint64_t pol) const {
+        const int lane = threadIdx.x & 31;
+        const int v = (int)(T % rd.G);
+        const unsigned int m = (unsigned int)(T / rd.G);
+        unsigned int *chain = fs.chain_d + v * CGO_NW + cw;
+        const int64_t left = nslices - T * FU_SPT;
+        const unsigned int nsl = (unsigned int)(left < FU_SPT ? left : FU_SPT);
+        if (lane == 0) {
+            fu_wait(fs.cnt + T, (unsigned long long)nsl);
+            if (m > 0) fu_wait(chain, m);
+        }
+        __syncwarp();
+        cgo_warp_subtile(opd, T, cw, nd, rd, fs.carry_d, pol);
+        fu_publish_fence();
+        if (lane == 0) {
+            fu_st_release(chain, m + 1);
+            if (atomicAdd(fs.cnt + T, 1u) == nsl + CGO_NW - 1) {
+                fs.cnt[T] = 0u;
+                __threadfence();
+                if (T + rd.G >= ntd) cgo_subtile_publish<OpD::K>(rd, v, fs.carry_d, pol);
+            }
+        }
+        __syncwarp();
+    }
+    __device__ __forceinline__ unsigned long long advance() const {
+        const int lane = threadIdx.x & 31;
+        unsigned long long f0 = 0;
+        if (lane == 0) f0 = fu_ld_acquire(fs.frontier);
+        f0 = __shfl_sync(0xffffffffu, f0, 0);
+        unsigned long long f = f0;
+        for (;;) {
+            const unsigned long long b = f + 4ULL * lane;
+            int run = 0;
+            bool ok = true;
+#pragma unroll
+            for (int k = 0; k < 4; ++k) {
+                const bool d = b + k < (unsigned long long)nta && fu_ld_acquire(fs.cnt_a + b + k) == CGO_NW;
+                ok = ok && d;
+                run += ok ? 1 : 0;
+            }
+            const unsigned int short_ = __ballot_sync(0xffffffffu, run < 4);
+            if (short_ == 0) { f += 128; continue; }
+            const int first = __ffs(short_) - 1;
+            f += 4ULL * first + (unsigned long long)__shfl_sync(0xffffffffu, run, first);
+            break;
+        }
+        if (lane == 0 && f > f0) {
+            __threadfence();
+            atomicMax(fs.frontier, f);
+        }
+        return f;
+    }
+    __device__ __forceinline__ int64_t item(int64_t i, uint64_t pol, unsigned int &seen) const {
+        if (i < ne) { xp_only(e0 + i); return -1; }
+        i -= ne;
+        const int64_t s = i / PER;
+        int slot = (int)(i - s * PER);
+        if (HAS_A) {
+            if (slot < CGO_NW) { if (s < nta) tile_a(s, slot, pol); return -1; }
+            slot -= CGO_NW;
+        }
+        if (slot < FU_SPT) {
+            const int64_t T = s - lead, sl = T * FU_SPT + slot;
+            if (T < 0 || sl >= nslices) return -1;
+            if (HAS_A) {
+                const unsigned int need = (unsigned int)(((unsigned int)__ldg(reach + T) + (unsigned int)FU_TILE - 1) / FU_TILE);
+                if (seen < need || seen == 0) {
+                    if ((threadIdx.x & 31) == 0 && ne > 0 && seen == 0) fu_wait(fs.edone, (unsigned long long)ne);
+                    __syncwarp();
+                    unsigned int polls = 0;
+                    while ((seen = (unsigned int)advance()) < need) {
+                        __nanosleep(64);
+                        if (++polls > (1u << 28)) asm volatile("trap;");
+                    }
+                }
+            }
+            return sl;
+        }
+        const int64_t T = s - lead - lag;
+        if (T >= 0 && T < ntd) tile_d(T, slot - FU_SPT, pol);
+        return -1;
+    }
+    __device__ __forceinline__ void slice_done(int64_t sl) const {
+        fu_publish_fence();
+        if ((threadIdx.x & 31) == 0) atomicAdd(fs.cnt + sl / FU_SPT, 1u);
+    }
+    __device__ __forceinline__ void finish(double *sm) const {
+        if constexpr (HAS_A) cgo_grid_sum<OpA::K>(ra, (int)(nta < ra.G ? nta : ra.G), sm);
+        cgo_grid_sum<OpD::K>(rd, (int)(ntd < rd.G ? ntd : rd.G), sm);
+        for (int c = threadIdx.x; c < rd.G * CGO_NW; c += CGO_B) { fs.chain_a[c] = 0u; fs.chain_d[c] = 0u; }
+        if constexpr (HAS_A)
+            for (int64_t t = threadIdx.x; t < nta; t += CGO_B) fs.cnt_a[t] = 0u;
+        if (threadIdx.x == 0) { *fs.frontier = 0ULL; *fs.edone = 0ULL; }
+    }
+};
+
+template <class F, class X, int UN, int OCC>
 __global__ void __launch_bounds__(CGO_B, OCC)
-k_spmv_direct(CsrMat A, const double *__restrict__ xg, F f, DirArgs da) {
+k_spmv_direct(CsrMat A, const double *__restrict__ xg, F f, const __grid_constant__ X x, DirArgs da) {
     const int tid = threadIdx.x, lane = tid & 31;
     const uint32_t lt = (1u << lane) - 1u;
     const int64_t nrows = A.nrows, nslices = (nrows + 31) / 32;
@@ -514,15 +730,22 @@
         __syncthreads();
     }
     const uint64_t gpol = l2_policy_evict_last();
+    int64_t nitems = nslices;
+    if constexpr (X::ITEMS) nitems = x.nitems();
+    unsigned int seen = 0;
     for (;;) {
         unsigned long long s0 = 0;
         if (lane == 0) s0 = atomicAdd(da.next, (unsigned long long)DIR_GRAB);
         s0 = __shfl_sync(0xffffffffu, s0, 0);
-        if ((int64_t)s0 >= nslices) break;
+        if ((int64_t)s0 >= nitems) break;
 #pragma unroll 1
         for (int g = 0; g < DIR_GRAB; ++g) {
-            const int64_t s = (int64_t)s0 + g;
-            if (s >= nslices) break;
+            int64_t s = (int64_t)s0 + g;
+            if (s >= nitems) break;
+            if constexpr (X::ITEMS) {
+                s = x.item(s, gpol, seen);
+                if (s < 0) continue;
+            }
             const int64_t row = s * 32 + lane;
             const bool valid = row < nrows;
             int64_t rp0 = 0, rp1 = 0;
@@ -533,28 +756,36 @@
             const bool uniform = __all_sync(0xffffffffu, len == maxlen);
             double sum = valid ? f.init(row) : 0.0;
             int64_t off = 0;
-            if (uniform) { for (int k0 = 0; k0 < maxlen; k0 += UN) sum = dir_batch<UN, true>(A, xg, gpol, sb, off, len, k0, lane, lt, sum); }
-            else { for (int k0 = 0; k0 < maxlen; k0 += UN) sum = dir_batch<UN, false>(A, xg, gpol, sb, off, len, k0, lane, lt, sum); }
+            if (uniform) { for (int k0 = 0; k0 < maxlen; k0 += UN) sum = dir_batch<UN, true, X::COH>(A, xg, gpol, sb, off, len, k0, lane, lt, sum); }
+            else { for (int k0 = 0; k0 < maxlen; k0 += UN) sum = dir_batch<UN, false, X::COH>(A, xg, gpol, sb, off, len, k0, lane, lt, sum); }
             if (valid) f.row(row, sum);
+            if constexpr (X::ITEMS) x.slice_done(s);
         }
     }
     __shared__ bool is_last;
+    __shared__ double s_red[X::ITEMS ? CGO_MAXK * CGO_NW : 1];
     if (da.sig0 != nullptr || da.flags_all != nullptr) __threadfence_system();
     else __threadfence();
     __syncthreads();
     if (tid == 0) is_last = atomicAdd(da.ticket, 1u) == gridDim.x - 1;
     __syncthreads();
-    if (is_last && tid == 0) {
-        *da.ticket = 0u;
-        *da.next = 0ULL;
-        __threadfence_system();
-        if (da.sig0 != nullptr) {
-            cgo_st_release_sys(da.sig0, da.sig_val);
-            if (da.sig1 != nullptr) cgo_st_release_sys(da.sig1, da.sig_val);
-        }
-        if (da.flags_all != nullptr)
-            for (int r = 0; r < da.nranks; ++r)
-                cgo_st_release_sys((unsigned long long *)da.flags_all[r] + da.sig_all_slot + da.me, da.sig_val);
+    if (is_last) {
+        if constexpr (X::ITEMS) {
+            __threadfence();
+            x.finish(s_red);
+        }
+        if (tid == 0) {
+            *da.ticket = 0u;
+            *da.next = 0ULL;
+            __threadfence_system();
+            if (da.sig0 != nullptr) {
+                cgo_st_release_sys(da.sig0, da.sig_val);
+                if (da.sig1 != nullptr) cgo_st_release_sys(da.sig1, da.sig_val);
+            }
+            if (da.flags_all != nullptr)
+                for (int r = 0; r < da.nranks; ++r)
+                    cgo_st_release_sys((unsigned long long *)da.flags_all[r] + da.sig_all_slot + da.me, da.sig_val);
+        }
     }
 }
 
@@ -605,26 +836,29 @@
     }
     return d;
 }
-template <class F, int UN, int OCC>
-static int launch_direct_k(cgo_ctx *c, const CsrMat &A, const double *xg, const F &f, const DirArgs &da, int tclass) {
-    const int64_t nslices = (A.nrows + 31) / 32;
-    int64_t want = (nslices + 8 * DIR_GRAB - 1) / (8 * DIR_GRAB), phys = (int64_t)c->sms * OCC;
+template <class F, class X, int UN, int OCC>
+static int launch_direct_k(cgo_ctx *c, const CsrMat &A, const double *xg, const F &f, const DirArgs &da, int tclass,
+                           const X &x) {
+    int64_t nitems = (A.nrows + 31) / 32;
+    if constexpr (X::ITEMS) nitems = x.nitems();
+    int64_t want = (nitems + 8 * DIR_GRAB - 1) / (8 * DIR_GRAB), phys = (int64_t)c->sms * OCC;
     int grid = (int)(want < phys ? want : phys);
     if (grid < 1) grid = 1;
     cgo_timer_begin(c, tclass);
-    k_spmv_direct<F, UN, OCC><<<grid, CGO_B, 0, c->stream>>>(A, xg, f, da);
+    k_spmv_direct<F, X, UN, OCC><<<grid, CGO_B, 0, c->stream>>>(A, xg, f, x, da);
     cgo_timer_end(c);
     c->launches++;
     CGO_CUDA(cudaGetLastError());
     return 0;
 }
-template <class F>
-static int launch_direct(cgo_ctx *c, const CsrMat &A, const double *xg, const F &f, const DirArgs &da, int tclass) {
+template <class F, class X = DirNoItems>
+static int launch_direct(cgo_ctx *c, const CsrMat &A, const double *xg, const F &f, const DirArgs &da, int tclass,
+                         const X &x = X()) {
     CGO_CHECK(A.sliced, "internal: k_spmv_direct needs the sliced layout");
     const int cfg = c->direct_cfg ? c->direct_cfg : (A.ragged ? 3 : 2);
-    if (cfg == 1) return launch_direct_k<F, 8, 4>(c, A, xg, f, da, tclass);
-    if (cfg == 3) return launch_direct_k<F, 6, 5>(c, A, xg, f, da, tclass);
-    return launch_direct_k<F, 10, 4>(c, A, xg, f, da, tclass);
+    if (cfg == 1) return launch_direct_k<F, X, 8, 4>(c, A, xg, f, da, tclass, x);
+    if (cfg == 3) return launch_direct_k<F, X, 6, 5>(c, A, xg, f, da, tclass, x);
+    return launch_direct_k<F, X, 10, 4>(c, A, xg, f, da, tclass, x);
 }
 
 __host__ __device__ __forceinline__ uint64_t g_mix64(uint64_t z) {
@@ -840,7 +1074,7 @@
 }
 
 static void csr_free(CsrMat &M) {
-    cudaFree(M.rowptr); cudaFree(M.col); cudaFree(M.val);
+    cudaFree(M.rowptr); cudaFree(M.col); cudaFree(M.val); cudaFree(M.reach);
     M = CsrMat();
 }
 static int csr_alloc(CsrMat &M, int64_t nrows, int64_t nnz) {
@@ -941,6 +1175,62 @@
     M.sliced = 1;
     M.ragged = 16 * n_ragged > (unsigned long long)((M.nrows + 31) / 32);
     return 0;
+}
+
+__global__ void k_tile_reach(CsrMat M, int32_t *near, int32_t *all, int *far) {
+    __shared__ int s_near, s_all, s_far;
+    const int64_t T = blockIdx.x;
+    if (threadIdx.x == 0) { s_near = 0; s_all = 0; s_far = 0x7fffffff; }
+    __syncthreads();
+    const int64_t r1 = (T + 1) * FU_TILE < M.nrows ? (T + 1) * FU_TILE : M.nrows;
+    const int64_t p0 = M.rowptr[T * FU_TILE], p1 = M.rowptr[r1];
+    const int64_t lim = (T + 1 + FU_FAR) * FU_TILE;
+    int mn = 0, ma = 0, mf = 0x7fffffff;
+    for (int64_t p = p0 + threadIdx.x; p < p1; p += blockDim.x) {
+        const int c = M.col[p];
+        ma = max(ma, c + 1);
+        if (c < lim) mn = max(mn, c + 1);
+        else mf = min(mf, c);
+    }
+    atomicMax(&s_near, mn); atomicMax(&s_all, ma); atomicMin(&s_far, mf);
+    __syncthreads();
+    if (threadIdx.x == 0) { near[T] = s_near; all[T] = s_all; atomicMin(far, s_far); }
+}
+static int csr_build_reach(cgo_ctx *c, CsrMat &M, int64_t ncols) {
+    const int64_t nt = (M.nrows + FU_TILE - 1) / FU_TILE, nta = (ncols + FU_TILE - 1) / FU_TILE;
+    std::vector<int32_t> near((size_t)nt), all((size_t)nt);
+    int far = 0x7fffffff;
+    int32_t *d = nullptr;
+    auto body = [&]() -> int {
+        CGO_CUDA(cudaMalloc(&d, sizeof(int32_t) * (size_t)(2 * nt + 1)));
+        CGO_CUDA(cudaMemcpyAsync(d + 2 * nt, &far, sizeof(int), cudaMemcpyHostToDevice, c->stream));
+        k_tile_reach<<<(unsigned int)nt, 256, 0, c->stream>>>(M, d, d + nt, (int *)(d + 2 * nt));
+        CGO_CUDA(cudaGetLastError());
+        CGO_CUDA(cudaMemcpyAsync(near.data(), d, sizeof(int32_t) * (size_t)nt, cudaMemcpyDeviceToHost, c->stream));
+        CGO_CUDA(cudaMemcpyAsync(all.data(), d + nt, sizeof(int32_t) * (size_t)nt, cudaMemcpyDeviceToHost, c->stream));
+        CGO_CUDA(cudaMemcpyAsync(&far, d + 2 * nt, sizeof(int), cudaMemcpyDeviceToHost, c->stream));
+        CGO_CUDA(cudaStreamSynchronize(c->stream));
+        int64_t e0 = nta;
+        if (far != 0x7fffffff && nta - far / FU_TILE <= nta / 8) e0 = far / FU_TILE;
+        const std::vector<int32_t> &src = e0 < nta ? near : all;
+        int32_t mx = 0;
+        int64_t lead = 0;
+        for (int64_t T = 0; T < nt; ++T) {
+            mx = src[(size_t)T] > mx ? src[(size_t)T] : mx;
+            near[(size_t)T] = mx;
+            const int64_t need = ((int64_t)mx + FU_TILE - 1) / FU_TILE;
+            if (need - 1 - T > lead) lead = need - 1 - T;
+        }
+        CGO_CUDA(cudaMalloc(&M.reach, sizeof(int32_t) * (size_t)nt));
+        CGO_CUDA(cudaMemcpyAsync(M.reach, near.data(), sizeof(int32_t) * (size_t)nt, cudaMemcpyHostToDevice, c->stream));
+        CGO_CUDA(cudaStreamSynchronize(c->stream));
+        M.early_col = e0 * FU_TILE;
+        M.reach_lead = lead;
+        return 0;
+    };
+    int rc = body();
+    cudaFree(d);
+    return rc;
 }
 
 template <class Src, class Fin>
@@ -1118,6 +1408,9 @@
     std::vector<void *> xpf_peers, cf_peers;
     void **d_xpf_dst = nullptr;
     void **d_cf_dst = nullptr;
+    FuseState fs{};
+    void *fs_mem = nullptr;
+    int fs_G = 0;
     ~CsrObj() override {
         if (ctx && cgo_ctx_alive(ctx)) cudaSetDevice(ctx->device);
         csr_free(A); csr_free(AT);
@@ -1130,6 +1423,7 @@
         cudaFree(d_xpf_dst); cudaFree(d_cf_dst);
         cudaFree(b); cudaFree(r_base); cudaFree(qv);
         cudaFree(xp_full); cudaFree(c_full);
+        cudaFree(fs_mem);
     }
     int alloc_r() {
         size_t bytes = sizeof(double) * (size_t)(nrows + 2 * halo + 4);
@@ -1218,8 +1512,69 @@
         out[CGO_P_PHI] = out[CGO_P_PHI] / (double)nsamples + (0.5 * lambda) * out[CGO_P_XPXP];
         return 0;
     }
+    int fuse_alloc() {
+        const int G = ctx->G;
+        if (fs_mem && G <= fs_G) return 0;
+        cudaFree(fs_mem);
+        fs_mem = nullptr;
+        const int64_t ta = (A.nrows + FU_TILE - 1) / FU_TILE, tt = (AT.nrows + FU_TILE - 1) / FU_TILE;
+        const size_t words = 16 + 8 * (size_t)G * CGO_NW + 4 * (size_t)(ta + tt);
+        const size_t cbytes = sizeof(double) * (size_t)(3 + 8) * (size_t)G * CGO_B;
+        const size_t wpad = (words + 255) & ~(size_t)255;
+        CGO_CUDA(cudaMalloc(&fs_mem, wpad + cbytes));
+        CGO_CUDA(cudaMemsetAsync(fs_mem, 0, wpad, ctx->stream));
+        char *p = (char *)fs_mem;
+        fs.frontier = (unsigned long long *)p;
+        fs.edone = fs.frontier + 1;
+        fs.chain_a = (unsigned int *)(p + 16);
+        fs.chain_d = fs.chain_a + (size_t)G * CGO_NW;
+        fs.cnt = fs.chain_d + (size_t)G * CGO_NW;
+        fs.cnt_a = fs.cnt + ta;
+        fs.carry_a = (double *)(p + wpad);
+        fs.carry_d = fs.carry_a + (size_t)3 * G * CGO_B;
+        fs_G = G;
+        return 0;
+    }
+    template <class X>
+    void fuse_queue(X &x, const CsrMat &M, int64_t na) {
+        x.na = na;
+        x.nslices = (M.nrows + 31) / 32;
+        x.ntd = (M.nrows + FU_TILE - 1) / FU_TILE;
+        x.nta = (na + FU_TILE - 1) / FU_TILE;
+        x.e0 = X::HAS_A ? M.early_col / FU_TILE : 0;
+        x.ne = X::HAS_A ? x.nta - x.e0 : 0;
+        x.lead = X::HAS_A ? M.reach_lead + FU_AHEAD : 0;
+        x.lag = FU_AHEAD;
+        x.steps = x.ntd + x.lead + x.lag > x.nta ? x.ntd + x.lead + x.lag : x.nta;
+        x.reach = M.reach;
+        x.fs = fs;
+    }
+    template <bool FUSED>
+    int eval_trial_ls_fused(cgo_state *st, double a, double beta, double *out) {
+        CGO_TRY(fuse_alloc());
+        DirFused<AxpyDir<FUSED, 0>, VecSumSq<true>> xab{};
+        AxpyDir<FUSED, 0> &ka = xab.opa;
+        ka.x = (const double2 *)st->x; ka.g = (const double2 *)st->g; ka.u = (double2 *)st->u;
+        ka.xp = (double2 *)st->xp; ka.a = a; ka.beta = FUSED ? beta : 0.0;
+        ka.prev_right = ka.next_left = nullptr; ka.hq = 0; ka.nq = st->n / 2; ka.dst_all = nullptr; ka.nranks = 1;
+        xab.opd.a = (const double2 *)r;
+        xab.ra = cgo_red_args(ctx, CGO_P_DIR_GU);
+        xab.rd = cgo_red_args(ctx, CGO_P_PHI);
+        xab.rd.partial = xab.ra.partial + (size_t)AxpyDir<FUSED, 0>::K * xab.ra.G;
+        xab.nd = nrows;
+        fuse_queue(xab, A, st->n);
+        DirResidual<false> f1{b, r, nullptr, nullptr, 0, nrows};
+        CGO_TRY(launch_direct(ctx, A, st->xp, f1, dir_args(ctx), CGO_T_SPMV, xab));
+        CGO_TRY(launch_direct(ctx, AT, r, DirGradLS{st->gp}, dir_args(ctx), CGO_T_SPMVT));
+        CGO_TRY(cgo_blas1_grad_dots(st));
+        CGO_TRY(cgo_finish_pack(ctx, 12, out));
+        out[CGO_P_PHI] = 0.5 * out[CGO_P_PHI];
+        return 0;
+    }
     int eval_trial_ls_direct(cgo_state *st, double a, bool fused, double beta, double *out) {
         const bool peer = r_is_peer && st->peer_x;
+        if (!peer && ctx->nranks == 1 && A.reach)
+            return fused ? eval_trial_ls_fused<true>(st, a, beta, out) : eval_trial_ls_fused<false>(st, a, 0.0, out);
         RedArgs fb, fc;
         if (peer) {
             const int R = ctx->nranks, me = ctx->rank, prev = (me + R - 1) % R, next = (me + 1) % R;
@@ -1425,6 +1780,7 @@
         if (ctx->csr_mode == 2 || (ctx->csr_mode == 0 && coh_log2 < 4 && K > 1)) {
             CGO_TRY(csr_make_sliced(ctx, o->A));
             CGO_TRY(csr_make_sliced(ctx, o->AT));
+            if (!multi && o->A.sliced) CGO_TRY(csr_build_reach(ctx, o->A, nloc));
         }
         return 0;
     };
@@ -1470,6 +1826,7 @@
         if (ctx->csr_mode == 2 || (ctx->csr_mode == 0 && la > 4.0f && lt > 4.0f && nrows >= 4096)) {
             CGO_TRY(csr_make_sliced(ctx, o->A));
             CGO_TRY(csr_make_sliced(ctx, o->AT));
+            if (o->A.sliced) CGO_TRY(csr_build_reach(ctx, o->A, ncols));
         }
         return 0;
     };
diff --git a/conjugategradientoptim.jl_b200/csrc/internal.cuh b/conjugategradientoptim.jl_b200/csrc/internal.cuh
--- a/conjugategradientoptim.jl_b200/csrc/internal.cuh
+++ b/conjugategradientoptim.jl_b200/csrc/internal.cuh
@@ -180,4 +180,6 @@
     int32_t ragged = 0;
     int64_t max_tile_nnz = 0;
     float lines_per_gather = 1.f;
+    int32_t *reach = nullptr;
+    int64_t early_col = 0, reach_lead = 0;
 };
diff --git a/conjugategradientoptim.jl_b200/csrc/reduce.cuh b/conjugategradientoptim.jl_b200/csrc/reduce.cuh
--- a/conjugategradientoptim.jl_b200/csrc/reduce.cuh
+++ b/conjugategradientoptim.jl_b200/csrc/reduce.cuh
@@ -47,6 +47,22 @@
 }
 
 template <int K, class Bar = BarAll>
+__device__ __forceinline__ void cgo_grid_sum(const RedArgs &red, int nact, double *sm, Bar bar = Bar()) {
+    double acc[K];
+#pragma unroll
+    for (int k = 0; k < K; ++k) {
+        double s = 0.0;
+        for (int c = threadIdx.x; c < nact; c += CGO_B) s = s + __ldcg(&red.partial[(size_t)k * red.G + c]);
+        acc[k] = s;
+    }
+    cgo_cta_combine<K, Bar>(acc, sm, bar);
+    if (threadIdx.x == 0) {
+#pragma unroll
+        for (int k = 0; k < K; ++k) red.out[k] = acc[k];
+    }
+}
+
+template <int K, class Bar = BarAll>
 __device__ __forceinline__ void cgo_grid_finish(const RedArgs &red, int nact, double *sm, Bar bar = Bar()) {
     __shared__ bool is_last;
     if (red.sig0 != nullptr || red.flags_all != nullptr) __threadfence_system();
@@ -59,17 +75,8 @@
     bar();
     if (!is_last) return;
     __threadfence();
-    double acc[K];
-#pragma unroll
-    for (int k = 0; k < K; ++k) {
-        double s = 0.0;
-        for (int c = threadIdx.x; c < nact; c += CGO_B) s = s + __ldcg(&red.partial[(size_t)k * red.G + c]);
-        acc[k] = s;
-    }
-    cgo_cta_combine<K, Bar>(acc, sm, bar);
+    cgo_grid_sum<K, Bar>(red, nact, sm, bar);
     if (threadIdx.x == 0) {
-#pragma unroll
-        for (int k = 0; k < K; ++k) red.out[k] = acc[k];
         *red.ticket = 0u;
         __threadfence_system();
         if (red.sig0 != nullptr) {
@@ -105,6 +112,11 @@
     asm volatile("ld.global.nc.L1::no_allocate.v2.f64 {%0, %1}, [%2];" : "=d"(r.x), "=d"(r.y) : "l"(p));
     return r;
 }
+__device__ __forceinline__ double2 cgo_ld2cg(const double2 *p) {
+    double2 r;
+    asm volatile("ld.global.cg.v2.f64 {%0, %1}, [%2];" : "=d"(r.x), "=d"(r.y) : "l"(p) : "memory");
+    return r;
+}
 __device__ __forceinline__ void cgo_st2(double2 *p, double2 v) {
     asm volatile("st.global.L1::no_allocate.v2.f64 [%0], {%1, %2};" ::"l"(p), "d"(v.x), "d"(v.y) : "memory");
 }
```

Result: slower. 43.62 (median of 6 runs) (-13.1%).
